# yahoo/bftkv

Measured on AMD Instinct MI355X. Metric: pgp_rsa2048_signature_verifies_per_sec, higher is better.
Workload: dtype u32; 1 GPU; 64-replica quorum, 10000 RSA-2048 signed writes per GPU (cfg2 of BASELINE.json), 534164 signature packets per GPU, 1.0% corrupt / 0.5% unknown issuer / 0.5% duplicate / 1.0% one-short; parallelism=shard-by-write x1, RCCL all-gather of verdict bitmaps on the verifier's stream, replicas=64, writes_per_gpu=10000, sigs_per_gpu=534164, batches_in_flight=3

## Files before the change

### bftkv_amd/_native.py

```python
from __future__ import annotations

import ctypes as C
import os
from typing import Optional

import numpy as np

_HERE = os.path.dirname(os.path.abspath(__file__))
LIB_PATH = os.path.join(_HERE, "libbftkv_gpu.so")


class NativeError(RuntimeError):
    pass


class PubKey(C.Structure):
    _fields_ = [("key_id", C.c_uint64), ("entity_id", C.c_uint64), ("pk_algo", C.c_uint8),
                ("usable_sign", C.c_uint8), ("reserved", C.c_uint8 * 6),
                ("n", C.c_void_p), ("n_len", C.c_uint32), ("e", C.c_void_p), ("e_len", C.c_uint32),
                ("g", C.c_void_p), ("g_len", C.c_uint32), ("y", C.c_void_p), ("y_len", C.c_uint32)]


class QC(C.Structure):
    _fields_ = [("f", C.c_int32), ("min", C.c_int32), ("threshold", C.c_int32), ("suff", C.c_int32),
                ("node_ids", C.c_void_p), ("n_nodes", C.c_uint32)]


EXPORTS = [
    "bftkv_gpu_init", "bftkv_gpu_destroy", "bftkv_gpu_last_error", "bftkv_gpu_error_string",
    "bftkv_gpu_keyring_set", "bftkv_gpu_quorum_create", "bftkv_gpu_quorum_destroy",
    "bftkv_gpu_collective_verify", "bftkv_gpu_collective_verify_dev", "bftkv_gpu_sync",
    "bftkv_gpu_signature_verify", "bftkv_gpu_last_statuses", "bftkv_gpu_last_counters",
    "bftkv_gpu_signers", "bftkv_gpu_quorum_tally", "bftkv_gpu_modexp", "bftkv_gpu_last_timing",
    "bftkv_gpu_stream", "bftkv_gpu_modmul_product", "bftkv_gpu_lagrange_combine", "bftkv_gpu_dsa_calculate_r", "bftkv_gpu_selftest_reduce",
    "bftkv_gpu_comm_unique_id", "bftkv_gpu_comm_init", "bftkv_gpu_allgather_verdicts", "bftkv_gpu_sss_distribute", "bftkv_gpu_modinv",
    "bftkv_gpu_batcher_create", "bftkv_gpu_batcher_destroy", "bftkv_gpu_batcher_collective_verify",
    "bftkv_gpu_batcher_signature_verify", "bftkv_gpu_batcher_stats", "bftkv_gpu_set_dsa_window_bits", "bftkv_gpu_dsa_window_bits", "bftkv_gpu_set_dsa_table_budget", "bftkv_gpu_dsa_table_bytes", "bftkv_gpu_collective_verify_segments", "bftkv_gpu_message_verify", "bftkv_gpu_batcher_message_verify",
    "bftkv_gpu_modexp_ops", "bftkv_gpu_allgather_errs_dev", "bftkv_gpu_set_early_exit", "bftkv_gpu_last_sclk_mhz", "bftkv_gpu_modmul_product_dev", "bftkv_gpu_lagrange_combine_dev",
    "bftkv_gpu_dsa_calculate_r_dev", "bftkv_gpu_sss_distribute_dev", "bftkv_gpu_modinv_dev",
    "bftkv_gpu_ctx_fork", "bftkv_gpu_batcher_create_lanes", "bftkv_gpu_batcher_times", "bftkv_gpu_comm_library", "bftkv_gpu_comm_selftest",
    "bftkv_gpu_collective_verify_small", "bftkv_gpu_signature_verify_small", "bftkv_gpu_set_hash_policy", "bftkv_gpu_signers_fenced",
    "bftkv_gpu_set_host_pipeline", "bftkv_gpu_batcher_cert_verify", "bftkv_gpu_host_pipeline_trace",
    "bftkv_gpu_batcher_cert_entity", "bftkv_gpu_set_lagrange_x_bound", "bftkv_gpu_batcher_modmul_product", "bftkv_gpu_batcher_lagrange_combine", "bftkv_gpu_batcher_dsa_calculate_r", "bftkv_gpu_batcher_modexp",
    "bftkv_gpu_ecdsa_calculate_r", "bftkv_gpu_ecdsa_calculate_r_dev", "bftkv_gpu_batcher_ecdsa_calculate_r", "bftkv_gpu_ec_scalar_base_mult",
    "bftkv_gpu_ecdsa_verify", "bftkv_gpu_ecdsa_verify_dev", "bftkv_gpu_batcher_ecdsa_verify",
    "bftkv_gpu_dsa_verify", "bftkv_gpu_dsa_verify_dev", "bftkv_gpu_batcher_dsa_verify",
    "bftkv_gpu_ecdsa_keyset_create", "bftkv_gpu_ecdsa_keyset_destroy", "bftkv_gpu_ecdsa_keyset_info", "bftkv_gpu_ecdsa_verify_keyset",
    "bftkv_gpu_ecdsa_verify_keyset_dev", "bftkv_gpu_batcher_ecdsa_verify_keyset", "bftkv_gpu_selftest_ecdsa_keyset_table",
    "bftkv_gpu_dsa_keyset_create", "bftkv_gpu_dsa_keyset_destroy", "bftkv_gpu_dsa_keyset_info", "bftkv_gpu_dsa_verify_keyset",
    "bftkv_gpu_dsa_verify_keyset_dev", "bftkv_gpu_batcher_dsa_verify_keyset", "bftkv_gpu_selftest_dsa_keyset_table",
    "bftkv_gpu_rsa_verify", "bftkv_gpu_rsa_verify_dev", "bftkv_gpu_rsa_keyset_create", "bftkv_gpu_rsa_keyset_destroy", "bftkv_gpu_rsa_keyset_info",
    "bftkv_gpu_rsa_verify_keyset", "bftkv_gpu_rsa_verify_keyset_dev", "bftkv_gpu_batcher_rsa_verify", "bftkv_gpu_batcher_rsa_verify_keyset",
]

_lib = None


def load_library() -> C.CDLL:
    global _lib
    if _lib is not None:
        return _lib
    if not os.path.exists(LIB_PATH):
        raise NativeError("%s not built -- run `python -c 'import __graft_entry__ as g; g.build()'`" % LIB_PATH)
    lib = C.CDLL(LIB_PATH)
    vp, u32, u64p, u8p = C.c_void_p, C.c_uint32, C.c_void_p, C.c_void_p
    lib.bftkv_gpu_init.argtypes = [C.c_int, C.POINTER(vp)]
    lib.bftkv_gpu_destroy.argtypes = [vp]
    lib.bftkv_gpu_destroy.restype = None
    lib.bftkv_gpu_last_error.argtypes = [vp]
    lib.bftkv_gpu_last_error.restype = C.c_char_p
    lib.bftkv_gpu_error_string.argtypes = [C.c_int]
    lib.bftkv_gpu_error_string.restype = C.c_char_p
    lib.bftkv_gpu_keyring_set.argtypes = [vp, C.POINTER(PubKey), u32]
    lib.bftkv_gpu_set_dsa_window_bits.argtypes = [vp, u32]
    lib.bftkv_gpu_dsa_window_bits.argtypes = [vp, C.POINTER(u32)]
    lib.bftkv_gpu_set_dsa_table_budget.argtypes = [vp, C.c_uint64]
    lib.bftkv_gpu_dsa_table_bytes.argtypes = [vp, C.POINTER(C.c_uint64), C.POINTER(u32)]
    lib.bftkv_gpu_set_hash_policy.argtypes = [vp, C.c_int, C.c_int]
    lib.bftkv_gpu_message_verify.argtypes = [vp, u32, vp, vp, vp, vp, vp, vp, C.c_uint64, vp, vp, vp]
    lib.bftkv_gpu_quorum_create.argtypes = [vp, C.POINTER(QC), u32, C.POINTER(C.c_int)]
    lib.bftkv_gpu_quorum_destroy.argtypes = [vp, C.c_int]
    lib.bftkv_gpu_collective_verify.argtypes = [vp, C.c_int, u32, u8p, u64p, u8p, u64p, u8p, vp, u8p, u8p]
    lib.bftkv_gpu_collective_verify_segments.argtypes = [vp, C.c_int, u32, u8p, u64p, u8p, u64p, u32, vp, u8p, u64p, u8p, vp, u8p, u8p]
    lib.bftkv_gpu_collective_verify_dev.argtypes = [vp, C.c_int, u32, u8p, u64p, u8p, u64p, C.c_uint64, u8p, vp, u8p, u8p]
    lib.bftkv_gpu_collective_verify_small.argtypes = [vp, C.c_int, u32, u8p, u64p, u8p, u64p, u8p, u8p]
    lib.bftkv_gpu_signature_verify_small.argtypes = [vp, u32, u8p, u64p, u8p, u64p, u64p, u8p, u8p]
    lib.bftkv_gpu_sync.argtypes = [vp]
    lib.bftkv_gpu_signature_verify.argtypes = [vp, u32, u8p, u64p, u8p, u64p, u64p, u8p, u8p]
    lib.bftkv_gpu_last_statuses.argtypes = [vp, u8p, vp, u32, C.POINTER(u32)]
    lib.bftkv_gpu_last_counters.argtypes = [vp, C.POINTER(C.c_uint64)]
    lib.bftkv_gpu_signers.argtypes = [vp, u32, u8p, u64p, u64p, u64p, C.c_uint64]
    lib.bftkv_gpu_signers_fenced.argtypes = [vp, u32, u8p, u64p, u64p, u64p, C.c_uint64, u8p]
    lib.bftkv_gpu_quorum_tally.argtypes = [vp, C.c_int, u32, u64p, u64p, u8p]
    lib.bftkv_gpu_modexp.argtypes = [vp, u32, u8p, u32, vp, u32, u8p, u8p, u32, u8p]
    lib.bftkv_gpu_last_timing.argtypes = [vp, C.POINTER(C.c_float)]
    lib.bftkv_gpu_modmul_product.argtypes = [vp, u32, u32, u8p, u32, vp, u32, u8p, u8p]
    lib.bftkv_gpu_lagrange_combine.argtypes = [vp, u32, u32, vp, u8p, u32, vp, u32, u8p, u8p, u8p]
    lib.bftkv_gpu_dsa_calculate_r.argtypes = [vp, u32, u32, vp, u8p, u32, u8p, u32, vp, u32, u8p, u8p, u8p, u8p]
    lib.bftkv_gpu_stream.argtypes = [vp]
    lib.bftkv_gpu_batcher_create.argtypes = [vp, u32, u32]
    lib.bftkv_gpu_batcher_create.restype = vp
    lib.bftkv_gpu_batcher_create_lanes.argtypes = [vp, u32, u32, u32]
    lib.bftkv_gpu_batcher_create_lanes.restype = vp
    lib.bftkv_gpu_ctx_fork.argtypes = [vp, C.POINTER(vp)]
    lib.bftkv_gpu_batcher_destroy.argtypes = [vp]
    lib.bftkv_gpu_batcher_destroy.restype = None
    lib.bftkv_gpu_batcher_collective_verify.argtypes = [vp, C.c_int, C.c_char_p, C.c_uint64, C.c_char_p, C.c_uint64, u8p, u8p]
    lib.bftkv_gpu_batcher_signature_verify.argtypes = [vp, C.c_char_p, C.c_uint64, C.c_char_p, C.c_uint64, vp, u8p, u8p]
    lib.bftkv_gpu_batcher_cert_verify.argtypes = [vp, C.c_char_p, C.c_uint64, C.c_char_p, C.c_uint64, C.c_char_p, C.c_uint64, u8p, u8p, vp, u8p]
    lib.bftkv_gpu_set_lagrange_x_bound.argtypes = [vp, u32]
    lib.bftkv_gpu_batcher_cert_entity.argtypes = [vp, C.c_char_p, C.c_uint64, u8p, u8p, vp, u8p, vp, vp, vp, u32, vp]
    lib.bftkv_gpu_batcher_message_verify.argtypes = [vp, C.c_char_p, C.c_uint64, vp, vp, vp, vp, C.c_uint64, vp, vp, vp]
    lib.bftkv_gpu_batcher_stats.argtypes = [vp, C.POINTER(C.c_uint64)]
    lib.bftkv_gpu_batcher_modmul_product.argtypes = [vp, u32, u8p, u32, u8p, u8p, u8p]
    lib.bftkv_gpu_batcher_lagrange_combine.argtypes = [vp, u32, vp, u8p, u32, u8p, u8p, u8p]
    lib.bftkv_gpu_batcher_dsa_calculate_r.argtypes = [vp, u32, vp, u8p, u32, u8p, u32, u8p, u8p, u8p, u8p]
    lib.bftkv_gpu_batcher_modexp.argtypes = [vp, u8p, u32, u8p, u32, u8p, u8p, u8p]
    lib.bftkv_gpu_batcher_times.argtypes = [vp, C.POINTER(C.c_uint64)]
    lib.bftkv_gpu_sss_distribute.argtypes = [vp, u32, u32, u32, u8p, u32, vp, u32, u8p, u8p]
    lib.bftkv_gpu_modinv.argtypes = [vp, u32, u8p, u32, vp, u32, u8p, u8p, u8p]
    lib.bftkv_gpu_comm_unique_id.argtypes = [u8p]
    lib.bftkv_gpu_comm_init.argtypes = [vp, C.c_int, C.c_int, u8p]
    lib.bftkv_gpu_comm_library.argtypes = [C.c_char_p, u32, C.POINTER(C.c_int)]
    lib.bftkv_gpu_comm_selftest.argtypes = [vp, u32, C.POINTER(u32)]
    lib.bftkv_gpu_allgather_verdicts.argtypes = [vp, u8p, C.c_uint64, u8p]
    lib.bftkv_gpu_stream.restype = vp
    lib.bftkv_gpu_set_early_exit.argtypes = [vp, C.c_int]
    lib.bftkv_gpu_set_host_pipeline.argtypes = [vp, u32]
    lib.bftkv_gpu_host_pipeline_trace.argtypes = [vp, C.POINTER(C.c_float), u32, C.POINTER(u32)]
    lib.bftkv_gpu_last_sclk_mhz.argtypes = [vp, C.POINTER(C.c_float)]
    lib.bftkv_gpu_modexp_ops.argtypes = lib.bftkv_gpu_modexp.argtypes
    lib.bftkv_gpu_allgather_errs_dev.argtypes = [vp, u8p, u32, u32, u8p]
    lib.bftkv_gpu_modmul_product_dev.argtypes = lib.bftkv_gpu_modmul_product.argtypes
    lib.bftkv_gpu_lagrange_combine_dev.argtypes = lib.bftkv_gpu_lagrange_combine.argtypes
    lib.bftkv_gpu_dsa_calculate_r_dev.argtypes = lib.bftkv_gpu_dsa_calculate_r.argtypes
    lib.bftkv_gpu_sss_distribute_dev.argtypes = lib.bftkv_gpu_sss_distribute.argtypes
    lib.bftkv_gpu_modinv_dev.argtypes = lib.bftkv_gpu_modinv.argtypes
    lib.bftkv_gpu_ecdsa_calculate_r.argtypes = [vp, u32, u32, vp, u8p, u8p, u8p, u32, u8p, u8p]
    lib.bftkv_gpu_ecdsa_calculate_r_dev.argtypes = lib.bftkv_gpu_ecdsa_calculate_r.argtypes
    lib.bftkv_gpu_batcher_ecdsa_calculate_r.argtypes = [vp, u32, vp, u8p, u8p, u8p, u32, u8p, u8p]
    lib.bftkv_gpu_ec_scalar_base_mult.argtypes = [vp, u32, u8p, u32, u8p, u32, u8p, u8p]
    lib.bftkv_gpu_ecdsa_verify.argtypes = [vp, u32, u8p, u32, u8p, vp, u32, u8p, u8p, u32, u8p, u8p]
    lib.bftkv_gpu_ecdsa_verify_dev.argtypes = lib.bftkv_gpu_ecdsa_verify.argtypes
    lib.bftkv_gpu_batcher_ecdsa_verify.argtypes = [vp, u8p, u32, u8p, u8p, u8p, u32, u8p, u8p]
    lib.bftkv_gpu_dsa_verify.argtypes = [vp, u32, u8p, u32, u8p, u32, vp, u32, u8p, vp, u32, u32, u8p, u8p, u8p, u8p, u8p]
    lib.bftkv_gpu_dsa_verify_dev.argtypes = lib.bftkv_gpu_dsa_verify.argtypes
    lib.bftkv_gpu_batcher_dsa_verify.argtypes = [vp, u8p, u32, u8p, u32, u8p, u32, u8p, u8p, u8p, u8p, u8p]
    lib.bftkv_gpu_ecdsa_keyset_create.argtypes = [vp, u32, u8p, u8p, u32, C.POINTER(C.c_int)]
    lib.bftkv_gpu_ecdsa_keyset_destroy.argtypes = [vp, C.c_int]
    lib.bftkv_gpu_ecdsa_keyset_info.argtypes = [vp, C.c_int, C.POINTER(u32), C.POINTER(u32), C.POINTER(u32), C.POINTER(C.c_uint64)]
    lib.bftkv_gpu_ecdsa_verify_keyset.argtypes = [vp, C.c_int, u32, u8p, u32, u8p, vp, u8p, u8p]
    lib.bftkv_gpu_ecdsa_verify_keyset_dev.argtypes = lib.bftkv_gpu_ecdsa_verify_keyset.argtypes
    lib.bftkv_gpu_batcher_ecdsa_verify_keyset.argtypes = [vp, C.c_int, u32, u8p, u32, u8p, u8p, u8p]
    lib.bftkv_gpu_selftest_ecdsa_keyset_table.argtypes = [vp, C.c_int, u32, vp, C.c_uint64]
    lib.bftkv_gpu_dsa_keyset_create.argtypes = [vp, u32, u8p, vp, u32, u32, u8p, u8p, u8p, u32, u32, C.POINTER(C.c_int)]
    lib.bftkv_gpu_dsa_keyset_destroy.argtypes = [vp, C.c_int]
    lib.bftkv_gpu_dsa_keyset_info.argtypes = [vp, C.c_int] + [C.POINTER(u32)] * 6 + [C.POINTER(C.c_uint64)]
    lib.bftkv_gpu_dsa_verify_keyset.argtypes = [vp, C.c_int, u32, u8p, u32, u8p, vp, u8p, u8p]
    lib.bftkv_gpu_dsa_verify_keyset_dev.argtypes = lib.bftkv_gpu_dsa_verify_keyset.argtypes
    lib.bftkv_gpu_batcher_dsa_verify_keyset.argtypes = [vp, C.c_int, u32, u8p, u32, u8p, u8p, u8p]
    lib.bftkv_gpu_selftest_dsa_keyset_table.argtypes = [vp, C.c_int, u32, vp, C.c_uint64]
    lib.bftkv_gpu_rsa_verify.argtypes = [vp, u32, u8p, u32, u32, u8p, u32, vp, u32, u8p, vp, u8p, u8p]
    lib.bftkv_gpu_rsa_verify_dev.argtypes = lib.bftkv_gpu_rsa_verify.argtypes
    lib.bftkv_gpu_rsa_keyset_create.argtypes = [vp, u32, u8p, vp, u32, C.POINTER(C.c_int)]
    lib.bftkv_gpu_rsa_keyset_destroy.argtypes = [vp, C.c_int]
    lib.bftkv_gpu_rsa_keyset_info.argtypes = [vp, C.c_int] + [C.POINTER(u32)] * 3
    lib.bftkv_gpu_rsa_verify_keyset.argtypes = [vp, C.c_int, u32, u8p, u32, u32, u8p, vp, u8p, u8p]
    lib.bftkv_gpu_rsa_verify_keyset_dev.argtypes = lib.bftkv_gpu_rsa_verify_keyset.argtypes
    lib.bftkv_gpu_batcher_rsa_verify.argtypes = [vp, u8p, u32, u32, u8p, u32, u8p, u32, u8p, u8p]
    lib.bftkv_gpu_batcher_rsa_verify_keyset.argtypes = [vp, C.c_int, u32, u8p, u32, u32, u8p, u8p, u8p]
    for name in EXPORTS:
        if name not in ("bftkv_gpu_destroy", "bftkv_gpu_last_error", "bftkv_gpu_error_string", "bftkv_gpu_stream",
                        "bftkv_gpu_batcher_create", "bftkv_gpu_batcher_create_lanes", "bftkv_gpu_batcher_destroy"):
            getattr(lib, name).restype = C.c_int
    _lib = lib
    return lib


def _ptr(a: Optional[np.ndarray]):
    if a is None:
        return None
    assert a.flags["C_CONTIGUOUS"]
    return a.ctypes.data_as(C.c_void_p)


class Context:

    def __init__(self, device: int = 0):
        self.lib = load_library()
        h = C.c_void_p()
        rc = self.lib.bftkv_gpu_init(device, C.byref(h))
        if rc != 0:
            raise NativeError("bftkv_gpu_init(device=%d) failed with %d: no usable MI355X / HIP runtime "
                              "(there is no CPU fallback)" % (device, rc))
        self.h = h
        self._keep = []

    def close(self):
        if self.h:
            self.lib.bftkv_gpu_destroy(self.h)
            self.h = None

    def set_hash_policy(self, hash_id: int, state: int):
        self._check(self.lib.bftkv_gpu_set_hash_policy(self.h, hash_id, state), "set_hash_policy")

    def fork(self) -> "Context":
        h = C.c_void_p()
        self._check(self.lib.bftkv_gpu_ctx_fork(self.h, C.byref(h)), "ctx_fork")
        f = Context.__new__(Context)
        f.lib, f.h, f._keep, f.root = self.lib, h, [], self
        return f

    def __del__(self):
        try:
            self.close()
        except Exception:
            pass

    def _check(self, rc: int, what: str):
        if rc != 0:
            raise NativeError("%s failed (%d): %s" % (what, rc, self.lib.bftkv_gpu_last_error(self.h).decode()))

    def keyring_set(self, keys):
        keys = list(keys)
        arr = (PubKey * max(1, len(keys)))()
        bufs = []
        for i, k in enumerate(keys):
            arr[i].key_id = k["key_id"]
            arr[i].entity_id = k.get("entity_id", k["key_id"])
            arr[i].pk_algo = k["pk_algo"]
            arr[i].usable_sign = 1 if k.get("usable_sign", True) else 0
            for name in ("n", "e", "g", "y"):
                b = k.get(name) or b""
                cb = C.create_string_buffer(b, len(b)) if b else None
                bufs.append(cb)
                setattr(arr[i], name, C.cast(cb, C.c_void_p) if cb is not None else None)
                setattr(arr[i], name + "_len", len(b))
        self._check(self.lib.bftkv_gpu_keyring_set(self.h, arr, len(keys)), "keyring_set")

    def message_verify(self, messages):
        n = len(messages)
        blob = np.frombuffer(b"".join(messages), dtype=np.uint8) if n and sum(map(len, messages)) else np.zeros(1, dtype=np.uint8)
        off = np.zeros(n + 1, dtype=np.uint64)
        off[1:] = np.cumsum([len(m) for m in messages], dtype=np.uint64)
        st = np.zeros(max(1, n), dtype=np.uint8)
        signer = np.zeros(max(1, n), dtype=np.uint64)
        peer = np.zeros(max(1, n), dtype=np.uint64)
        plain = np.zeros(max(1, int(off[n])), dtype=np.uint8)
        poff = np.zeros(n + 1, dtype=np.uint64)
        fn = np.zeros((max(1, n), 256), dtype=np.uint8)
        fl = np.zeros(max(1, n), dtype=np.uint8)
        self._check(self.lib.bftkv_gpu_message_verify(self.h, n, _ptr(np.ascontiguousarray(blob)), _ptr(off), _ptr(st), _ptr(signer), _ptr(peer),
                                                      _ptr(plain), len(plain), _ptr(poff), _ptr(fn), _ptr(fl)), "message_verify")
        plains = [plain[int(poff[i]):int(poff[i + 1])].tobytes() for i in range(n)]
        names = [fn[i, :int(fl[i])].tobytes() for i in range(n)]
        return st[:n], signer[:n], peer[:n], plains, names

    def set_early_exit(self, on: bool) -> None:
        self._check(self.lib.bftkv_gpu_set_early_exit(self.h, 1 if on else 0), "set_early_exit")

    def set_host_pipeline(self, pieces: int, copy: str = "", tight: bool = False) -> None:
        mode = {"": 0, "ring": 0x100, "direct": 0x200}[copy]
        self._check(self.lib.bftkv_gpu_set_host_pipeline(self.h, pieces | mode | (0x400 if tight else 0)), "set_host_pipeline")

    def host_pipeline_trace(self):
        buf = (C.c_float * 96)()
        n = C.c_uint32(0)
        self._check(self.lib.bftkv_gpu_host_pipeline_trace(self.h, buf, 96, C.byref(n)), "host_pipeline_trace")
        v = [float(buf[i]) for i in range(min(96, n.value))]
        if not v:
            return None
        P = int(v[0])
        names = ("ss_enqueued", "payload_enqueued", "picked_up", "payload_hook", "enqueued", "drained", "gpu_start", "gpu_modexp_start", "gpu_modexp_end", "gpu_end")
        return {"pieces": P, "ring": bool(v[1]), "copiers_joined_us": v[2], "copy_stream_drained_us": v[3], "done_us": v[4], "largest_piece_items": int(v[5]), "second_passes": int(v[6]),
                "per_piece_us": [{nm: round(v[8 + 10 * k + j], 1) for j, nm in enumerate(names)} for k in range(P)]}

    def set_dsa_window_bits(self, bits: int) -> None:
        self._check(self.lib.bftkv_gpu_set_dsa_window_bits(self.h, bits), "set_dsa_window_bits")

    def dsa_window_bits(self) -> int:
        b = C.c_uint32(0)
        self._check(self.lib.bftkv_gpu_dsa_window_bits(self.h, C.byref(b)), "dsa_window_bits")
        return int(b.value)

    def set_dsa_table_budget(self, nbytes: int) -> None:
        self._check(self.lib.bftkv_gpu_set_dsa_table_budget(self.h, int(nbytes)), "set_dsa_table_budget")

    def dsa_table_bytes(self):
        b, e = C.c_uint64(0), C.c_uint32(0)
        self._check(self.lib.bftkv_gpu_dsa_table_bytes(self.h, C.byref(b), C.byref(e)), "dsa_table_bytes")
        return int(b.value), int(e.value)

    def quorum_create(self, qcs) -> int:
        qcs = list(qcs)
        arr = (QC * max(1, len(qcs)))()
        keep = []
        for i, (f, mn, thr, suff, nodes) in enumerate(qcs):
            ids = np.ascontiguousarray(np.array(list(nodes), dtype=np.uint64))
            keep.append(ids)
            arr[i].f, arr[i].min, arr[i].threshold, arr[i].suff = f, mn, thr, suff
            arr[i].node_ids = ids.ctypes.data if len(ids) else None
            arr[i].n_nodes = len(ids)
        out = C.c_int(-1)
        self._check(self.lib.bftkv_gpu_quorum_create(self.h, arr, len(qcs), C.byref(out)), "quorum_create")
        return out.value

    def quorum_destroy(self, q: int):
        self._check(self.lib.bftkv_gpu_quorum_destroy(self.h, q), "quorum_destroy")

    def collective_verify(self, quorum: int, tbs_blob, tbs_off, ss_blob, ss_off):
        n = len(tbs_off) - 1
        tbs_blob, ss_blob = _u8(tbs_blob), _u8(ss_blob)
        tbs_off, ss_off = _u64(tbs_off), _u64(ss_off)
        err = np.zeros(n, dtype=np.uint8)
        nver = np.zeros(n, dtype=np.uint32)
        verdict = np.zeros(n, dtype=np.uint8)
        self.last_fenced = np.zeros(n, dtype=np.uint8)
        small = self.collective_verify_small(quorum, tbs_blob, tbs_off, ss_blob, ss_off) if self._cross_check(n) else None
        self._check(self.lib.bftkv_gpu_collective_verify(self.h, quorum, n, _ptr(tbs_blob), _ptr(tbs_off), _ptr(ss_blob),
                                                         _ptr(ss_off), _ptr(err), _ptr(nver), _ptr(verdict), _ptr(self.last_fenced)),
                    "collective_verify")
        self._compare_small("collective_verify", small, err, self.last_fenced)
        return err, nver, verdict

    check_small = False

    def collective_verify_segments(self, quorum: int, prefix_blob, prefix_off, shared_blob, shared_off, seg_of_item, ss_blob, ss_off):
        n = len(prefix_off) - 1
        prefix_blob, shared_blob, ss_blob = _u8(prefix_blob), _u8(shared_blob), _u8(ss_blob)
        prefix_off, shared_off, ss_off = _u64(prefix_off), _u64(shared_off), _u64(ss_off)
        seg = np.ascontiguousarray(seg_of_item, dtype=np.uint32)
        err = np.zeros(n, dtype=np.uint8)
        nver = np.zeros(n, dtype=np.uint32)
        verdict = np.zeros(n, dtype=np.uint8)
        self.last_fenced = np.zeros(n, dtype=np.uint8)
        self._check(self.lib.bftkv_gpu_collective_verify_segments(self.h, quorum, n, _ptr(prefix_blob), _ptr(prefix_off), _ptr(shared_blob),
                                                                  _ptr(shared_off), len(shared_off) - 1, _ptr(seg), _ptr(ss_blob), _ptr(ss_off),
                                                                  _ptr(err), _ptr(nver), _ptr(verdict), _ptr(self.last_fenced)),
                    "collective_verify_segments")
        return err, nver, verdict

    def _cross_check(self, n: int) -> bool:
        return bool(self.check_small) and 0 < n <= 4096

    @staticmethod
    def _compare_small(what, small, err, fenced):
        if small is None:
            return
        e2, f2 = small
        if not (np.array_equal(e2, err) and np.array_equal(f2, fenced)):
            bad = [int(i) for i in np.nonzero((e2 != err) | (f2 != fenced))[0][:8]]
            raise NativeError("%s: the small-call route disagrees with the batched one at items %s: err %s vs %s, fenced %s vs %s"
                              % (what, bad, e2[bad].tolist(), err[bad].tolist(), f2[bad].tolist(), fenced[bad].tolist()))

    def collective_verify_small(self, quorum: int, tbs_blob, tbs_off, ss_blob, ss_off):
        n = len(tbs_off) - 1
        tbs_blob, ss_blob = _u8(tbs_blob), _u8(ss_blob)
        tbs_off, ss_off = _u64(tbs_off), _u64(ss_off)
        err = np.zeros(n, dtype=np.uint8)
        fenced = np.zeros(n, dtype=np.uint8)
        self._check(self.lib.bftkv_gpu_collective_verify_small(self.h, quorum, n, _ptr(tbs_blob), _ptr(tbs_off), _ptr(ss_blob), _ptr(ss_off),
                                                               _ptr(err), _ptr(fenced)), "collective_verify_small")
        return err, fenced

    def signature_verify_small(self, tbs_blob, tbs_off, sig_blob, sig_off, cert_key_id=None):
        n = len(tbs_off) - 1
        tbs_blob, sig_blob = _u8(tbs_blob), _u8(sig_blob)
        tbs_off, sig_off = _u64(tbs_off), _u64(sig_off)
        ck = None if cert_key_id is None else _u64(cert_key_id)
        err = np.zeros(n, dtype=np.uint8)
        fenced = np.zeros(n, dtype=np.uint8)
        self._check(self.lib.bftkv_gpu_signature_verify_small(self.h, n, _ptr(tbs_blob), _ptr(tbs_off), _ptr(sig_blob), _ptr(sig_off), _ptr(ck),
                                                              _ptr(err), _ptr(fenced)), "signature_verify_small")
        return err, fenced

    def collective_verify_dev(self, quorum: int, n_items: int, tbs_ptr: int, tbs_off_ptr: int, ss_ptr: int, ss_off_ptr: int,
                              ss_len: int, err_ptr: int, nver_ptr: int, verdict_ptr: int, fenced_ptr: int = 0):
        self._check(self.lib.bftkv_gpu_collective_verify_dev(self.h, quorum, n_items, tbs_ptr, tbs_off_ptr, ss_ptr, ss_off_ptr,
                                                             ss_len, err_ptr, nver_ptr, verdict_ptr, fenced_ptr or None), "collective_verify_dev")

    def sync(self):
        self._check(self.lib.bftkv_gpu_sync(self.h), "sync")

    def signature_verify(self, tbs_blob, tbs_off, sig_blob, sig_off, cert_key_id=None):
        n = len(tbs_off) - 1
        tbs_blob, sig_blob = _u8(tbs_blob), _u8(sig_blob)
        tbs_off, sig_off = _u64(tbs_off), _u64(sig_off)
        ck = None if cert_key_id is None else _u64(cert_key_id)
        err = np.zeros(n, dtype=np.uint8)
        self.last_fenced = np.zeros(n, dtype=np.uint8)
        small = self.signature_verify_small(tbs_blob, tbs_off, sig_blob, sig_off, cert_key_id) if self._cross_check(n) else None
        self._check(self.lib.bftkv_gpu_signature_verify(self.h, n, _ptr(tbs_blob), _ptr(tbs_off), _ptr(sig_blob), _ptr(sig_off),
                                                        _ptr(ck), _ptr(err), _ptr(self.last_fenced)), "signature_verify")
        self._compare_small("signature_verify", small, err, self.last_fenced)
        return err

    def last_statuses(self):
        n = C.c_uint32(0)
        self._check(self.lib.bftkv_gpu_last_statuses(self.h, None, None, 0, C.byref(n)), "last_statuses")
        st = np.zeros(max(1, n.value), dtype=np.uint8)
        item = np.zeros(max(1, n.value), dtype=np.uint32)
        self._check(self.lib.bftkv_gpu_last_statuses(self.h, _ptr(st), _ptr(item), n.value, C.byref(n)), "last_statuses")
        return st[:n.value], item[:n.value]

    def last_counters(self):
        c = (C.c_uint64 * 4)()
        self._check(self.lib.bftkv_gpu_last_counters(self.h, c), "last_counters")
        return {"packets": c[0], "pubkey_ops": c[1], "items": c[2], "dsa_ops": c[3]}

    def last_sclk_mhz(self) -> float:
        v = C.c_float(0)
        self._check(self.lib.bftkv_gpu_last_sclk_mhz(self.h, C.byref(v)), "last_sclk_mhz")
        return float(v.value)

    def last_timing(self):
        ms = (C.c_float * 8)()
        self._check(self.lib.bftkv_gpu_last_timing(self.h, ms), "last_timing")
        return {"total": ms[0], "parse": ms[1], "hash": ms[2], "rsa": ms[3], "tally": ms[4], "compare": ms[5], "dsa": ms[6]}

    def signers(self, ss_blob, ss_off):
        n = len(ss_off) - 1
        ss_blob, ss_off = _u8(ss_blob), _u64(ss_off)
        cap = max(1, int(len(ss_blob) // 12) + 1)
        ids = np.zeros(cap, dtype=np.uint64)
        off = np.zeros(n + 1, dtype=np.uint64)
        self.last_fenced = np.zeros(n, dtype=np.uint8)
        self._check(self.lib.bftkv_gpu_signers_fenced(self.h, n, _ptr(ss_blob), _ptr(ss_off), _ptr(ids), _ptr(off), cap, _ptr(self.last_fenced)), "signers")
        return ids[:int(off[n])], off

    def quorum_tally(self, quorum: int, ids, list_off):
        n = len(list_off) - 1
        ids, list_off = _u64(ids), _u64(list_off)
        v = np.zeros(n, dtype=np.uint8)
        self._check(self.lib.bftkv_gpu_quorum_tally(self.h, quorum, n, _ptr(ids), _ptr(list_off), _ptr(v)), "quorum_tally")
        return v

    @staticmethod
    def comm_unique_id() -> np.ndarray:
        uid = np.zeros(128, dtype=np.uint8)
        rc = load_library().bftkv_gpu_comm_unique_id(_ptr(uid))
        if rc:
            raise NativeError("bftkv_gpu_comm_unique_id failed (%d): librccl not loadable" % rc)
        return uid

    def comm_init(self, n_ranks: int, rank: int, uid: np.ndarray):
        self._check(self.lib.bftkv_gpu_comm_init(self.h, n_ranks, rank, _ptr(np.ascontiguousarray(uid, dtype=np.uint8))), "comm_init")

    @staticmethod
    def comm_library():
        buf = C.create_string_buffer(1024)
        pre = C.c_int(0)
        rc = load_library().bftkv_gpu_comm_library(buf, 1024, C.byref(pre))
        if rc:
            raise NativeError("bftkv_gpu_comm_library failed (%d): librccl not loadable" % rc)
        return buf.value.decode(), bool(pre.value)

    def comm_selftest(self, nbytes: int = 4096):
        bad = C.c_uint32(0)
        self._check(self.lib.bftkv_gpu_comm_selftest(self.h, nbytes, C.byref(bad)), "comm_selftest")

    def allgather_verdicts(self, local_ptr: int, nbytes: int, out_ptr: int):
        self._check(self.lib.bftkv_gpu_allgather_verdicts(self.h, local_ptr, nbytes, out_ptr), "allgather_verdicts")

    def allgather_errs_dev(self, err_ptr: int, n_items: int, slots: int, out_ptr: int):
        self._check(self.lib.bftkv_gpu_allgather_errs_dev(self.h, err_ptr, n_items, slots, out_ptr), "allgather_errs_dev")

    def modmul_product(self, factors, moduli, mod_idx, nbytes: int = 256):
        n, k = len(factors), len(factors[0])
        f = _ints_to_be([x for row in factors for x in row], nbytes)
        m = _ints_to_be(moduli, nbytes)
        mi = np.ascontiguousarray(mod_idx, dtype=np.uint32)
        out = np.zeros((n, nbytes), dtype=np.uint8)
        self._check(self.lib.bftkv_gpu_modmul_product(self.h, n, k, _ptr(f), nbytes, _ptr(mi), len(moduli), _ptr(m), _ptr(out)), "modmul_product")
        return [int.from_bytes(out[i].tobytes(), "big") for i in range(n)]

    def lagrange_combine(self, xs, ys, moduli, mod_idx, nbytes: int = 256):
        n, k = len(xs), len(xs[0])
        x = np.ascontiguousarray(np.array(xs, dtype=np.int32))
        y = _ints_to_be([v for row in ys for v in row], nbytes)
        m = _ints_to_be(moduli, nbytes)
        mi = np.ascontiguousarray(mod_idx, dtype=np.uint32)
        out = np.zeros((n, nbytes), dtype=np.uint8)
        st = np.zeros(n + 8, dtype=np.uint8)
        self._check(self.lib.bftkv_gpu_lagrange_combine(self.h, n, k, _ptr(x), _ptr(y), nbytes, _ptr(mi), len(moduli), _ptr(m), _ptr(out),
                                                        _ptr(st)), "lagrange_combine")
        return [int.from_bytes(out[i].tobytes(), "big") for i in range(n)], st[:n]

    def dsa_calculate_r(self, xs, ri, vi, groups, group_idx, pbytes: int = 256, qbytes: int = 32):
        n, k = len(xs), len(xs[0])
        x = np.ascontiguousarray(np.array(xs, dtype=np.int32))
        r = _ints_to_be([v for row in ri for v in row], pbytes)
# ... 445 lines not shown
```

### bftkv_amd/csrc/capi.hip

```cpp
#include "../../include/bftkv_gpu.h"

#include <hip/hip_runtime.h>
#include <stdio.h>
#include <stdlib.h>
#include <string.h>

#include <limits.h>
#include <linux/futex.h>
#include <sched.h>
#include <sys/syscall.h>
#include <unistd.h>

#include <algorithm>
#include <array>
#include <atomic>
#include <memory>
#include <functional>
#include <map>
#include <set>
#include <chrono>
#include <condition_variable>
#include <mutex>
#include <shared_mutex>
#include <system_error>
// ... 16 lines not shown

inline void copy_out(void* dst, const void* src, size_t n) { if (n) memcpy(dst, src, n); }

struct DevBuf {
  void* p = nullptr;
  size_t cap = 0;
  hipError_t ensure(size_t bytes) {
    if (bytes <= cap) return hipSuccess;
    if (p) { hipError_t e = hipFree(p); if (e != hipSuccess) return e; p = nullptr; cap = 0; }
    size_t want = bytes + bytes / 4 + 256;
    hipError_t e = hipMalloc(&p, want);
    if (e == hipSuccess) cap = want;
    return e;
  }
  hipError_t ensure_exact(size_t bytes) {
    if (bytes <= cap) return hipSuccess;
    if (p) { hipError_t e = hipFree(p); if (e != hipSuccess) return e; p = nullptr; cap = 0; }
    hipError_t e = hipMalloc(&p, bytes);
    if (e == hipSuccess) cap = bytes;
    return e;
  }
  void release() { if (p) (void)hipFree(p); p = nullptr; cap = 0; }
  template <typename T> T* as() const { return (T*)p; }
};

struct KeyEntry {
  uint64_t key_id = 0, entity_id = 0;
  uint8_t algo = 0, flags = 0;
  uint32_t bits = 0, e = 0, n0 = 0, qbits = 0, n0_29 = 0;
  std::vector<uint32_t> nl29, r2_29;
  std::vector<uint32_t> nl, r2, r2w, qw, dtab, qpow, qconst;
  std::string material;
  bool cert_only = false;
  int cert_group = -1;
  uint32_t entity_index = 0;
  std::string cert_digest;
  uint64_t last_used = 0;
  bool dsa_unslotted = false;
};

struct QuorumHost {
  bool live = false;
  int n_qcs = 0;
  int32_t f[MAX_QC], mn[MAX_QC], thr[MAX_QC], suff[MAX_QC];
  std::vector<std::vector<uint64_t>> nodes;
  DevBuf member;
  uint64_t keyring_gen = ~0ull;
  DevBuf ids;
  uint32_t ids_off[MAX_QC + 1];
};

struct EcKeySet {
  bool live = false;
  int curve_id = -1;
  uint32_t bits = 0, n_keys = 0, n_refused = 0;
  uint32_t w = 0, nwin = 0;
  size_t key_words = 0;
  std::vector<uint8_t> curve;
  DevBuf tab;
  DevBuf refused;
  DevBuf mod[4];
  void release() { tab.release(); refused.release(); for (DevBuf& b : mod) b.release(); }
};

struct DsaKeySet {
  bool live = false;
  uint32_t n_keys = 0, n_groups = 0, pbytes = 0, qbytes = 0;
  uint32_t w = 0, windows = 0;
  DevBuf tab;
  DevBuf modp[3], modq[3];
  DevBuf q_be, key_group;
  uint64_t table_bytes() const { return (uint64_t)(n_groups + n_keys) * windows * ((1u << w) - 1u) * MONT_N * 4; }
  static ModTab rows(const DevBuf (&m)[3]) { return ModTab{m[0].as<uint32_t>(), m[1].as<uint32_t>(), m[2].as<uint32_t>(), nullptr}; }
  void release() { tab.release(); q_be.release(); key_group.release(); for (DevBuf& b : modp) b.release(); for (DevBuf& b : modq) b.release(); }
};

struct RsaKeySet {
  bool live = false;
  uint32_t n_keys = 0, n_refused = 0, nbytes = 0;
  DevBuf n29, r2_29, n80, r2_80;
  DevBuf meta;
  void release() { n29.release(); r2_29.release(); n80.release(); r2_80.release(); meta.release(); }
};

}

using ctx_lock = std::lock_guard<std::recursive_mutex>;

struct bftkv_gpu_ctx {
  int device = 0;
  hipStream_t stream = nullptr;
  hipStream_t stream_h = nullptr;
  hipStream_t stream_d = nullptr;
  std::recursive_mutex mu;
  std::string err;

  uint64_t keyring_gen = 0;
  uint32_t n_keys = 0, n_entities = 0;
  bool have_dsa_keys = false, have_rsa3072 = false, have_rsa4096 = false, have_ambiguous = false;
  std::vector<uint64_t> h_key_id, h_entity_id;
  std::vector<uint32_t> h_key_entity;
  std::vector<uint8_t> h_key_flags;
  std::vector<KeyEntry> ring, certs;
  uint32_t n_ring_entities = 0;
  std::map<std::string, bool> cert_valid;
  DevBuf k_r2w;
  DevBuf k_n29, k_r2_29, k_n0_29;
  DevBuf k_id, k_entity, k_algo, k_flags, k_bits, k_e, k_n, k_r2, k_n0, k_q, k_qbits, k_dsatab, k_dsaslot, k_sorted_id, k_sorted_slot;
  DevBuf dsa_comb;
  uint32_t dsa_wbits = 8, dsa_wbits_pinned = 0;
  std::map<std::string, uint32_t> dsa_comb_slot;
  std::set<std::string> dsa_cert_materials;
  uint64_t ring_epoch = 0, dsa_ring_epoch_seen = ~0ull;
  uint32_t dsa_wbits_want = 0;
  uint32_t dsa_entry_limbs = DSA_N_SMALL;
  size_t dsa_budget_bytes = 0;
  bool have_dsa3072 = false, have_dsa2048 = false;
  DevBuf dsa_idx;
  uint64_t cert_clock = 0;
  struct CertFast { uint64_t issuer_id; int group; uint64_t epoch; };
  std::shared_mutex cert_fast_mu;
  std::unordered_map<std::string, CertFast> cert_fast;
  size_t cert_fast_bytes = 0;
  uint64_t cert_epoch = 0, kt_cert_epoch = 0;
  std::vector<uint32_t> kt_group_ent;
  KeyTableDev kt{};

  std::vector<QuorumHost> quorums;
  std::vector<EcKeySet> ec_keysets;
  std::vector<DsaKeySet> dsa_keysets;
  std::vector<RsaKeySet> rsa_keysets;

  DevBuf txt_mid32, txt_mid64, txt_tail, txt_len;
  DevBuf forced_iss;
  DevBuf counts, base, total, item_flags, walk_scratch, cert_ent, sig_class, mid, mid64, hash_mask, recs, digests, r, xr, pk_list, pk_list3072, pk_list4096, r3072, r4096, pk_count, dsa_list, dsa_u, ids_tmp;
  DevBuf o_err, o_nver, o_verdict, o_fenced;
  DevBuf in_tbs, in_tbs_off, in_ss, in_ss_off;
  hipEvent_t seg_ev = nullptr;
  DevBuf in_prefix, in_prefix_off, in_shared, in_shared_off, in_seg;
  DevBuf st_tmp, item_tmp, bits_tmp, plan_cut;
  DevBuf chunk_arena, chunk_ctr;
  uint32_t multiexp_parts = 0;
  uint32_t ec_split = 0;
  uint32_t ec_window = 0;
  DevBuf ec_fb_tab[4];
  uint32_t ec_fb_w[4] = {};
  uint32_t multiexp_block = 0;
  uint32_t multiexp_lanes = 0;
  uint32_t rsav_lanes = 0;
  uint32_t dsa_inv_mode = 0;
  uint32_t n_cus = 256;
  uint32_t lagrange_x_bound = 0;
  bool early_exit = true;
  std::vector<DevBuf*> scratch_pool;
  std::unordered_map<std::string, std::vector<uint32_t>> modrow_cache;
  std::unordered_map<std::string, std::vector<uint32_t>> rsav_row_cache[2];
  std::map<std::string, std::array<DevBuf, 4>> modtab_cache;
  uint32_t* h_mail = nullptr;
  uint32_t* d_mail = nullptr;
  uint32_t last_total = 0, last_rsa = 0, last_items = 0;
  bool last_total_on_dev = false;
  hipEvent_t ev[10] = {};
  hipEvent_t ev_turn = nullptr;
  bool have_timing = false;
  void* rccl_comm = nullptr;
  int n_ranks = 1, rank = 0;

  bftkv_gpu_ctx* root = nullptr;
  std::shared_mutex kt_rw;
  std::atomic<int> kt_writers{0};
  std::atomic<int> n_forks{0};
  uint64_t quorum_gen = 0;
  uint64_t seen_keyring_gen = ~0ull, seen_quorum_gen = ~0ull;
  size_t n_dsa_slots = 0;
  int kt_read_depth = 0;
  DevBuf in_pack;
  uint8_t* h_out = nullptr; uint8_t* d_out = nullptr; size_t out_cap = 0;
  uint32_t out_seq = 0;
  std::vector<bftkv_gpu_ctx*> hb_workers;
  hipStream_t stream_c = nullptr;
  hipStream_t stream_c2 = nullptr;
  std::vector<hipEvent_t> hb_ev;
  uint8_t* hb_out = nullptr; size_t hb_out_cap = 0;
  uint32_t modexp_lds_pad = 0;
  uint32_t hb_pieces = 0;
  hipEvent_t hb_ev0 = nullptr;
  bool hb_tight = false;
  uint32_t hb_copy_mode = 0;
  void* hb_ring = nullptr;
  std::vector<float> hb_trace;
  uint32_t hb_last_pieces = 0;
  std::vector<uint32_t> hb_item0;
  void* small_pin = nullptr;
  uint32_t staged_spin_us = 50000;
};

void rccl_release(bftkv_gpu_ctx* c);
void release_small_pin(bftkv_gpu_ctx* c);
extern "C" int signature_verify_entities(bftkv_gpu_ctx* c, uint32_t n_items, const uint8_t* tbs, const uint64_t* tbs_off, const uint8_t* sig,
                                         const uint64_t* sig_off, const uint32_t* ent, uint8_t* err_out, const uint8_t* sig_class = nullptr,
                                         uint8_t* fenced_out = nullptr, const uint64_t* forced_issuer = nullptr);

namespace {

int fork_refresh(bftkv_gpu_ctx* c);

struct KtWrite {
  bftkv_gpu_ctx* c;
  explicit KtWrite(bftkv_gpu_ctx* c_) : c(c_) { c->kt_writers.fetch_add(1); c->kt_rw.lock(); }
  ~KtWrite() { c->kt_rw.unlock(); c->kt_writers.fetch_sub(1); }
};
struct KtRead {
  bftkv_gpu_ctx *c, *r;
  int rc = 0;
  explicit KtRead(bftkv_gpu_ctx* c_) : c(c_), r(c_->root) {
    if (!r || c->kt_read_depth++ > 0) return;
    while (r->kt_writers.load(std::memory_order_acquire) > 0) std::this_thread::yield();
    r->kt_rw.lock_shared();
    rc = fork_refresh(c);
  }
  ~KtRead() { if (r && --c->kt_read_depth == 0) r->kt_rw.unlock_shared(); }
};

struct Turnstile { std::mutex mu; hipEvent_t last = nullptr; const void* owner = nullptr; };
Turnstile g_turnstile[16];
constexpr uint64_t HB_PIPE_MIN_BYTES = 24ull << 20;
constexpr uint32_t HB_PIPE_MAX_PIECES = 8;
std::mutex g_hb_mu[16];
constexpr size_t HB_TR = 10;
struct HbRing {
  static constexpr size_t SLOT = 16u << 20;
  static constexpr int NSLOT = 6;
  static constexpr int THREADS = 4;
  uint8_t* base = nullptr;
  hipEvent_t ev[NSLOT] = {};
  bool used[NSLOT] = {};
// ... 138 lines not shown
  HIPCHK(c, c->mid.ensure(sizeof(uint32_t) * 8 * N_MID32 * (size_t)n_items + 16));
  HIPCHK(c, c->mid64.ensure(sizeof(uint64_t) * 8 * 2 * (size_t)n_items + 16));
  HIPCHK(c, c->hash_mask.ensure(sizeof(uint32_t) * (size_t)n_items + 16));
  constexpr size_t CHUNK_ARENA_MIN = 64u << 10;
  if (!c->chunk_ctr.p) { HIPCHK(c, c->chunk_ctr.ensure(16)); HIPCHK(c, hipMemsetAsync(c->chunk_ctr.p, 0, 16, c->stream)); }
  HIPCHK(c, c->chunk_arena.ensure(CHUNK_ARENA_MIN + (staged_cap ? 2 * (size_t)ss_len : 0)));
  HIPCHK(c, c->pk_count.ensure(96));
  if (plan_q) HIPCHK(c, c->plan_cut.ensure(sizeof(uint32_t) * (size_t)n_items + 16));
  TextDev txt{nullptr, nullptr, nullptr, nullptr};
  if (!d_mid_in) {
    HIPCHK(c, c->txt_mid32.ensure(sizeof(uint32_t) * 8 * N_MID32 * (size_t)n_items + 16));
    HIPCHK(c, c->txt_mid64.ensure(sizeof(uint64_t) * 8 * N_MID64 * (size_t)n_items + 16));
    HIPCHK(c, c->txt_tail.ensure((size_t)128 * N_HASHES * n_items + 16));
    HIPCHK(c, c->txt_len.ensure(sizeof(uint64_t) * N_HASHES * (size_t)n_items + 16));
    txt = TextDev{c->txt_mid32.as<uint32_t>(), c->txt_mid64.as<uint64_t>(), c->txt_tail.as<uint8_t>(), c->txt_len.as<uint64_t>()};
  }
  if (ev_input) HIPCHK(c, hipStreamWaitEvent(s, ev_input, 0));
  HIPCHK(c, rec(0, s));
  HIPCHK(c, join(sh, 0));
  HIPCHK(c, rec(5, sh));
  if (!upload_tbs && !d_mid_in)
    hipLaunchKernelGGL(k_sha256_mid, dim3((n_items + 63) / 64), dim3(64), 0, sh, d_tbs, d_tbs_off, n_items, c->mid.as<uint32_t>());
  hipLaunchKernelGGL(k_walk<false>, dim3(n_items), dim3(64), 0, s, d_ss, d_ss_off, n_items, c->counts.as<uint32_t>(),
                     (const uint32_t*)nullptr, (SigRec*)nullptr, c->item_flags.as<uint8_t>(), c->walk_scratch.as<WalkEnt>(), walk_cap,
                     c->chunk_ctr.as<uint32_t>());
  constexpr uint32_t MAIL_EMPTY = 0xFFFFFFFFu;
  if (c->h_mail && !staged_cap) __atomic_store_n(&c->h_mail[0], MAIL_EMPTY, __ATOMIC_RELEASE);
  hipLaunchKernelGGL(k_scan_counts, dim3(1), dim3(1024), 0, s, c->counts.as<uint32_t>(), n_items, c->base.as<uint32_t>(),
                     c->total.as<uint32_t>(), staged_cap ? (uint32_t*)nullptr : c->d_mail, c->pk_count.as<uint32_t>(), c->hash_mask.as<uint32_t>(),
                     staged_cap, c->chunk_ctr.as<uint32_t>());
  uint32_t total = staged_cap ? staged_cap : MAIL_EMPTY;
  const uint32_t* const n_recs_dev = staged_cap ? c->total.as<uint32_t>() : nullptr;
  if (c->h_mail && !staged_cap) {
    const auto t_spin = std::chrono::steady_clock::now();
    for (uint32_t it = 0;; ++it) {
      total = __atomic_load_n(&c->h_mail[0], __ATOMIC_ACQUIRE);
      if (total != MAIL_EMPTY) break;
      if ((it & 1023u) == 1023u && std::chrono::steady_clock::now() - t_spin > std::chrono::milliseconds(20)) break;
      __builtin_ia32_pause();
    }
  }
  uint32_t chunk_units = (c->h_mail && !staged_cap && total != MAIL_EMPTY) ? c->h_mail[2] : 0u;
  if (total == MAIL_EMPTY) {
    HIPCHK(c, hipMemcpyAsync(&total, c->total.p, sizeof(uint32_t), hipMemcpyDeviceToHost, s));
    HIPCHK(c, hipMemcpyAsync(&chunk_units, c->chunk_ctr.as<uint32_t>() + 2, sizeof(uint32_t), hipMemcpyDeviceToHost, s));
    HIPCHK(c, hipStreamSynchronize(s));
  }
  if (!staged_cap && (size_t)chunk_units * 16 > c->chunk_arena.cap) HIPCHK(c, c->chunk_arena.ensure((size_t)chunk_units * 16));
  c->last_total = staged_cap ? 0u : total;
  c->last_total_on_dev = staged_cap != 0 && ev_input != nullptr;
  c->last_items = n_items;
  c->hb_last_pieces = 0;
  const size_t tr = total ? total : 1;
  HIPCHK(c, c->recs.ensure(sizeof(SigRec) * tr));
  HIPCHK(c, c->digests.ensure(sizeof(uint32_t) * 16 * tr));
  HIPCHK(c, c->r.ensure(sizeof(uint32_t) * EM_LOW_LIMBS * tr));
  HIPCHK(c, c->xr.ensure(sizeof(uint32_t) * (c->have_rsa4096 ? MONT_NMAX : c->have_rsa3072 ? MONT_TPI_BIG * MONT_L3072 : 80) * tr));
  HIPCHK(c, c->pk_list.ensure(sizeof(uint32_t) * tr));
  HIPCHK(c, c->pk_list3072.ensure(c->have_rsa3072 ? sizeof(uint32_t) * tr : 16));
  HIPCHK(c, c->pk_list4096.ensure(c->have_rsa4096 ? sizeof(uint32_t) * tr : 16));
  if (c->have_rsa3072) HIPCHK(c, c->r3072.ensure(sizeof(uint32_t) * EM_LOW_LIMBS * tr));
  if (c->have_rsa4096) HIPCHK(c, c->r4096.ensure(sizeof(uint32_t) * EM_LOW_LIMBS * tr));
  HIPCHK(c, c->dsa_list.ensure(sizeof(uint32_t) * tr));
  if (c->have_dsa_keys) HIPCHK(c, c->dsa_u.ensure(sizeof(uint32_t) * DSA_U_WORDS * tr));
  if (c->have_dsa3072 && c->have_dsa2048) HIPCHK(c, c->dsa_idx.ensure(sizeof(uint32_t) * 4 * (size_t)tr + 16));
  hipLaunchKernelGGL(k_walk<true>, dim3(n_items), dim3(64), 0, s, d_ss, d_ss_off, n_items, c->counts.as<uint32_t>(),
                     c->base.as<uint32_t>(), c->recs.as<SigRec>(), c->item_flags.as<uint8_t>(), (WalkEnt*)nullptr, walk_cap, (uint32_t*)nullptr);
  if (total) {
    ParseArgs pa;
    pa.sig_blob = d_ss; pa.sig_off = d_ss_off; pa.rec_base = c->base.as<uint32_t>(); pa.counts = c->counts.as<uint32_t>(); pa.n_items = n_items;
    pa.scratch = c->walk_scratch.as<WalkEnt>(); pa.walk_cap = walk_cap; pa.recs = c->recs.as<SigRec>(); pa.n_recs = total; pa.cert_ent = d_cert_ent;
    pa.pk_list = c->pk_list.as<uint32_t>(); pa.pk_list3072 = c->pk_list3072.as<uint32_t>(); pa.pk_list4096 = c->pk_list4096.as<uint32_t>();
    pa.pk_count = c->pk_count.as<uint32_t>(); pa.dsa_list = c->dsa_list.as<uint32_t>(); pa.item_hash_mask = c->hash_mask.as<uint32_t>();
    pa.sig_class = d_sig_class; pa.forced_issuer = d_forced_issuer; pa.msg_slot = d_msg_slot; pa.msg_hash = d_msg_hash; pa.item_flags = c->item_flags.as<uint8_t>();
    pa.defer_queue = plan_q ? 1u : 0u;
    pa.n_recs_dev = n_recs_dev;
    pa.chunk_arena = c->chunk_arena.as<uint8_t>(); pa.chunk_cap_units = (uint32_t)std::min<size_t>(c->chunk_arena.cap / 16, 0xFFFFFFF0u);
    pa.chunk_bump = c->chunk_ctr.as<uint32_t>() + 1;
    if (!staged_cap && (uint64_t)total >= 128ull * n_items)
      hipLaunchKernelGGL(k_parse_body_items, dim3(n_items), dim3(PARSE_ITEM_BLOCK), 0, s, pa, c->kt);
    else
      hipLaunchKernelGGL(k_parse_body, dim3((total + 255) / 256), dim3(256), 0, s, pa, c->kt);
  }
  uint32_t* const cnt_p = c->pk_count.as<uint32_t>();
  const uint32_t* const start0 = cnt_p + 12;
  PlanArgs pl{};
  if (total && plan_q) {
    pl.recs = c->recs.as<SigRec>(); pl.rec_base = c->base.as<uint32_t>(); pl.counts = c->counts.as<uint32_t>(); pl.n_items = n_items;
    pl.pk_list = c->pk_list.as<uint32_t>(); pl.dsa_list = c->dsa_list.as<uint32_t>(); pl.pk_list3072 = c->pk_list3072.as<uint32_t>();
    pl.pk_list4096 = c->pk_list4096.as<uint32_t>(); pl.pk_count = cnt_p; pl.plan_cut = c->plan_cut.as<uint32_t>(); pl.verdict = nullptr;
    int min_suff = 0;
    for (int i = 0; i < plan_q->n_qcs; ++i) if (plan_q->suff[i] > 0 && (min_suff == 0 || plan_q->suff[i] < min_suff)) min_suff = plan_q->suff[i];
    pl.margin = 1u + (uint32_t)min_suff / 64u;
    pl.mail = c->d_mail ? c->d_mail + 3 : nullptr;
    if (c->h_mail) __atomic_store_n(&c->h_mail[3], 0u, __ATOMIC_RELEASE);
    hipLaunchKernelGGL(k_plan<1>, dim3((n_items + PLAN_ITEMS - 1) / PLAN_ITEMS), dim3(PLAN_BLOCK), 0, s, pl, c->kt, *plan_q);
  }
  const bool dsa_side = total && c->have_dsa_keys;
  if (one_stream && dsa_side) HIPCHK(c, hipEventRecord(c->ev[1], s)); else HIPCHK(c, rec(1, s));
  const size_t n_slots = c->root ? c->n_dsa_slots : c->dsa_comb_slot.size();
  const uint32_t inv_batch_min = c->dsa_inv_mode == 1 || n_slots > (c->dsa_inv_mode == 2 ? (size_t)INV_MAX_SLOTS : 256) ? 0xFFFFFFFFu
                                 : c->dsa_inv_mode == 2 ? 0u : (uint32_t)std::max<size_t>(4096, 64 * n_slots);
  auto launch_dsa_inv = [&](hipStream_t st, const uint32_t* start) {
    if (inv_batch_min != 0xFFFFFFFFu)
      hipLaunchKernelGGL(k_dsa_inv_batched, dim3((total + INV_TILE - 1) / INV_TILE), dim3(INV_BLOCK), 0, st, d_ss, c->recs.as<SigRec>(),
                         c->dsa_list.as<uint32_t>(), c->pk_count.as<uint32_t>(), start, c->kt, c->dsa_u.as<uint32_t>(), inv_batch_min);
    if (inv_batch_min != 0u)
      hipLaunchKernelGGL(k_dsa_inv, dim3((total + 63) / 64), dim3(64), 0, st, d_ss, c->recs.as<SigRec>(), c->dsa_list.as<uint32_t>(),
                         c->pk_count.as<uint32_t>(), start, c->kt, c->dsa_u.as<uint32_t>(), inv_batch_min);
  };
  if (total && c->have_dsa_keys) {
    HIPCHK(c, hipStreamWaitEvent(c->stream_d, c->ev[1], 0));
    launch_dsa_inv(c->stream_d, start0);
    HIPCHK(c, hipEventRecord(c->ev[7], c->stream_d));
  }
  auto hash_stream_work = [&]() -> int {
    HIPCHK(c, join(sh, 1));
    if (total) {
      if (!d_mid_in) {
        hipLaunchKernelGGL(k_hash_mid_other, dim3((n_items + 63) / 64, N_HASHES - 1), dim3(64), 0, sh, d_tbs, d_tbs_off, n_items,
                           c->hash_mask.as<uint32_t>(), c->mid.as<uint32_t>(), c->mid64.as<uint64_t>());
        hipLaunchKernelGGL(k_hash_mid_text, dim3((n_items + 63) / 64, N_HASHES), dim3(64), 0, sh, d_tbs, d_tbs_off, n_items, c->hash_mask.as<uint32_t>(), txt);
      }
      hipLaunchKernelGGL(k_digest_sha256, dim3((total + 255) / 256), dim3(256), 0, sh, d_tbs, d_tbs_off, d_ss,
                         d_mid_in ? d_mid_in : c->mid.as<uint32_t>(), c->mid64.as<uint64_t>(), n_items, c->recs.as<SigRec>(), total,
                         c->digests.as<uint32_t>(), d_tbs_prefix, n_recs_dev);
    }
    HIPCHK(c, rec(6, sh));
    return 0;
  };
  if (!upload_tbs) { int hrc = hash_stream_work(); if (hrc) return hrc; }
  const dim3 qg((total + MODEXP_BLOCK / MONT_TPI - 1) / (MODEXP_BLOCK / MONT_TPI));
  const dim3 qg8((total + MODEXP_BLOCK / MONT_TPI_BIG - 1) / (MODEXP_BLOCK / MONT_TPI_BIG));
  static const bool wide8_off = getenv("BFTKV_NO_WIDE8") != nullptr;
  const bool wide8 = staged_cap != 0 && ss_len / 256 <= 8192 && !wide8_off;
  auto launch_modexp = [&](const uint32_t* start) {
    if (wide8)
      hipLaunchKernelGGL((k_rsa_modexp<10, MONT_TPI_BIG>), qg8, dim3(MODEXP_BLOCK), 0, s, d_ss, c->recs.as<SigRec>(), c->pk_list.as<uint32_t>(),
                         cnt_p, start, c->kt, c->r.as<uint32_t>(), c->xr.as<uint32_t>(), (uint64_t*)(cnt_p + 16));
    else {
#if BFTKV_RSA_FORM == 29
      hipLaunchKernelGGL((k_rsa_modexp<RSA29_L, MONT_TPI, RSA29_W>), qg, dim3(MODEXP_BLOCK), c->modexp_lds_pad, s, d_ss, c->recs.as<SigRec>(), c->pk_list.as<uint32_t>(),
                         cnt_p, start, c->kt, c->r.as<uint32_t>(), c->xr.as<uint32_t>(), (uint64_t*)(cnt_p + 16), (const uint32_t*)(cnt_p + 5));
      hipLaunchKernelGGL((k_rsa_modexp<MONT_L, MONT_TPI, MONT_W, true>), qg, dim3(MODEXP_BLOCK), c->modexp_lds_pad, s, d_ss, c->recs.as<SigRec>(), c->pk_list.as<uint32_t>(),
                         cnt_p, start, c->kt, c->r.as<uint32_t>(), c->xr.as<uint32_t>(), (uint64_t*)nullptr, (const uint32_t*)(cnt_p + 5));
#else
      hipLaunchKernelGGL((k_rsa_modexp<MONT_L, MONT_TPI>), qg, dim3(MODEXP_BLOCK), c->modexp_lds_pad, s, d_ss, c->recs.as<SigRec>(), c->pk_list.as<uint32_t>(),
                         cnt_p, start, c->kt, c->r.as<uint32_t>(), c->xr.as<uint32_t>(), (uint64_t*)(cnt_p + 16));
#endif
    }
    if (c->have_rsa3072)
      hipLaunchKernelGGL((k_rsa_modexp<MONT_L3072, MONT_TPI_BIG>), qg8, dim3(MODEXP_BLOCK), 0, s, d_ss, c->recs.as<SigRec>(), c->pk_list3072.as<uint32_t>(),
                         cnt_p + 2, start + 2, c->kt, c->r3072.as<uint32_t>(), c->xr.as<uint32_t>(), (uint64_t*)nullptr);
    if (c->have_rsa4096)
      hipLaunchKernelGGL((k_rsa_modexp<MONT_L4096, MONT_TPI_BIG>), qg8, dim3(MODEXP_BLOCK), 0, s, d_ss, c->recs.as<SigRec>(), c->pk_list4096.as<uint32_t>(),
                         cnt_p + 3, start + 3, c->kt, c->r4096.as<uint32_t>(), c->xr.as<uint32_t>(), (uint64_t*)nullptr);
  };
  static const bool turnstile_off = getenv("BFTKV_NO_TURNSTILE") != nullptr;
  const bool big = staged_cap ? (ev_input != nullptr && ss_len / 320 >= TURNSTILE_MIN_PACKETS) : total >= TURNSTILE_MIN_PACKETS;
  if (big && !turnstile_off) {
    Turnstile& g = g_turnstile[(unsigned)c->device & 15u];
    std::lock_guard<std::mutex> tl(g.mu);
    if (g.last && g.owner != c) HIPCHK(c, hipStreamWaitEvent(s, g.last, 0));
    HIPCHK(c, rec(9, s));
    launch_modexp(start0);
    if (!c->ev_turn) HIPCHK(c, hipEventCreateWithFlags(&c->ev_turn, hipEventDisableTiming));
    HIPCHK(c, hipEventRecord(c->ev_turn, s));
    g.last = c->ev_turn; g.owner = c;
  } else {
    HIPCHK(c, rec(9, s));
    if (total) launch_modexp(start0);
  }
  HIPCHK(c, rec(2, s));
  if (upload_tbs) {
    int hrc = (*upload_tbs)(sh);
    if (hrc) return hrc;
    if (!mid_prelaunched)
      hipLaunchKernelGGL(k_sha256_mid, dim3((n_items + 63) / 64), dim3(64), 0, sh, d_tbs, d_tbs_off, n_items, c->mid.as<uint32_t>());
    if ((hrc = hash_stream_work())) return hrc;
  }
  HIPCHK(c, join(s, 6));
  bool other_hashes = true;
  if (total && !d_mid_in && plan_q && big && c->h_mail) {
    const auto t_spin = std::chrono::steady_clock::now();
    for (uint32_t it = 0;; ++it) {
      const uint32_t v = __atomic_load_n(&c->h_mail[3], __ATOMIC_ACQUIRE);
      if (v) { other_hashes = (v & 1u) != 0; break; }
      if ((it & 255u) == 255u && std::chrono::steady_clock::now() - t_spin > std::chrono::microseconds(300) + std::chrono::nanoseconds((uint64_t)total / 2)) break;
      __builtin_ia32_pause();
    }
  }
  if (total && !d_mid_in && other_hashes)
    hipLaunchKernelGGL(k_digest_other, dim3(std::min<uint32_t>((total + 255) / 256, DIGEST_OTHER_MAX_BLOCKS)), dim3(256), 0, s,
                       d_tbs, d_tbs_off, d_ss, c->mid.as<uint32_t>(), c->mid64.as<uint64_t>(), n_items, c->recs.as<SigRec>(), total,
                       c->digests.as<uint32_t>(), c->pk_count.as<uint32_t>() + 4, txt, n_recs_dev);
  const dim3 cg(((uint64_t)total * CMP_LANES + 255) / 256);
  auto launch_compare = [&](const uint32_t* start) {
    hipLaunchKernelGGL(k_rsa_compare, cg, dim3(256), 0, s, c->recs.as<SigRec>(), c->pk_list.as<uint32_t>(),
                       cnt_p, start, c->kt, c->r.as<uint32_t>(), c->digests.as<uint32_t>());
    if (c->have_rsa3072)
      hipLaunchKernelGGL(k_rsa_compare, cg, dim3(256), 0, s, c->recs.as<SigRec>(), c->pk_list3072.as<uint32_t>(),
                         cnt_p + 2, start + 2, c->kt, c->r3072.as<uint32_t>(), c->digests.as<uint32_t>());
    if (c->have_rsa4096)
      hipLaunchKernelGGL(k_rsa_compare, cg, dim3(256), 0, s, c->recs.as<SigRec>(), c->pk_list4096.as<uint32_t>(),
                         cnt_p + 3, start + 3, c->kt, c->r4096.as<uint32_t>(), c->digests.as<uint32_t>());
  };
  auto launch_dsa = [&](const uint32_t* start) {
    hipLaunchKernelGGL(k_dsa_mul, dim3((total + 63) / 64), dim3(64), 0, s, c->recs.as<SigRec>(), c->dsa_list.as<uint32_t>(),
                       cnt_p, start, c->kt, c->digests.as<uint32_t>(), c->dsa_u.as<uint32_t>());
    const uint32_t* idx_s = nullptr; const uint32_t* idx_b = nullptr; const uint32_t* cnt_cls = nullptr;
    if (c->have_dsa3072 && c->have_dsa2048) {
      uint32_t* cc = cnt_p + (start == start0 ? 20 : 22);
      uint32_t* is = c->dsa_idx.as<uint32_t>() + (start == start0 ? 0 : 2 * (size_t)total);
      hipLaunchKernelGGL(k_dsa_split, dim3((total + 255) / 256), dim3(256), 0, s, c->recs.as<SigRec>(), c->dsa_list.as<uint32_t>(), cnt_p, start, c->kt,
                         is, is + total, cc);
      idx_s = is; idx_b = is + total; cnt_cls = cc;
    }
    if (c->have_dsa2048)
      hipLaunchKernelGGL((k_dsa_modexp<MONT_L, MONT_TPI>), dim3((total + QUADS_PER_BLOCK - 1) / QUADS_PER_BLOCK), dim3(RSA_BLOCK), 0, s,
                         c->recs.as<SigRec>(), c->dsa_list.as<uint32_t>(), cnt_p, start, c->kt, c->dsa_u.as<uint32_t>(), idx_s, cnt_cls);
    if (c->have_dsa3072)
      hipLaunchKernelGGL((k_dsa_modexp<MONT_L3072, MONT_TPI_BIG>), dim3((total + RSA_BLOCK / MONT_TPI_BIG - 1) / (RSA_BLOCK / MONT_TPI_BIG)), dim3(RSA_BLOCK), 0, s,
                         c->recs.as<SigRec>(), c->dsa_list.as<uint32_t>(), cnt_p, start, c->kt, c->dsa_u.as<uint32_t>(), idx_b, cnt_cls ? cnt_cls + 1 : nullptr);
  };
  if (total) launch_compare(start0);
  HIPCHK(c, rec(8, s));
  if (total && c->have_dsa_keys) {
    HIPCHK(c, hipStreamWaitEvent(s, c->ev[7], 0));
    launch_dsa(start0);
  }
  if (total && plan_q) {
    HIPCHK(c, c->o_nver.ensure(sizeof(uint32_t) * n_items));
    HIPCHK(c, c->o_verdict.ensure(n_items));
    hipLaunchKernelGGL(k_tally, dim3((n_items + 3) / 4), dim3(256), 0, s, c->recs.as<SigRec>(), c->base.as<uint32_t>(), c->counts.as<uint32_t>(),
                       n_items, c->kt, *plan_q, c->o_verdict.as<uint8_t>(), c->o_nver.as<uint32_t>(), (uint32_t*)nullptr);
    hipLaunchKernelGGL(k_plan_snapshot, dim3(1), dim3(64), 0, s, cnt_p);
    pl.verdict = c->o_verdict.as<uint8_t>();
    hipLaunchKernelGGL(k_plan<2>, dim3((n_items + PLAN_ITEMS - 1) / PLAN_ITEMS), dim3(PLAN_BLOCK), 0, s, pl, c->kt, *plan_q);
    const uint32_t* const start1 = cnt_p + 8;
    if (c->have_dsa_keys) launch_dsa_inv(s, start1);
    launch_modexp(start1);
    launch_compare(start1);
    if (c->have_dsa_keys) launch_dsa(start1);
  }
  if (total && c->have_ambiguous && !d_msg_slot)
    hipLaunchKernelGGL(k_candidates, dim3((total + 63) / 64), dim3(64), 0, s, d_tbs, d_tbs_off, d_ss, d_mid_in ? d_mid_in : c->mid.as<uint32_t>(),
                       c->mid64.as<uint64_t>(), n_items, c->recs.as<SigRec>(), total, n_recs_dev, d_tbs_prefix, c->kt, d_cert_ent, d_sig_class, txt,
                       c->hash_mask.as<uint32_t>());
  HIPCHK(c, rec(3, s));
  HIPCHK(c, hipGetLastError());
  return 0;
}

int make_key_entry(bftkv_gpu_ctx* c, const bftkv_gpu_pubkey& k, bool cert_only, KeyEntry* out) {
  KeyEntry& e = *out;
  e.key_id = k.key_id; e.entity_id = k.entity_id; e.algo = k.pk_algo; e.cert_only = cert_only;
  e.material.clear();
  e.material.push_back((char)k.pk_algo);
  e.material.push_back((char)k.usable_sign);
  auto app = [&](const uint8_t* p, uint32_t l) {
    uint32_t z = 0;
    while (z < l && p[z] == 0) ++z;
    if (l > z) e.material.append((const char*)p + z, l - z);
    e.material.push_back('|');
  };
  app(k.n, k.n_len); app(k.e, k.e_len); app(k.g, k.g_len); app(k.y, k.y_len);
  e.flags = 0;
  if (k.usable_sign) e.flags |= KEYF_USABLE_SIGN;
  if (k.pk_algo != PK_RSA_ENCRYPT_ONLY && k.pk_algo != PK_ELGAMAL) e.flags |= KEYF_CAN_SIGN;
  if (k.key_id == k.entity_id) e.flags |= KEYF_PRIMARY;
  if (cert_only) e.flags |= KEYF_CERT_ONLY;
  e.bits = (uint32_t)hostbn::bit_length(k.n, k.n_len);
  e.e = 0; e.n0 = 0; e.qbits = 0;
  e.r2w.clear(); e.nl29.clear(); e.r2_29.clear(); e.n0_29 = 0;
  e.nl.assign(MONT_NMAX, 0); e.r2.assign(MONT_NMAX, 0); e.qw.assign(8, 0); e.dtab.assign(2 * DSA_N_BIG, 0); e.qpow.clear(); e.qconst.clear();
  if (k.pk_algo == PK_RSA || k.pk_algo == PK_RSA_SIGN_ONLY) {
    if (hostbn::bit_length(k.e, k.e_len) > 32) return fail(c, BFTKV_E_UNSUPPORTED, "RSA public exponent wider than 32 bits");
    for (uint32_t j = 0; j < k.e_len; ++j) e.e = (e.e << 8) | k.e[j];
    const int nlimbs = e.bits <= 2048 ? MONT_N : (e.bits <= 3072 ? MONT_TPI_BIG * MONT_L3072 : MONT_TPI_BIG * MONT_L4096);
    if (e.bits > 4096) e.bits = 0xFFFFFFFFu;
    else if (!hostbn::mont_setup(k.n, k.n_len, nlimbs, e.nl.data(), e.r2.data(), &e.n0)) e.bits = 0xFFFFFFFFu;
    else if (e.bits <= 2048) {
      std::vector<uint32_t> nl80(80);
      uint32_t n0b = 0;
      e.r2w.assign(80, 0);
      (void)hostbn::mont_setup(k.n, k.n_len, 80, nl80.data(), e.r2w.data(), &n0b);
      e.nl29.assign(RSA29_N, 0); e.r2_29.assign(RSA29_N, 0);
      (void)hostbn::mont_setup(k.n, k.n_len, RSA29_N, e.nl29.data(), e.r2_29.data(), &e.n0_29, RSA29_W);
    }
  } else if (k.pk_algo == PK_DSA) {
    e.qbits = (uint32_t)hostbn::bit_length(k.e, k.e_len);
    const int NLp = e.bits <= 2048 ? (int)DSA_N_SMALL : (int)DSA_N_BIG;
    const uint32_t cap_bits = e.bits <= 2048 ? 2048u : 3072u;
    const int nwords = (28 * NLp + 31) / 32 + 1;
    std::vector<uint32_t> p(nwords), g(nwords), y(nwords), q(nwords);
    hostbn::from_be(k.e, k.e_len, q.data(), nwords);
    bool ok = e.bits >= 2 && e.bits <= 3072 && e.qbits >= 32 && e.qbits <= 256 && (q[0] & 1u) &&
              hostbn::mont_setup(k.n, k.n_len, NLp, e.nl.data(), e.r2.data(), &e.n0);
    if (ok && (hostbn::bit_length(k.g, k.g_len) > cap_bits || hostbn::bit_length(k.y, k.y_len) > cap_bits)) ok = false;
    if (ok) {
      hostbn::from_be(k.n, k.n_len, p.data(), nwords);
      hostbn::from_be(k.g, k.g_len, g.data(), nwords);
      hostbn::from_be(k.y, k.y_len, y.data(), nwords);
      hostbn::reduce(g.data(), p.data(), nwords);
      hostbn::reduce(y.data(), p.data(), nwords);
      hostbn::to_mont_limbs(g.data(), p.data(), nwords, NLp, &e.dtab[0]);
      hostbn::to_mont_limbs(y.data(), p.data(), nwords, NLp, &e.dtab[DSA_N_BIG]);
      for (int j = 0; j < 8; ++j) e.qw[j] = q[j];
      e.qpow.assign((size_t)NLp * 10, 0);
      uint32_t x[9] = {1, 0, 0, 0, 0, 0, 0, 0, 0}, q9[9];
      for (int j = 0; j < 9; ++j) q9[j] = j < 8 ? q[j] : 0;
      for (int j = 0; j < NLp; ++j) {
        hostbn::to_limbs28(x, 9, &e.qpow[(size_t)j * 10], 10);
        for (int b = 0; b < MONT_W; ++b) hostbn::dbl_mod(x, q9, 9);
      }
      e.qconst.assign(12, 0);
      uint32_t r2q[9] = {1, 0, 0, 0, 0, 0, 0, 0, 0};
      for (int b = 0; b < 512; ++b) hostbn::dbl_mod(r2q, q9, 9);
      for (int j = 0; j < 8; ++j) e.qconst[j] = r2q[j];
      uint32_t inv = 1;
      for (int it = 0; it < 5; ++it) inv *= 2u - q[0] * inv;
      e.qconst[8] = 0u - inv;
    } else {
      e.bits = 0xFFFFFFFFu;
// ... 221 lines not shown
    const_cast<KeyEntry&>(e).entity_index = group_ent;
    if (e.cert_group >= 0) {
      if (group_ents.size() <= (size_t)e.cert_group) group_ents.resize((size_t)e.cert_group + 1, 0xFFFFFFFEu);
      group_ents[(size_t)e.cert_group] = group_ent;
    }
  }
  std::vector<uint32_t> sorted_slot(key_id.size());
  for (size_t i = 0; i < sorted_slot.size(); ++i) sorted_slot[i] = (uint32_t)i;
  std::stable_sort(sorted_slot.begin(), sorted_slot.end(), [&](uint32_t a, uint32_t b) { return key_id[a] < key_id[b]; });
  std::vector<uint64_t> sorted_id(key_id.size());
  for (size_t i = 0; i < sorted_slot.size(); ++i) sorted_id[i] = key_id[sorted_slot[i]];
  int rc;
  if ((rc = upload(c, c->k_sorted_id, sorted_id)) || (rc = upload(c, c->k_sorted_slot, sorted_slot))) return rc;
  if ((rc = upload(c, c->k_id, key_id)) || (rc = upload(c, c->k_entity, entity)) || (rc = upload(c, c->k_algo, algo)) ||
      (rc = upload(c, c->k_flags, flags)) || (rc = upload(c, c->k_bits, bits)) || (rc = upload(c, c->k_e, e32)) ||
      (rc = upload(c, c->k_n, nl)) || (rc = upload(c, c->k_r2, r2)) || (rc = upload(c, c->k_n0, n0)) ||
      (rc = upload(c, c->k_q, qw)) || (rc = upload(c, c->k_qbits, qbits)) || (rc = upload(c, c->k_dsatab, dtab)) || (rc = upload(c, c->k_r2w, r2w)) ||
      (rc = upload(c, c->k_n29, nl29)) || (rc = upload(c, c->k_r2_29, r2_29)) || (rc = upload(c, c->k_n0_29, n0_29)))
    return rc;
  c->kt.r2_limbs80 = c->k_r2w.as<uint32_t>();
  c->kt.n_limbs29 = c->k_n29.as<uint32_t>(); c->kt.r2_limbs29 = c->k_r2_29.as<uint32_t>(); c->kt.n0inv29 = c->k_n0_29.as<uint32_t>();
  c->n_keys = (uint32_t)key_id.size();
  c->kt.n_keys = c->n_keys;
  c->kt.n_limbs = c->k_n.as<uint32_t>();
  c->kt.r2_limbs = c->k_r2.as<uint32_t>();
  c->kt.n0inv = c->k_n0.as<uint32_t>();
  c->kt.dsa_tab = c->k_dsatab.as<uint32_t>();
  bool bits_changed = false;
  if ((rc = sync_dsa_tables(c, rows, algo, bits, &bits_changed))) return rc;
  if (bits_changed && (rc = upload(c, c->k_bits, bits))) return rc;
  HIPCHK(c, hipStreamSynchronize(c->stream));
  c->have_dsa_keys = c->have_dsa3072 = c->have_dsa2048 = c->have_rsa3072 = c->have_rsa4096 = c->have_ambiguous = false;
  for (size_t i = 0; i < algo.size(); ++i) {
    if (flags[i] & KEYF_AMBIGUOUS) c->have_ambiguous = true;
    if (algo[i] == PK_DSA) c->have_dsa_keys = true;
    if (algo[i] == PK_DSA && bits[i] != 0xFFFFFFFFu && bits[i] > 2048) c->have_dsa3072 = true;
    if (algo[i] == PK_DSA && (bits[i] == 0xFFFFFFFFu || bits[i] <= 2048)) c->have_dsa2048 = true;
    if ((algo[i] == PK_RSA || algo[i] == PK_RSA_SIGN_ONLY) && bits[i] != 0xFFFFFFFFu) {
      if (bits[i] > 3072) c->have_rsa4096 = true; else if (bits[i] > 2048) c->have_rsa3072 = true;
    }
  }
  c->n_entities = (uint32_t)entity_ids.size();
  c->h_key_id = key_id;
  c->h_entity_id = entity_ids;
  c->h_key_entity = entity;
  c->h_key_flags = flags;
  c->kt.n_keys = c->n_keys;
  c->kt.key_id = c->k_id.as<uint64_t>();
  c->kt.sorted_id = c->k_sorted_id.as<uint64_t>();
  c->kt.sorted_slot = c->k_sorted_slot.as<uint32_t>();
  c->kt.entity = c->k_entity.as<uint32_t>();
  c->kt.pk_algo = c->k_algo.as<uint8_t>();
  c->kt.flags = c->k_flags.as<uint8_t>();
  c->kt.mod_bits = c->k_bits.as<uint32_t>();
  c->kt.rsa_e = c->k_e.as<uint32_t>();
  c->kt.n_limbs = c->k_n.as<uint32_t>();
  c->kt.r2_limbs = c->k_r2.as<uint32_t>();
  c->kt.n0inv = c->k_n0.as<uint32_t>();
  c->kt.q_words = c->k_q.as<uint32_t>();
  c->kt.q_bits = c->k_qbits.as<uint32_t>();
  c->kt.dsa_tab = c->k_dsatab.as<uint32_t>();
  c->kt.dsa_slot = c->k_dsaslot.as<uint32_t>();
  c->kt.dsa_comb = c->dsa_comb.as<uint32_t>();
  c->kt.dsa_wbits = c->dsa_wbits;
  c->kt.dsa_entry_limbs = c->dsa_entry_limbs;
  c->kt_group_ent = std::move(group_ents);
  c->kt_cert_epoch = c->cert_epoch;
  ++c->keyring_gen;
  return 0;
}

int fork_refresh(bftkv_gpu_ctx* c) {
  bftkv_gpu_ctx* r = c->root;
  if (c->seen_keyring_gen != r->keyring_gen) {
    c->kt = r->kt;
    c->n_keys = r->n_keys; c->n_entities = r->n_entities; c->n_ring_entities = r->n_ring_entities;
    c->have_dsa_keys = r->have_dsa_keys; c->have_dsa3072 = r->have_dsa3072; c->have_dsa2048 = r->have_dsa2048; c->have_rsa3072 = r->have_rsa3072; c->have_rsa4096 = r->have_rsa4096; c->have_ambiguous = r->have_ambiguous;
    c->h_key_id = r->h_key_id; c->h_entity_id = r->h_entity_id; c->h_key_entity = r->h_key_entity; c->h_key_flags = r->h_key_flags;
    c->n_dsa_slots = r->dsa_comb_slot.size(); c->dsa_wbits = r->dsa_wbits; c->dsa_entry_limbs = r->dsa_entry_limbs;
    c->keyring_gen = r->keyring_gen;
    c->seen_keyring_gen = r->keyring_gen;
  }
  c->early_exit = r->early_exit;
  if (c->seen_quorum_gen != r->quorum_gen) {
    for (auto& q : c->quorums) { q.member.release(); q.ids.release(); }
    c->quorums.clear();
    c->quorums.resize(r->quorums.size());
    for (size_t i = 0; i < r->quorums.size(); ++i) {
      const QuorumHost& s = r->quorums[i];
      QuorumHost& d = c->quorums[i];
      d.live = s.live; d.n_qcs = s.n_qcs; d.nodes = s.nodes;
      for (int k = 0; k < MAX_QC; ++k) { d.f[k] = s.f[k]; d.mn[k] = s.mn[k]; d.thr[k] = s.thr[k]; d.suff[k] = s.suff[k]; }
      d.keyring_gen = ~0ull;
    }
    c->seen_quorum_gen = r->quorum_gen;
  }
  return 0;
}

int check_offsets(bftkv_gpu_ctx* c, const uint64_t* off, uint32_t n, const char* what) {
  if (off[0] != 0) return fail(c, BFTKV_E_INVALID, what);
  for (uint32_t i = 0; i < n; ++i) if (off[i + 1] < off[i]) return fail(c, BFTKV_E_INVALID, what);
  return 0;
}

int check_quorum(bftkv_gpu_ctx* c, int quorum) {
  if (quorum < 0 || (size_t)quorum >= c->quorums.size() || !c->quorums[quorum].live) return fail(c, BFTKV_E_INVALID, "bad quorum handle");
  return 0;
}

}

extern "C" {

int bftkv_gpu_init(int device_ordinal, bftkv_gpu_ctx** out) {
  if (!out) return BFTKV_E_INVALID;
  int n = 0;
  if (hipGetDeviceCount(&n) != hipSuccess || n <= 0) return BFTKV_E_DEVICE;
  if (device_ordinal < 0 || device_ordinal >= n) return BFTKV_E_INVALID;
  if (hipSetDevice(device_ordinal) != hipSuccess) return BFTKV_E_DEVICE;
  bftkv_gpu_ctx* c = new bftkv_gpu_ctx();
  c->device = device_ordinal;
  if (hipHostMalloc((void**)&c->h_mail, 64, hipHostMallocMapped) == hipSuccess) {
    if (hipHostGetDevicePointer((void**)&c->d_mail, c->h_mail, 0) != hipSuccess) { (void)hipHostFree(c->h_mail); c->h_mail = nullptr; c->d_mail = nullptr; }
    else memset(c->h_mail, 0, 64);
  } else c->h_mail = nullptr;
  if (hipStreamCreateWithFlags(&c->stream, hipStreamNonBlocking) != hipSuccess ||
      hipStreamCreateWithFlags(&c->stream_h, hipStreamNonBlocking) != hipSuccess ||
      hipStreamCreateWithFlags(&c->stream_d, hipStreamNonBlocking) != hipSuccess) { delete c; return BFTKV_E_DEVICE; }
  { std::lock_guard<std::mutex> lk(g_live_mu); g_live.push_back(c); }
  if (const char* e = getenv("BFTKV_STAGED_SPIN_US")) c->staged_spin_us = (uint32_t)atoi(e);
  if (const char* e = getenv("BFTKV_MODEXP_LDS_PAD")) c->modexp_lds_pad = (uint32_t)atoi(e);
  if (const char* e = getenv("BFTKV_MULTIEXP_PARTS")) c->multiexp_parts = (uint32_t)atoi(e);
  if (const char* e = getenv("BFTKV_EC_SPLIT")) c->ec_split = (uint32_t)atoi(e);
  if (const char* e = getenv("BFTKV_EC_WINDOW")) c->ec_window = (uint32_t)atoi(e);
  if (const char* e = getenv("BFTKV_MULTIEXP_LANES")) c->multiexp_lanes = (uint32_t)atoi(e);
  if (const char* e = getenv("BFTKV_RSAV_LANES")) c->rsav_lanes = (uint32_t)atoi(e);
  if (const char* e = getenv("BFTKV_MULTIEXP_BLOCK")) c->multiexp_block = (uint32_t)atoi(e);
  if (const char* e = getenv("BFTKV_DSA_INV")) c->dsa_inv_mode = !strcmp(e, "batched") ? 2u : !strcmp(e, "single") ? 1u : 0u;
  { int cus = 0; if (hipDeviceGetAttribute(&cus, hipDeviceAttributeMultiprocessorCount, device_ordinal) == hipSuccess && cus > 0) c->n_cus = (uint32_t)cus; }
  *out = c;
  return BFTKV_OK;
}

int bftkv_gpu_ctx_fork(bftkv_gpu_ctx* root, bftkv_gpu_ctx** out) {
  if (!root || !out) return BFTKV_E_INVALID;
  if (root->root) return fail(root, BFTKV_E_INVALID, "fork of a fork");
  bftkv_gpu_ctx* c = nullptr;
  int rc = bftkv_gpu_init(root->device, &c);
  if (rc) return rc;
  c->root = root;
  c->early_exit = root->early_exit;
  c->dsa_inv_mode = root->dsa_inv_mode;
  root->n_forks.fetch_add(1);
  *out = c;
  return 0;
}

void bftkv_gpu_destroy(bftkv_gpu_ctx* c) {
  if (!c) return;
  for (bftkv_gpu_ctx* w : c->hb_workers) bftkv_gpu_destroy(w);
  c->hb_workers.clear();
  if (!c->root && c->n_forks.load() > 0) {
    fprintf(stderr, "bftkv_gpu_destroy: context still has %d forked context(s); not destroyed\n", c->n_forks.load());
    return;
  }
  {
    std::lock_guard<std::mutex> lk(g_live_mu);
    for (size_t i = 0; i < g_live.size(); ++i) if (g_live[i] == c) { g_live.erase(g_live.begin() + i); break; }
  }
  (void)hipSetDevice(c->device);
  (void)hipStreamSynchronize(c->stream);
  (void)hipStreamSynchronize(c->stream_h);
  (void)hipStreamSynchronize(c->stream_d);
  for (DevBuf* b : {&c->k_id, &c->k_entity, &c->k_algo, &c->k_flags, &c->k_bits, &c->k_e, &c->k_n, &c->k_r2, &c->k_n0, &c->k_q, &c->k_qbits, &c->k_dsatab, &c->k_dsaslot, &c->dsa_comb, &c->k_sorted_id, &c->k_sorted_slot, &c->k_r2w, &c->k_n29, &c->k_r2_29, &c->k_n0_29,
                    &c->chunk_arena, &c->chunk_ctr, &c->counts, &c->base, &c->total, &c->item_flags, &c->walk_scratch, &c->cert_ent, &c->sig_class, &c->mid, &c->mid64, &c->hash_mask, &c->recs, &c->digests, &c->r, &c->xr,
                    &c->pk_list, &c->pk_list3072, &c->pk_list4096, &c->r3072, &c->r4096, &c->pk_count, &c->dsa_list, &c->dsa_u, &c->dsa_idx, &c->ids_tmp, &c->o_err, &c->o_nver, &c->o_verdict, &c->o_fenced, &c->in_tbs, &c->in_tbs_off,
                    &c->in_ss, &c->in_ss_off, &c->in_prefix, &c->in_prefix_off, &c->in_shared, &c->in_shared_off, &c->in_seg, &c->st_tmp, &c->item_tmp, &c->bits_tmp, &c->plan_cut, &c->txt_mid32, &c->txt_mid64, &c->txt_tail, &c->txt_len})
    b->release();
  for (auto& q : c->quorums) { q.member.release(); q.ids.release(); }
  for (EcKeySet& ks : c->ec_keysets) ks.release();
  for (DsaKeySet& ks : c->dsa_keysets) ks.release();
  for (RsaKeySet& ks : c->rsa_keysets) ks.release();
  c->in_pack.release();
  c->forced_iss.release();
  release_small_pin(c);
  if (c->h_out) (void)hipHostFree(c->h_out);
  if (c->root) c->root->n_forks.fetch_sub(1);
  for (DevBuf* b : c->scratch_pool) { b->release(); delete b; }
  for (auto& kv : c->modtab_cache) for (DevBuf& b : kv.second) b.release();
  for (DevBuf& b : c->ec_fb_tab) b.release();
  if (c->h_mail) (void)hipHostFree(c->h_mail);
  if (c->hb_out) (void)hipHostFree(c->hb_out);
  if (c->hb_ring) { if (c->stream_c) (void)hipStreamSynchronize(c->stream_c); delete (HbRing*)c->hb_ring; }
  for (hipEvent_t e : c->hb_ev) (void)hipEventDestroy(e);
  if (c->hb_ev0) (void)hipEventDestroy(c->hb_ev0);
  if (c->seg_ev) (void)hipEventDestroy(c->seg_ev);
  if (c->stream_c) { (void)hipStreamSynchronize(c->stream_c); (void)hipStreamDestroy(c->stream_c); }
  if (c->stream_c2) { (void)hipStreamSynchronize(c->stream_c2); (void)hipStreamDestroy(c->stream_c2); }
  rccl_release(c);
  for (auto& e : c->ev) if (e) (void)hipEventDestroy(e);
  if (c->ev_turn) {
    Turnstile& g = g_turnstile[(unsigned)c->device & 15u];
    std::lock_guard<std::mutex> tl(g.mu);
    if (g.owner == c) { g.last = nullptr; g.owner = nullptr; }
    (void)hipEventDestroy(c->ev_turn);
  }
  (void)hipStreamDestroy(c->stream);
  (void)hipStreamDestroy(c->stream_h);
  (void)hipStreamDestroy(c->stream_d);
  delete c;
}

const char* bftkv_gpu_last_error(const bftkv_gpu_ctx* c) { return c ? c->err.c_str() : "null context"; }

const char* bftkv_gpu_error_string(int e) {
  switch (e) {
    case BFTKV_ERR_NONE: return "";
    case BFTKV_ERR_INVALID_SIGNATURE: return "crypto: invalid signature";
    case BFTKV_ERR_INSUFFICIENT_SIGNATURES: return "crypto: insufficient number of signatures";
    default: return "unknown";
  }
}

void* bftkv_gpu_stream(bftkv_gpu_ctx* c) { return c ? (void*)c->stream : nullptr; }

int bftkv_gpu_sync(bftkv_gpu_ctx* c) {
  if (!c) return BFTKV_E_INVALID;
  HIPCHK(c, hipStreamSynchronize(c->stream));
  return 0;
}

int bftkv_gpu_set_host_pipeline(bftkv_gpu_ctx* c, uint32_t pieces) {
  const uint32_t mode = (pieces >> 8) & 3u, tight = (pieces >> 10) & 1u;
  if (!c || (pieces & 0xFFu) > HB_PIPE_MAX_PIECES || mode > 2 || (pieces >> 11)) return BFTKV_E_INVALID;
  pieces &= 0xFFu;
  ctx_lock lk(c->mu);
  c->hb_pieces = pieces;
  c->hb_copy_mode = mode;
  c->hb_tight = tight != 0;
  return 0;
}

int bftkv_gpu_host_pipeline_trace(bftkv_gpu_ctx* c, float* out, uint32_t cap, uint32_t* n_out) {
  if (!c || !n_out) return BFTKV_E_INVALID;
  ctx_lock lk(c->mu);
  *n_out = (uint32_t)c->hb_trace.size();
  if (out) copy_out(out, c->hb_trace.data(), sizeof(float) * std::min<size_t>(cap, c->hb_trace.size()));
  return 0;
}

int bftkv_gpu_set_early_exit(bftkv_gpu_ctx* c, int on) {
  if (!c) return BFTKV_E_INVALID;
  ctx_lock lk(c->mu);
  if (c->root) return fail(c, BFTKV_E_STATE, "set on the root context; its forks follow");
  KtWrite kw(c);
  c->early_exit = on != 0;
  return 0;
}

int bftkv_gpu_set_hash_policy(bftkv_gpu_ctx* c, int hash_id, int state) {
  if (!c || (hash_id != HASH_MD5 && hash_id != HASH_RIPEMD160) || state < 0 || state > 2) return BFTKV_E_INVALID;
  ctx_lock lk(c->mu);
  if (c->root) return fail(c, BFTKV_E_STATE, "set on the root context; its forks follow");
  KtWrite kw(c);
  const int sh = hash_id == HASH_MD5 ? 0 : 2;
  c->kt.hash_policy = (c->kt.hash_policy & ~(3u << sh)) | ((uint32_t)state << sh);
  ++c->keyring_gen;
  return 0;
}

static bool dsa_width_ok(uint32_t bits) { return bits == 4 || (bits >= 8 && bits <= 20); }

int bftkv_gpu_set_dsa_window_bits(bftkv_gpu_ctx* c, uint32_t bits) {
  if (!c || (bits != 0 && !dsa_width_ok(bits))) return BFTKV_E_INVALID;
  ctx_lock lk(c->mu);
  c->dsa_wbits_pinned = bits;
  return 0;
}

int bftkv_gpu_set_dsa_table_budget(bftkv_gpu_ctx* c, uint64_t bytes) {
  if (!c) return BFTKV_E_INVALID;
  ctx_lock lk(c->mu);
  if (c->root) return fail(c, BFTKV_E_STATE, "a forked context cannot change the key table (use its root)");
  c->dsa_budget_bytes = (size_t)bytes;
  c->dsa_wbits_want = 0;
  return 0;
}

int bftkv_gpu_dsa_table_bytes(bftkv_gpu_ctx* c, uint64_t* bytes_out, uint32_t* entry_limbs_out) {
  if (!c) return BFTKV_E_INVALID;
  ctx_lock lk(c->mu);
  const bftkv_gpu_ctx* r = c->root ? c->root : c;
  if (bytes_out) *bytes_out = (uint64_t)r->dsa_comb.cap;
  if (entry_limbs_out) *entry_limbs_out = r->dsa_entry_limbs;
  return 0;
}

int bftkv_gpu_dsa_window_bits(bftkv_gpu_ctx* c, uint32_t* bits_out) {
  if (!c || !bits_out) return BFTKV_E_INVALID;
  ctx_lock lk(c->mu);
  const bftkv_gpu_ctx* r = c->root ? c->root : c;
  *bits_out = r->dsa_comb_slot.empty() ? 0u : r->dsa_wbits;
  return 0;
}

int bftkv_gpu_keyring_set(bftkv_gpu_ctx* c, const bftkv_gpu_pubkey* keys, uint32_t n_keys) {
  if (!c || (!keys && n_keys)) return BFTKV_E_INVALID;
  ctx_lock lk(c->mu);
  if (c->root) return fail(c, BFTKV_E_STATE, "a forked context cannot change the key table (use its root)");
  HIPCHK(c, hipSetDevice(c->device));
  std::vector<KeyEntry> ring;
  for (uint32_t i = 0; i < n_keys; ++i) {
    KeyEntry e;
    int rc = make_key_entry(c, keys[i], false, &e);
    if (rc) return rc;
    bool dup = false;
    for (auto& o : ring) {
      if (o.key_id == e.key_id) {
        if (o.material == e.material) { dup = true; break; }
        o.flags |= KEYF_AMBIGUOUS; e.flags |= KEYF_AMBIGUOUS;
      }
    }
    if (!dup) ring.push_back(std::move(e));
  }
  c->ring = std::move(ring);
  c->certs.clear();
  c->cert_valid.clear();
  ++c->cert_epoch;
  { std::unique_lock<std::shared_mutex> fl(c->cert_fast_mu); c->cert_fast.clear(); c->cert_fast_bytes = 0; }
  ++c->ring_epoch;
  return upload_key_table(c);
}

int bftkv_gpu_quorum_create(bftkv_gpu_ctx* c, const bftkv_gpu_qc* qcs, uint32_t n_qcs, int* out) {
  if (!c || !out || (!qcs && n_qcs)) return BFTKV_E_INVALID;
  if (n_qcs > MAX_QC) return fail(c, BFTKV_E_UNSUPPORTED, "more than MAX_QC cliques in one quorum");
  ctx_lock lk(c->mu);
  if (c->root) return fail(c, BFTKV_E_STATE, "quorums are created on the root context; its forks see them");
  HIPCHK(c, hipSetDevice(c->device));
  QuorumHost q;
  q.live = true;
  q.n_qcs = (int)n_qcs;
  std::vector<uint64_t> all;
  q.ids_off[0] = 0;
  for (uint32_t i = 0; i < n_qcs; ++i) {
    q.f[i] = qcs[i].f; q.mn[i] = qcs[i].min; q.thr[i] = qcs[i].threshold; q.suff[i] = qcs[i].suff;
    q.nodes.emplace_back(qcs[i].node_ids, qcs[i].node_ids + qcs[i].n_nodes);
    all.insert(all.end(), qcs[i].node_ids, qcs[i].node_ids + qcs[i].n_nodes);
    q.ids_off[i + 1] = (uint32_t)all.size();
  }
  std::vector<uint64_t> blob = all;
  size_t ids_words = blob.size();
  blob.resize(ids_words + (MAX_QC + 2) / 2 + 1, 0);
  memcpy(&blob[ids_words], q.ids_off, sizeof(uint32_t) * (n_qcs + 1));
  int rc = upload(c, q.ids, blob);
  if (rc) return rc;
  HIPCHK(c, hipStreamSynchronize(c->stream));
  q.ids_off[MAX_QC] = (uint32_t)ids_words;
  int h = -1;
  for (size_t i = 0; i < c->quorums.size(); ++i) if (!c->quorums[i].live) { h = (int)i; break; }
  KtWrite kw(c);
  if (h < 0) { c->quorums.emplace_back(); h = (int)c->quorums.size() - 1; }
  c->quorums[h] = std::move(q);
  ++c->quorum_gen;
  *out = h;
  return 0;
}

int bftkv_gpu_quorum_destroy(bftkv_gpu_ctx* c, int quorum) {
  if (!c) return BFTKV_E_INVALID;
  ctx_lock lk(c->mu);
  if (c->root) return fail(c, BFTKV_E_STATE, "quorums are destroyed on the root context");
  int rc = check_quorum(c, quorum);
  if (rc) return rc;
  KtWrite kw(c);
  c->quorums[quorum].member.release();
  c->quorums[quorum].ids.release();
  c->quorums[quorum] = QuorumHost();
  ++c->quorum_gen;
  return 0;
}

static int collective_verify_impl(bftkv_gpu_ctx* c, int quorum, uint32_t n_items, const uint8_t* tbs, const uint64_t* tbs_off,
                                  const uint8_t* ss, const uint64_t* ss_off, uint8_t* err_out, uint32_t* nver_out,
                                  uint8_t* verdict_out, uint8_t* fenced_out, const std::function<int(hipStream_t)>* upload_tbs, uint64_t ss_len,
                                  hipEvent_t ev_input = nullptr, uint32_t cap = 0, bool mid_prelaunched = false) {
  HIPCHK(c, hipSetDevice(c->device));
  int rc = check_quorum(c, quorum);
  if (rc) return rc;
  if (n_items == 0) return 0;
  QuorumHost& q = c->quorums[quorum];
  if ((rc = build_member(c, q))) return rc;
  const QuorumDev qd = quorum_dev(c, q);
  if ((rc = run_pipeline(c, n_items, tbs, tbs_off, ss, ss_off, nullptr, nullptr, nullptr, nullptr, upload_tbs, c->early_exit ? &qd : nullptr, ss_len, nullptr, nullptr, cap, ev_input, mid_prelaunched))) return rc;
  HIPCHK(c, c->o_nver.ensure(sizeof(uint32_t) * n_items));
  HIPCHK(c, c->o_verdict.ensure(n_items));
  uint32_t* nv = nver_out ? nver_out : c->o_nver.as<uint32_t>();
  uint8_t* vd = verdict_out ? verdict_out : c->o_verdict.as<uint8_t>();
  hipLaunchKernelGGL(k_tally, dim3((n_items + 3) / 4), dim3(256), 0, c->stream, c->recs.as<SigRec>(), c->base.as<uint32_t>(),
                     c->counts.as<uint32_t>(), n_items, c->kt, quorum_dev(c, q), vd, nv, (uint32_t*)nullptr);
  if (err_out) {
    hipLaunchKernelGGL(k_err_from_verdict, dim3((n_items + 255) / 256), dim3(256), 0, c->stream, vd, n_items, err_out);
  }
  if (fenced_out)
    hipLaunchKernelGGL(k_fenced_out, dim3((n_items + 255) / 256), dim3(256), 0, c->stream, c->item_flags.as<uint8_t>(),
                       c->hash_mask.as<uint32_t>(), n_items, fenced_out);
  HIPCHK(c, hipEventRecord(c->ev[4], c->stream));
  HIPCHK(c, hipGetLastError());
  c->have_timing = true;
  return 0;
}

int bftkv_gpu_collective_verify_dev(bftkv_gpu_ctx* c, int quorum, uint32_t n_items, const uint8_t* tbs, const uint64_t* tbs_off,
                                    const uint8_t* ss, const uint64_t* ss_off, uint64_t ss_len, uint8_t* err_out,
                                    uint32_t* nver_out, uint8_t* verdict_out, uint8_t* fenced_out) {
  if (!c) return BFTKV_E_INVALID;
  ctx_lock lk(c->mu);
  KtRead kr(c);
  if (kr.rc) return kr.rc;
  return collective_verify_impl(c, quorum, n_items, tbs, tbs_off, ss, ss_off, err_out, nver_out, verdict_out, fenced_out, nullptr, ss_len);
}


struct HbPiece { uint32_t i0, i1; };

struct HbSeg { const uint8_t* prefix; const uint64_t* prefix_off; const uint8_t* shared; const uint64_t* shared_off; uint32_t n_shared; const uint32_t* seg; };

struct HbCopy { uint32_t piece; int half; const uint8_t* src; uint8_t* dst; uint64_t len; };

static uint32_t hb_forced_pieces(const bftkv_gpu_ctx* c) {
  static const int env = getenv("BFTKV_HB_PIECES") ? atoi(getenv("BFTKV_HB_PIECES")) : 0;
  return c->hb_pieces ? c->hb_pieces : (uint32_t)std::max(env, 0);
}

static uint32_t hb_pieces_for(const bftkv_gpu_ctx* c, uint64_t bytes, uint32_t n_items) {
  const uint32_t forced = hb_forced_pieces(c);
  if (forced == 1) return 1;
  if (forced > 1) return std::max<uint32_t>(1, std::min<uint32_t>(std::min(forced, HB_PIPE_MAX_PIECES), n_items));
  if (bytes < HB_PIPE_MIN_BYTES || n_items < 64) return 1;
  const uint32_t p = (uint32_t)std::min<uint64_t>(HB_PIPE_MAX_PIECES, std::max<uint64_t>(2, bytes / (40ull << 20)));
  return std::min<uint32_t>(p, n_items / 16);
}

static int collective_verify_pipelined(bftkv_gpu_ctx* c, int quorum, uint32_t n_items, const uint8_t* tbs, const uint64_t* tbs_off,
                                       const uint8_t* ss, const uint64_t* ss_off, uint8_t* err_out, uint32_t* nver_out,
                                       uint8_t* verdict_out, uint8_t* fenced_out, uint32_t n_pieces, const HbSeg* sg = nullptr) {
  std::unique_lock<std::mutex> link_turn(g_hb_mu[(unsigned)c->device & 15u]);
  const auto t_call = std::chrono::steady_clock::now();
  auto us_now = [&] { return (float)std::chrono::duration_cast<std::chrono::nanoseconds>(std::chrono::steady_clock::now() - t_call).count() * 1e-3f; };
  bftkv_gpu_ctx* const root = c->root ? c->root : c;
  int rc = check_quorum(c, quorum);
  if (rc) return rc;
  const uint64_t tl = tbs_off[n_items], sl = ss_off[n_items];
  std::vector<HbPiece> pc;
  {
    const uint64_t* const poff = sg ? sg->prefix_off : tbs_off;
    const uint64_t total = poff[n_items] + sl;
    uint32_t i = 0;
    for (uint32_t k = 0; k < n_pieces && i < n_items; ++k) {
      const uint64_t want = total / n_pieces * (k + 1);
      uint32_t lo = i + 1, hi = n_items;
      while (lo < hi) { const uint32_t m = lo + (hi - lo) / 2; if (poff[m] + ss_off[m] < want) lo = m + 1; else hi = m; }
      const uint32_t j = (k + 1 == n_pieces) ? n_items : lo;
      pc.push_back({i, j});
      i = j;
    }
  }
  const uint32_t P = (uint32_t)pc.size();
  while (c->hb_workers.size() < P) {
    bftkv_gpu_ctx* w = nullptr;
    if ((rc = bftkv_gpu_init(c->device, &w))) return fail(c, rc, "host-buffer pipeline: worker context");
    w->root = root; w->dsa_inv_mode = root->dsa_inv_mode;
    if (const char* e = getenv("BFTKV_HB_MODEXP_LDS_PAD")) w->modexp_lds_pad = (uint32_t)atoi(e);
    root->n_forks.fetch_add(1);
    c->hb_workers.push_back(w);
  }
  if (!c->stream_c) {
    int lo_p = 0, hi_p = 0;
    (void)hipDeviceGetStreamPriorityRange(&lo_p, &hi_p);
    static const bool prio = !getenv("BFTKV_HB_COPY_NO_PRIORITY");
    if (!prio || hipStreamCreateWithPriority(&c->stream_c, hipStreamNonBlocking, hi_p) != hipSuccess) { c->stream_c = nullptr; HIPCHK(c, hipStreamCreateWithFlags(&c->stream_c, hipStreamNonBlocking)); }
    if (!prio || hipStreamCreateWithPriority(&c->stream_c2, hipStreamNonBlocking, hi_p) != hipSuccess) { c->stream_c2 = nullptr; HIPCHK(c, hipStreamCreateWithFlags(&c->stream_c2, hipStreamNonBlocking)); }
  }
// ... 433 lines not shown
    HIPCHK(c, hipMemcpyAsync(c->cert_ent.p, ent, sizeof(uint32_t) * n_items, hipMemcpyHostToDevice, c->stream));
    d_cert = c->cert_ent.as<uint32_t>();
  }
  const uint8_t* d_cls = nullptr;
  if (sig_class) {
    HIPCHK(c, c->sig_class.ensure(n_items + 16));
    HIPCHK(c, hipMemcpyAsync(c->sig_class.p, sig_class, n_items, hipMemcpyHostToDevice, c->stream));
    d_cls = c->sig_class.as<uint8_t>();
  }
  const uint64_t* d_forced = nullptr;
  if (forced_issuer && sig_class) {
    HIPCHK(c, c->forced_iss.ensure(sizeof(uint64_t) * n_items + 16));
    HIPCHK(c, hipMemcpyAsync(c->forced_iss.p, forced_issuer, sizeof(uint64_t) * n_items, hipMemcpyHostToDevice, c->stream));
    d_forced = c->forced_iss.as<uint64_t>();
  }
  int rc = run_pipeline(c, n_items, c->in_tbs.as<uint8_t>(), c->in_tbs_off.as<uint64_t>(), c->in_ss.as<uint8_t>(),
                        c->in_ss_off.as<uint64_t>(), d_cert, d_cls, nullptr, nullptr, nullptr, nullptr, sl, nullptr, nullptr, 0, nullptr, false, d_forced);
  if (rc) return rc;
  hipLaunchKernelGGL(k_sigverify_fold, dim3((n_items + 255) / 256), dim3(256), 0, c->stream, c->recs.as<SigRec>(),
                     c->base.as<uint32_t>(), c->counts.as<uint32_t>(), c->item_flags.as<uint8_t>(), n_items, c->o_err.as<uint8_t>());
  if (fenced_out) {
    HIPCHK(c, c->o_fenced.ensure(n_items));
    hipLaunchKernelGGL(k_fenced_out, dim3((n_items + 255) / 256), dim3(256), 0, c->stream, c->item_flags.as<uint8_t>(),
                       c->hash_mask.as<uint32_t>(), n_items, c->o_fenced.as<uint8_t>());
    HIPCHK(c, hipMemcpyAsync(fenced_out, c->o_fenced.p, n_items, hipMemcpyDeviceToHost, c->stream));
  }
  HIPCHK(c, hipEventRecord(c->ev[4], c->stream));
  HIPCHK(c, hipMemcpyAsync(err_out, c->o_err.p, n_items, hipMemcpyDeviceToHost, c->stream));
  HIPCHK(c, hipStreamSynchronize(c->stream));
  HIPCHK(c, hipGetLastError());
  c->have_timing = true;
  return 0;
}

int bftkv_gpu_signature_verify(bftkv_gpu_ctx* c, uint32_t n_items, const uint8_t* tbs, const uint64_t* tbs_off,
                               const uint8_t* sig, const uint64_t* sig_off, const uint64_t* cert_key_id, uint8_t* err_out,
                               uint8_t* fenced_out) {
  if (!c || (n_items && (!tbs_off || !sig_off || !err_out))) return BFTKV_E_INVALID;
  if (n_items == 0) return 0;
  std::vector<uint32_t> ce;
  ctx_lock lk(c->mu);
  KtRead kr(c);
  if (kr.rc) return kr.rc;
  if (cert_key_id) {
    ce.resize(n_items);
    for (uint32_t i = 0; i < n_items; ++i) {
      uint32_t e = 0xFFFFFFFEu;
      for (uint32_t k = 0; k < c->n_entities; ++k) if (c->h_entity_id[k] == cert_key_id[i]) { e = k; break; }
      ce[i] = e;
    }
  }
  int rc = signature_verify_entities(c, n_items, tbs, tbs_off, sig, sig_off, cert_key_id ? ce.data() : nullptr, err_out, nullptr, fenced_out);
  if (!rc && fenced_out && cert_key_id)
    for (uint32_t i = 0; i < n_items; ++i) if (ce[i] == 0xFFFFFFFEu) fenced_out[i] = 1;
  return rc;
}

int bftkv_gpu_last_statuses(bftkv_gpu_ctx* c, uint8_t* st, uint32_t* item, uint32_t cap, uint32_t* n_out) {
  if (!c || !n_out) return BFTKV_E_INVALID;
  ctx_lock lk(c->mu);
  HIPCHK(c, hipSetDevice(c->device));
  if (c->last_total_on_dev && !c->hb_last_pieces) {
    HIPCHK(c, hipMemcpy(&c->last_total, c->total.p, sizeof(uint32_t), hipMemcpyDeviceToHost));
    c->last_total_on_dev = false;
  }
  *n_out = c->last_total;
  if (c->hb_last_pieces) {
    uint32_t done = 0;
    for (uint32_t k = 0; k < c->hb_last_pieces && st && done < cap; ++k) {
      uint32_t nk = 0;
      const int rc = bftkv_gpu_last_statuses(c->hb_workers[k], st + done, item ? item + done : nullptr, cap - done, &nk);
      if (rc) return fail(c, rc, c->hb_workers[k]->err.c_str());
      nk = std::min(nk, cap - done);
      if (item) for (uint32_t j = 0; j < nk; ++j) item[done + j] += c->hb_item0[k];
      done += nk;
    }
    return 0;
  }
  uint32_t n = c->last_total < cap ? c->last_total : cap;
  if (!n || !st) return 0;
  HIPCHK(c, c->st_tmp.ensure(n));
  HIPCHK(c, c->item_tmp.ensure(sizeof(uint32_t) * n));
  hipLaunchKernelGGL(k_export_status, dim3((n + 255) / 256), dim3(256), 0, c->stream, c->recs.as<SigRec>(), n,
                     c->st_tmp.as<uint8_t>(), c->item_tmp.as<uint32_t>());
  HIPCHK(c, hipMemcpyAsync(st, c->st_tmp.p, n, hipMemcpyDeviceToHost, c->stream));
  if (item) HIPCHK(c, hipMemcpyAsync(item, c->item_tmp.p, sizeof(uint32_t) * n, hipMemcpyDeviceToHost, c->stream));
  HIPCHK(c, hipStreamSynchronize(c->stream));
  return 0;
}

int bftkv_gpu_last_counters(bftkv_gpu_ctx* c, uint64_t counters[4]) {
  if (!c || !counters) return BFTKV_E_INVALID;
  ctx_lock lk(c->mu);
  HIPCHK(c, hipSetDevice(c->device));
  uint32_t cnt[4] = {0, 0, 0, 0};
  if (c->hb_last_pieces) {
    for (uint32_t k = 0; k < c->hb_last_pieces; ++k) {
      uint32_t ck[4] = {0, 0, 0, 0};
      if (c->hb_workers[k]->pk_count.p) HIPCHK(c, hipMemcpy(ck, c->hb_workers[k]->pk_count.p, 16, hipMemcpyDeviceToHost));
      for (int j = 0; j < 4; ++j) cnt[j] += ck[j];
    }
  } else
  if (c->pk_count.p) HIPCHK(c, hipMemcpy(cnt, c->pk_count.p, 16, hipMemcpyDeviceToHost));
  counters[0] = c->last_total;
  counters[1] = (uint64_t)cnt[0] + cnt[1] + cnt[2] + cnt[3];
  counters[2] = c->last_items;
  counters[3] = cnt[1];
  return 0;
}

int bftkv_gpu_last_sclk_mhz(bftkv_gpu_ctx* c, float* mhz) {
  if (!c || !mhz) return BFTKV_E_INVALID;
  ctx_lock lk(c->mu);
  HIPCHK(c, hipSetDevice(c->device));
  uint64_t v[2] = {0, 0};
  if (c->pk_count.p) HIPCHK(c, hipMemcpy(v, (const char*)c->pk_count.p + 64, 16, hipMemcpyDeviceToHost));
  *mhz = v[1] ? (float)((double)v[0] / (double)v[1] * 100.0) : 0.0f;
  return 0;
}

int bftkv_gpu_last_timing(bftkv_gpu_ctx* c, float ms[8]) {
  if (!c || !ms) return BFTKV_E_INVALID;
  ctx_lock lk(c->mu);
  if (!c->have_timing) return fail(c, BFTKV_E_STATE, "no timed call yet");
  HIPCHK(c, hipSetDevice(c->device));
  HIPCHK(c, hipEventSynchronize(c->ev[4]));
  for (int i = 0; i < 8; ++i) ms[i] = 0;
  HIPCHK(c, hipEventElapsedTime(&ms[0], c->ev[0], c->ev[4]));
  HIPCHK(c, hipEventElapsedTime(&ms[1], c->ev[0], c->ev[1]));
  HIPCHK(c, hipEventElapsedTime(&ms[2], c->ev[5], c->ev[6]));
  HIPCHK(c, hipEventElapsedTime(&ms[3], c->ev[9], c->ev[2]));
  HIPCHK(c, hipEventElapsedTime(&ms[4], c->ev[3], c->ev[4]));
  HIPCHK(c, hipEventElapsedTime(&ms[5], c->ev[2], c->ev[8]));
  HIPCHK(c, hipEventElapsedTime(&ms[6], c->ev[8], c->ev[3]));
  return 0;
}

int bftkv_gpu_quorum_tally(bftkv_gpu_ctx* c, int quorum, uint32_t n_lists, const uint64_t* ids, const uint64_t* list_off,
                           uint8_t* verdict_out) {
  if (!c || (n_lists && (!list_off || !verdict_out))) return BFTKV_E_INVALID;
  if (n_lists == 0) return 0;
  ctx_lock lk(c->mu);
  if (c->root) return fail(c, BFTKV_E_STATE, "bftkv_gpu_quorum_tally runs on the root context");
  HIPCHK(c, hipSetDevice(c->device));
  int rc = check_quorum(c, quorum);
  if (rc) return rc;
  QuorumHost& q = c->quorums[quorum];
  if ((rc = check_offsets(c, list_off, n_lists, "list_off not monotone from 0"))) return rc;
  const uint64_t n_ids = list_off[n_lists];
  HIPCHK(c, c->in_ss.ensure(sizeof(uint64_t) * (n_ids + 1)));
  HIPCHK(c, c->in_ss_off.ensure(sizeof(uint64_t) * (n_lists + 1)));
  HIPCHK(c, c->o_verdict.ensure(n_lists));
  if (n_ids) HIPCHK(c, hipMemcpyAsync(c->in_ss.p, ids, sizeof(uint64_t) * n_ids, hipMemcpyHostToDevice, c->stream));
  HIPCHK(c, hipMemcpyAsync(c->in_ss_off.p, list_off, sizeof(uint64_t) * (n_lists + 1), hipMemcpyHostToDevice, c->stream));
  QuorumDev qd = quorum_dev(c, q);
  const uint64_t* d_ids = q.ids.as<uint64_t>();
  const uint32_t* d_off = (const uint32_t*)(d_ids + q.ids_off[MAX_QC]);
  hipLaunchKernelGGL(k_tally_ids, dim3((n_lists + 3) / 4), dim3(256), 0, c->stream, c->in_ss.as<uint64_t>(),
                     c->in_ss_off.as<uint64_t>(), n_lists, d_ids, d_off, qd, c->o_verdict.as<uint8_t>());
  HIPCHK(c, hipMemcpyAsync(verdict_out, c->o_verdict.p, n_lists, hipMemcpyDeviceToHost, c->stream));
  HIPCHK(c, hipStreamSynchronize(c->stream));
  HIPCHK(c, hipGetLastError());
  return 0;
}

int bftkv_gpu_signers(bftkv_gpu_ctx* c, uint32_t n_items, const uint8_t* ss, const uint64_t* ss_off, uint64_t* ids_out,
                      uint64_t* ids_off_out, uint64_t cap) {
  return bftkv_gpu_signers_fenced(c, n_items, ss, ss_off, ids_out, ids_off_out, cap, nullptr);
}

int bftkv_gpu_signers_fenced(bftkv_gpu_ctx* c, uint32_t n_items, const uint8_t* ss, const uint64_t* ss_off, uint64_t* ids_out,
                             uint64_t* ids_off_out, uint64_t cap, uint8_t* fenced_out) {
  if (!c || (n_items && (!ss_off || !ids_off_out))) return BFTKV_E_INVALID;
  ctx_lock lk(c->mu);
  KtRead kr(c);
  if (kr.rc) return kr.rc;
  HIPCHK(c, hipSetDevice(c->device));
  ids_off_out[0] = 0;
  if (n_items == 0) return 0;
  hipStream_t s = c->stream;
  { int rco = check_offsets(c, ss_off, n_items, "ss_off not monotone from 0"); if (rco) return rco; }
  const uint64_t sl = ss_off[n_items];
  HIPCHK(c, c->in_ss.ensure(sl + 64));
  HIPCHK(c, c->in_ss_off.ensure(sizeof(uint64_t) * (n_items + 1)));
  if (sl) HIPCHK(c, hipMemcpyAsync(c->in_ss.p, ss, sl, hipMemcpyHostToDevice, s));
  HIPCHK(c, hipMemcpyAsync(c->in_ss_off.p, ss_off, sizeof(uint64_t) * (n_items + 1), hipMemcpyHostToDevice, s));
  HIPCHK(c, c->counts.ensure(sizeof(uint32_t) * (n_items + 1)));
  HIPCHK(c, c->base.ensure(sizeof(uint32_t) * (n_items + 1)));
  HIPCHK(c, c->total.ensure(16));
  const uint32_t nb = (n_items + 63) / 64;
  if (fenced_out) HIPCHK(c, c->o_fenced.ensure(n_items));
// ... 41 lines not shown
```

### bftkv_amd/csrc/kernels.hip

```cpp
#include <hip/hip_runtime.h>
#include <stdint.h>

#include "device_types.h"
#include "mont28.h"
#include "value_load.h"
#include "u256.h"
#include "hashes.h"

namespace bftkv {

struct ParsedPacket {
  uint64_t next;
  bool event;
  SigRec rec;
};

__host__ __device__ __forceinline__ bool known_tag(uint32_t tag) {
  return tag < 32 && ((0x00066BFEu >> tag) & 1u);
}

struct SubpacketState {
  bool have_ctime = false, have_issuer = false, have_embedded = false;
  bool too_deep = false;
  uint64_t issuer = 0;
// ... 1037 lines not shown
  if ((uint8_t)(tag_hi >> 24) != rec.hash_tag[0] || (uint8_t)(tag_hi >> 16) != rec.hash_tag[1]) st = ST_HASH_TAG;
  else st = (rec.after_tag == AFTER_TAG_PUBKEY) ? (uint8_t)ST_PENDING_RSA : rec.after_tag;
  recs[ri].status = st;
}

__global__ void __launch_bounds__(256) k_digest_sha256(const uint8_t* __restrict__ tbs_blob, const uint64_t* __restrict__ tbs_off,
                                                       const uint8_t* __restrict__ sig_blob, const uint32_t* __restrict__ mid32,
                                                       const uint64_t* __restrict__ mid64, uint32_t n_items, SigRec* __restrict__ recs,
                                                       uint32_t n_recs, uint32_t* __restrict__ digests,
                                                       const uint64_t* __restrict__ tbs_prefix, const uint32_t* __restrict__ n_recs_dev) {
  digest_body<false>(tbs_blob, tbs_off, sig_blob, mid32, mid64, n_items, recs, n_recs_dev ? *n_recs_dev : n_recs, digests,
                     blockIdx.x * blockDim.x + threadIdx.x, tbs_prefix);
}
__global__ void __launch_bounds__(256) k_digest_other(const uint8_t* __restrict__ tbs_blob, const uint64_t* __restrict__ tbs_off,
                                                         const uint8_t* __restrict__ sig_blob, const uint32_t* __restrict__ mid32,
                                                         const uint64_t* __restrict__ mid64, uint32_t n_items, SigRec* __restrict__ recs,
                                                         uint32_t n_recs, uint32_t* __restrict__ digests,
                                                         const uint32_t* __restrict__ any_other , TextDev txt,
                                                         const uint32_t* __restrict__ n_recs_dev ) {
  if (*any_other == 0) return;
  if (n_recs_dev) n_recs = *n_recs_dev;
  for (uint64_t ri = (uint64_t)blockIdx.x * blockDim.x + threadIdx.x; ri < n_recs; ri += (uint64_t)gridDim.x * blockDim.x)
    digest_body<true>(tbs_blob, tbs_off, sig_blob, mid32, mid64, n_items, recs, n_recs, digests, (uint32_t)ri, nullptr, 1, nullptr, txt);
}

__global__ void __launch_bounds__(64) k_candidates(const uint8_t* __restrict__ tbs_blob, const uint64_t* __restrict__ tbs_off,
                                                   const uint8_t* __restrict__ sig_blob, const uint32_t* __restrict__ mid32,
                                                   const uint64_t* __restrict__ mid64, uint32_t n_items, SigRec* __restrict__ recs,
                                                   uint32_t n_recs, const uint32_t* __restrict__ n_recs_dev, const uint64_t* __restrict__ tbs_prefix,
                                                   KeyTableDev kt, const uint32_t* __restrict__ cert_ent, const uint8_t* __restrict__ sig_class,
                                                   TextDev txt, uint32_t* __restrict__ item_hash_mask) {
  const uint32_t ri = blockIdx.x * blockDim.x + threadIdx.x;
  const uint32_t nr = n_recs_dev ? *n_recs_dev : n_recs;
  if (ri >= nr) return;
  const SigRec rec = recs[ri];
  if (!(rec.flags & SIGF_MORE_CANDIDATES)) return;
  uint8_t st = rec.status;
  if (!(st == ST_KEY_CANNOT_SIGN || st == ST_HASH_TAG || st == ST_ALGO_MISMATCH || st == ST_BAD_SIG)) return;
  if (tbs_prefix && (rec.hash_id != HASH_SHA256 || (rec.flags & SIGF_TEXT))) return;
  const uint32_t slot = (uint32_t)rec.key_slot;
  const uint64_t issuer = kt.key_id[slot];
  const uint32_t only_ent = cert_ent ? cert_ent[rec.item] : 0xFFFFFFFFu;
  const uint32_t cls = sig_class ? sig_class[rec.item] : 0;
  uint32_t lo_i = 0, hi_i = kt.n_keys;
  while (lo_i < hi_i) {
    const uint32_t mid = (lo_i + hi_i) >> 1;
    if (kt.sorted_id[mid] < issuer) lo_i = mid + 1; else hi_i = mid;
  }
  bool behind = false;
  uint32_t writes = (kt.flags[slot] & KEYF_CAN_SIGN) ? 1u : 0u;
  for (uint32_t i = lo_i; i < kt.n_keys && kt.sorted_id[i] == issuer; ++i) {
    const uint32_t k = kt.sorted_slot[i];
    if (!key_is_candidate(kt, k, only_ent, cls)) continue;
    if (k == slot) { behind = true; continue; }
    if (!behind) continue;
    if (!(kt.flags[k] & KEYF_CAN_SIGN)) { st = ST_KEY_CANNOT_SIGN; continue; }
    ++writes;
    uint32_t tag = 0;
    if (rec.hash_id == HASH_SHA256 && !(rec.flags & SIGF_TEXT))
      digest_body<false>(tbs_blob, tbs_off, sig_blob, mid32, mid64, n_items, recs, nr, nullptr, ri, tbs_prefix, writes, &tag);
    else digest_body<true>(tbs_blob, tbs_off, sig_blob, mid32, mid64, n_items, recs, nr, nullptr, ri, tbs_prefix, writes, &tag, txt);
    if ((uint8_t)(tag >> 8) != rec.hash_tag[0] || (uint8_t)tag != rec.hash_tag[1]) st = ST_HASH_TAG;
    else if (kt.pk_algo[k] != rec.pk_algo) st = ST_ALGO_MISMATCH;
    else {
      st = ST_BAD_SIG;
      atomicOr(&item_hash_mask[rec.item], ITEM_FENCED);
    }
  }
  recs[ri].status = st;
}

constexpr int RSA_BLOCK = 256;
constexpr int QUADS_PER_BLOCK = RSA_BLOCK / MONT_TPI;
#ifndef BFTKV_MODEXP_BLOCK
#define BFTKV_MODEXP_BLOCK 256
#endif
constexpr int MODEXP_BLOCK = BFTKV_MODEXP_BLOCK;
#ifndef BFTKV_RSA_FORM
#define BFTKV_RSA_FORM 29
#endif
static_assert(BFTKV_RSA_FORM == 28 || BFTKV_RSA_FORM == 29, "BFTKV_RSA_FORM: 28 or 29");

enum : int { OP_TO_MONT = 0, OP_SQR = 1, OP_MULX = 2, OP_MULP = 3, OP_MUL1 = 4 };

constexpr int EM_LOW_BYTES = 84;
constexpr int EM_LOW_LIMBS = EM_LOW_BYTES * 8 / MONT_W;
static_assert(EM_LOW_LIMBS * MONT_W == EM_LOW_BYTES * 8, "the EM split must fall on a limb boundary");
constexpr uint32_t EM_HEAD_BAD = 0xFFFFFFFFu;

template <int W = MONT_W>
__device__ __forceinline__ uint32_t em_head_limb(uint32_t gi, uint32_t kbytes) {
  const int32_t top = 8 * ((int32_t)kbytes - 2), lo = (int32_t)gi * W;
  if (top < lo) return 0u;
  if (top >= lo + W - 1) return (1u << W) - 1u;
  return (1u << (top - lo + 1)) - 1u;
}

template <int L, int TPI, int W = MONT_W, bool WIDE_ONLY = false>
__global__ void __launch_bounds__(MODEXP_BLOCK, 3) k_rsa_modexp(const uint8_t* __restrict__ sig_blob, const SigRec* __restrict__ recs,
                                                          const uint32_t* __restrict__ pk_list, const uint32_t* __restrict__ pk_count_ptr,
                                                          const uint32_t* __restrict__ pk_start_ptr,
                                                          KeyTableDev kt, uint32_t* __restrict__ r_low,
                                                          uint32_t* __restrict__ xr_scratch, uint64_t* __restrict__ clk,
                                                          const uint32_t* __restrict__ wide_word = nullptr) {
  static_assert(W == MONT_W || (W == 29 && L == 18 && TPI == 4 && !WIDE_ONLY), "the only form at another radix is 18 x 4 at 2^29");
  constexpr int NL = TPI * L;
  constexpr int GROUPS = MODEXP_BLOCK / TPI;
  const bool stamp = clk && blockIdx.x == 0 && threadIdx.x == 0;
  uint64_t t0 = 0, r0 = 0;
  if (stamp) { t0 = __builtin_readcyclecounter(); r0 = __builtin_amdgcn_s_memrealtime(); }
  __shared__ uint32_t a_sh[GROUPS * NL];
  __shared__ uint32_t x_sh[GROUPS * NL];
  const uint32_t count = *pk_count_ptr, start = *pk_start_ptr;
  if (start + blockIdx.x * GROUPS >= count) return;
  if constexpr (WIDE_ONLY) { if (*wide_word == 0u) return; }
  const uint32_t quad = threadIdx.x / TPI;
  const int qlane = threadIdx.x % TPI;
  const uint32_t gq = start + blockIdx.x * GROUPS + quad;
  bool active = gq < count;
  if constexpr (W != MONT_W || WIDE_ONLY) {
    const bool wide = active && (recs[pk_list[gq]].flags & SIGF_WIDE_VALUE) != 0;
    active = active && (wide == WIDE_ONLY);
    if (WIDE_ONLY && !__any(active)) return;
  }
  const uint32_t pi = active ? gq : (count - 1);
  const uint32_t ri = pk_list[pi];
  const SigRec rec = recs[ri];
  const uint32_t key = (uint32_t)rec.key_slot;
  uint32_t* a_lds = a_sh + quad * NL + qlane * L;
  const uint32_t* a_rd = a_sh + quad * NL;
  uint32_t* x_lds = x_sh + quad * NL + qlane * L;

  uint32_t n[L], b[L], y[L];
  const uint32_t* np = W == 29 ? kt.n_limbs29 + (uint64_t)key * NL + qlane * L : kt.n_limbs + (uint64_t)key * MONT_NMAX + qlane * L;
  const uint32_t* rp = W == 29                 ? kt.r2_limbs29 + (uint64_t)key * NL + qlane * L
                       : (L == 10 && TPI == 8) ? kt.r2_limbs80 + (uint64_t)key * 80 + qlane * L
                                               : kt.r2_limbs + (uint64_t)key * MONT_NMAX + qlane * L;
  uint32_t* xrp = xr_scratch + (uint64_t)pi * NL + qlane * L;
#pragma unroll
  for (int k = 0; k < L; ++k) n[k] = np[k];
  {
    const uint32_t nb = (rec.mpi_bits[0] + 7u) >> 3;
    const uint8_t* mp = sig_blob + rec.body_off + rec.mpi_off[0];
    if constexpr (VALUE_LOAD_DWORDS) {
      uint32_t x[L];
      value_limbs<W, L, TPI>(x, nb, qlane,
                             [&](uint32_t o) -> uint32_t { uint32_t v; __builtin_memcpy(&v, mp + o, 4); return v; },
                             [&](uint32_t o) -> uint32_t { return mp[o]; });
#pragma unroll
      for (int k = 0; k < L; ++k) x_lds[k] = x[k];
    } else {
      auto sig_b = [&](uint32_t i) -> uint32_t { return i < nb ? mp[nb - 1 - i] : 0u; };
#pragma unroll
      for (int k = 0; k < L; ++k) x_lds[k] = limb_of<W>(sig_b, qlane * L + k);
    }
  }
  const uint32_t n0inv = W == 29 ? kt.n0inv29[key] : kt.n0inv[key];
  const uint32_t e = kt.rsa_e[key];
  const uint32_t kbytes = (kt.mod_bits[key] + 7) >> 3;
  const uint32_t cls = (e << 1) | (((e & 1u) && e > 1u && !(rec.flags & 1u)) ? 1u : 0u);

  uint64_t todo = __builtin_amdgcn_ballot_w64(true);
  while (todo) {
    const int lead = __builtin_ctzll(todo);
    const uint32_t cls_u = (uint32_t)__builtin_amdgcn_readlane((int)cls, lead);
    const bool live = (cls == cls_u);
    const uint32_t e_u = cls_u >> 1;
    const bool sc_u = cls_u & 1u;
    const int top = 31 - __builtin_clz(e_u | 1u);
    int kind = OP_TO_MONT, bitpos = top;
    while (true) {
      if (kind == OP_TO_MONT) {
#pragma unroll
        for (int k = 0; k < L; ++k) { b[k] = rp[k]; a_lds[k] = x_lds[k]; }
      } else {
#pragma unroll
        for (int k = 0; k < L; ++k) b[k] = y[k];
        if (kind == OP_SQR) {
#pragma unroll
          for (int k = 0; k < L; ++k) a_lds[k] = y[k];
        } else if (kind == OP_MULX) {
#pragma unroll
          for (int k = 0; k < L; ++k) a_lds[k] = xrp[k];
        } else if (kind == OP_MULP) {
#pragma unroll
          for (int k = 0; k < L; ++k) a_lds[k] = x_lds[k];
        } else {
#pragma unroll
          for (int k = 0; k < L; ++k) a_lds[k] = (qlane == 0 && k == 0) ? 1u : 0u;
        }
      }
      __builtin_amdgcn_fence(__ATOMIC_ACQ_REL, "wavefront");
      if (kind == OP_SQR) mont_mul<L, TPI, true, W>(y, a_rd, b, n, n0inv, qlane);
      else mont_mul<L, TPI, false, W>(y, a_rd, b, n, n0inv, qlane);
      __builtin_amdgcn_fence(__ATOMIC_ACQ_REL, "wavefront");
      if (kind == OP_TO_MONT && (e_u & (e_u - 1u)) != 0 && !(sc_u && __builtin_popcount(e_u) == 2)) {
#pragma unroll
// ... 583 lines not shown
  const uint32_t mi = mod_idx[op];
  uint32_t* a_lds = a_sh + quad * MONT_N + qlane * L;
  uint32_t* x_lds = x_sh + quad * MONT_N + qlane * L;
  const uint32_t* a_rd = a_sh + quad * MONT_N;
  const uint32_t* x_rd = x_sh + quad * MONT_N;
  uint32_t n[L], b[L], y[L], t[L];
#pragma unroll
  for (int k = 0; k < L; ++k) n[k] = n_limbs[(uint64_t)mi * MONT_N + qlane * L + k];
  const uint32_t n0inv = n0inv_tab[mi];
  const uint32_t* ew = exp_words + (uint64_t)(exp_per_op ? op : mi) * exp_nwords;
  const int nbits = (int)exp_nwords * 32;
  for (int step = -2; step <= 2 * nbits; ++step) {
    const uint32_t* ard = a_rd;
    if (step == -2) {
#pragma unroll
      for (int k = 0; k < L; ++k) { b[k] = r2_limbs[(uint64_t)mi * MONT_N + qlane * L + k]; a_lds[k] = base_limbs[(uint64_t)op * MONT_N + qlane * L + k]; }
    } else if (step == -1 || step == 2 * nbits) {
#pragma unroll
      for (int k = 0; k < L; ++k) a_lds[k] = (qlane == 0 && k == 0) ? 1u : 0u;
      if (step >= 0) {
#pragma unroll
        for (int k = 0; k < L; ++k) b[k] = y[k];
      }
    } else if ((step & 1) == 0) {
#pragma unroll
      for (int k = 0; k < L; ++k) { a_lds[k] = y[k]; b[k] = y[k]; }
    } else {
#pragma unroll
      for (int k = 0; k < L; ++k) b[k] = y[k];
      ard = x_rd;
    }
    __builtin_amdgcn_fence(__ATOMIC_ACQ_REL, "wavefront");
    if (step >= 0 && step < 2 * nbits && (step & 1) == 0) mont_mul<L, MONT_TPI, true>(t, ard, b, n, n0inv, qlane);
    else mont_mul(t, ard, b, n, n0inv, qlane);
    __builtin_amdgcn_fence(__ATOMIC_ACQ_REL, "wavefront");
    if (step == -2) {
#pragma unroll
      for (int k = 0; k < L; ++k) x_lds[k] = t[k];
    } else if (step >= 0 && step < 2 * nbits && (step & 1)) {
      const int bi = nbits - 1 - (step >> 1);
      const bool bit = (ew[bi >> 5] >> (bi & 31)) & 1u;
      if (bit) {
#pragma unroll
        for (int k = 0; k < L; ++k) y[k] = t[k];
      }
    } else {
#pragma unroll
      for (int k = 0; k < L; ++k) y[k] = t[k];
    }
  }
  canonicalize(y, qlane);
  uint32_t diff = 0;
#pragma unroll
  for (int k = 0; k < L; ++k) diff |= y[k] ^ n[k];
  diff = quad_or(diff);
  if (active) {
#pragma unroll
    for (int k = 0; k < L; ++k) out_limbs[(uint64_t)op * MONT_N + qlane * L + k] = (diff == 0) ? 0u : y[k];
  }
}

__global__ void k_bytes_to_limbs(const uint8_t* __restrict__ src, uint32_t nbytes, uint32_t n_nums, uint32_t* __restrict__ dst) {
  uint32_t i = blockIdx.x * blockDim.x + threadIdx.x;
  if (i >= n_nums * MONT_N) return;
  uint32_t num = i / MONT_N, j = i % MONT_N;
  const uint8_t* p = src + (uint64_t)num * nbytes;
  auto bf = [&](uint32_t k) -> uint32_t { return k < nbytes ? p[nbytes - 1 - k] : 0u; };
  dst[i] = limb_of(bf, (int)j);
}
__global__ void k_limbs_to_bytes(const uint32_t* __restrict__ src, uint32_t nbytes, uint32_t n_nums, uint8_t* __restrict__ dst) {
  uint32_t i = blockIdx.x * blockDim.x + threadIdx.x;
  if (i >= n_nums * nbytes) return;
  uint32_t num = i / nbytes, k = i % nbytes;
  uint32_t bit = k * 8, j = bit / 28, sh = bit % 28;
  const uint32_t* l = src + (uint64_t)num * MONT_N;
  uint64_t v = (j < MONT_N ? l[j] : 0u);
  if (j + 1 < MONT_N) v |= (uint64_t)l[j + 1] << 28;
  dst[(uint64_t)num * nbytes + (nbytes - 1 - k)] = (uint8_t)(v >> sh);
}

__global__ void __launch_bounds__(256) k_tally(const SigRec* __restrict__ recs, const uint32_t* __restrict__ rec_base,
                                               const uint32_t* __restrict__ counts, uint32_t n_items, KeyTableDev kt,
                                               QuorumDev q, uint8_t* __restrict__ verdict, uint32_t* __restrict__ n_verified,
                                               uint32_t* __restrict__ clique_counts ) {
  const uint32_t wave = (blockIdx.x * blockDim.x + threadIdx.x) >> 6;
  const uint32_t lane = threadIdx.x & 63;
  if (wave >= n_items) return;
  const uint32_t base = rec_base[wave], cnt = counts[wave];
  uint32_t cq[MAX_QC];
#pragma unroll
  for (int c = 0; c < MAX_QC; ++c) cq[c] = 0;
  uint32_t total_ok = 0;
  uint32_t first_suff = 0xFFFFFFFFu;
  for (uint32_t off = 0; off < cnt; off += 64) {
    const uint32_t i = off + lane;
    bool ok = false;
    uint32_t ent = 0;
    if (i < cnt) {
      const SigRec r = recs[base + i];
      ok = (r.status == ST_OK);
      if (ok) ent = kt.entity[r.key_slot];
    }
    const uint64_t okm = __builtin_amdgcn_ballot_w64(ok);
    const uint64_t below = (lane == 0) ? 0ull : (~0ull >> (64 - lane));
    bool reached = false;
#pragma unroll
    for (int c = 0; c < MAX_QC; ++c) {
      if (c < q.n_qcs) {
        const bool mem = ok && q.member[(uint64_t)c * q.n_entities + ent];
        const uint64_t mm = __builtin_amdgcn_ballot_w64(mem);
        const uint32_t run = cq[c] + (uint32_t)__builtin_popcountll(mm & below) + (mem ? 1u : 0u);
        if (ok && q.suff[c] > 0 && run >= (uint32_t)q.suff[c]) reached = true;
        cq[c] += (uint32_t)__builtin_popcountll(mm);
      }
    }
    const uint64_t rm = __builtin_amdgcn_ballot_w64(reached);
    if (rm != 0 && first_suff == 0xFFFFFFFFu) {
      const uint32_t fl = (uint32_t)__builtin_ctzll(rm);
      first_suff = total_ok + (uint32_t)__builtin_popcountll(okm & ((fl == 63) ? ~0ull : ((1ull << (fl + 1)) - 1)));
    }
    total_ok += (uint32_t)__builtin_popcountll(okm);
  }
  if (lane == 0) {
    bool is_quorum = q.n_qcs > 0, is_thr = q.n_qcs > 0, is_suff = false, reject = true;
    for (int c = 0; c < q.n_qcs; ++c) {
      if (q.f[c] > 0 && (int32_t)cq[c] < q.min[c]) is_quorum = false;
      if (q.threshold[c] > 0 && (int32_t)cq[c] < q.threshold[c]) is_thr = false;
      if (q.suff[c] > 0 && (int32_t)cq[c] >= q.suff[c]) is_suff = true;
      if (q.f[c] == 0 || (int32_t)cq[c] <= q.f[c]) reject = false;
    }
    verdict[wave] = (is_quorum ? V_IS_QUORUM : 0) | (is_thr ? V_IS_THRESHOLD : 0) | (is_suff ? V_IS_SUFFICIENT : 0) |
                    (reject ? V_REJECT : 0);
    n_verified[wave] = is_suff ? first_suff : total_ok;
    if (clique_counts)
      for (int c = 0; c < MAX_QC; ++c) clique_counts[(uint64_t)wave * MAX_QC + c] = cq[c];
  }
}

struct PlanArgs {
  SigRec* recs; const uint32_t* rec_base; const uint32_t* counts; uint32_t n_items;
  uint32_t *pk_list, *dsa_list, *pk_list3072, *pk_list4096;
  uint32_t* pk_count;
  uint32_t* plan_cut;
  const uint8_t* verdict;
  uint32_t margin;
  uint32_t* mail;
};

constexpr int PLAN_BLOCK = 1024, PLAN_ITEMS = PLAN_BLOCK / 64;
template <int PHASE>
__global__ void __launch_bounds__(PLAN_BLOCK) k_plan(PlanArgs a, KeyTableDev kt, QuorumDev q) {
  __shared__ uint32_t cnt_sh[PLAN_ITEMS][4];
  const uint32_t wib = threadIdx.x >> 6, lane = threadIdx.x & 63;
  const uint32_t item = blockIdx.x * PLAN_ITEMS + wib;
  if (PHASE == 1 && a.mail && blockIdx.x == 0 && threadIdx.x == 0)
    __hip_atomic_store(a.mail, 0x80000000u | (a.pk_count[4] ? 1u : 0u), __ATOMIC_RELEASE, __HIP_MEMORY_SCOPE_SYSTEM);
  const bool have = item < a.n_items;
  const uint32_t base = have ? a.rec_base[item] : 0, cnt = have ? a.counts[item] : 0;
  uint32_t* const lists[4] = {a.pk_list, a.dsa_list, a.pk_list3072, a.pk_list4096};
  const uint64_t below = (lane == 0) ? 0ull : (~0ull >> (64 - lane));
  uint32_t from = 0, covered = cnt;
  if (PHASE == 1) {
    uint32_t cq[MAX_QC];
#pragma unroll
    for (int c = 0; c < MAX_QC; ++c) cq[c] = 0;
    bool done = false;
    for (uint32_t off = 0; off < cnt && !done; off += 64) {
      const uint32_t i = off + lane;
      uint32_t kind = 0, ent = 0;
      if (i < cnt) {
        kind = a.recs[base + i].q_kind1;
        if (kind) ent = kt.entity[a.recs[base + i].key_slot];
      }
      bool reached = false;
#pragma unroll
      for (int c = 0; c < MAX_QC; ++c) {
        if (c < q.n_qcs) {
          const bool mem = kind != 0 && q.member[(uint64_t)c * q.n_entities + ent];
          const uint64_t mm = __builtin_amdgcn_ballot_w64(mem);
          const uint32_t run = cq[c] + (uint32_t)__builtin_popcountll(mm & below) + (mem ? 1u : 0u);
          if (mem && q.suff[c] > 0 && run >= (uint32_t)q.suff[c] + a.margin) reached = true;
          cq[c] += (uint32_t)__builtin_popcountll(mm);
        }
      }
      const uint64_t rm = __builtin_amdgcn_ballot_w64(reached);
      if (rm) { done = true; covered = off + (uint32_t)__builtin_ctzll(rm) + 1; }
    }
  } else {
    from = have ? a.plan_cut[item] : 0;
    if (!have || (a.verdict[item] & V_IS_SUFFICIENT)) from = covered;
  }
  auto wants = [&](uint32_t i, uint32_t& kind) -> bool {
    kind = 0;
    if (i >= covered) return false;
    if (PHASE == 1) { kind = a.recs[base + i].q_kind1; return kind != 0; }
    const SigRec r = a.recs[base + i];
    kind = r.q_kind1;
    return kind != 0 && !r.queued && r.status == ST_PENDING_RSA;
  };
  uint32_t n_k[4] = {0, 0, 0, 0};
  for (uint32_t off = from; off < covered; off += 64) {
    uint32_t kind;
    const bool w = wants(off + lane, kind);
#pragma unroll
    for (int k = 0; k < 4; ++k) n_k[k] += (uint32_t)__builtin_popcountll(__builtin_amdgcn_ballot_w64(w && kind == (uint32_t)k + 1));
  }
  if (lane == 0) {
#pragma unroll
    for (int k = 0; k < 4; ++k) cnt_sh[wib][k] = n_k[k];
  }
  __syncthreads();
  if (threadIdx.x < 4) {
    uint32_t tot = 0;
    for (int w = 0; w < PLAN_ITEMS; ++w) { const uint32_t v = cnt_sh[w][threadIdx.x]; cnt_sh[w][threadIdx.x] = tot; tot += v; }
    const uint32_t b0 = tot ? atomicAdd(a.pk_count + threadIdx.x, tot) : 0u;
    for (int w = 0; w < PLAN_ITEMS; ++w) cnt_sh[w][threadIdx.x] += b0;
  }
  __syncthreads();
  uint32_t run_k[4];
#pragma unroll
  for (int k = 0; k < 4; ++k) run_k[k] = cnt_sh[wib][k];
  for (uint32_t off = from; off < covered; off += 64) {
    const uint32_t i = off + lane;
    uint32_t kind;
    const bool w = wants(i, kind);
#pragma unroll
    for (int k = 0; k < 4; ++k) {
      const bool mine = w && kind == (uint32_t)k + 1;
      const uint64_t m = __builtin_amdgcn_ballot_w64(mine);
      if (mine) {
        const uint32_t idx = run_k[k] + (uint32_t)__builtin_popcountll(m & below);
        a.recs[base + i].pk_idx = idx; a.recs[base + i].queued = 1; lists[k][idx] = base + i;
      }
      run_k[k] += (uint32_t)__builtin_popcountll(m);
    }
  }
  if (have && lane == 0) a.plan_cut[item] = (PHASE == 1) ? covered : cnt;
}

__global__ void k_plan_snapshot(uint32_t* __restrict__ pk_count) {
  if (threadIdx.x < 4) pk_count[8 + threadIdx.x] = pk_count[threadIdx.x];
}

__global__ void k_fenced_out(const uint8_t* __restrict__ item_flags, const uint32_t* __restrict__ item_hash_mask, uint32_t n,
                             uint8_t* __restrict__ out, uint32_t rehash_bits = 0) {
  uint32_t i = blockIdx.x * blockDim.x + threadIdx.x;
  if (i < n) out[i] = (((item_flags[i] & 4) || (item_hash_mask[i] & ITEM_FENCED)) ? 1 : 0) | ((item_hash_mask[i] & rehash_bits) ? 2 : 0);
}

__device__ __forceinline__ void wave_copy_bytes(uint8_t* __restrict__ dst, const uint8_t* __restrict__ src, uint64_t len, uint32_t lane) {
  if (len == 0) return;
  const uint64_t head = ((4u - ((uintptr_t)dst & 3u)) & 3u) < len ? ((4u - ((uintptr_t)dst & 3u)) & 3u) : len;
  if (lane < head) dst[lane] = src[lane];
  const uint64_t body = (len - head) & ~(uint64_t)3;
  uint32_t* __restrict__ d4 = (uint32_t*)(dst + head);
  const uint8_t* sp = src + head;
  const uint32_t mis = (uint32_t)((uintptr_t)sp & 3u);
  const uint32_t* __restrict__ s4 = (const uint32_t*)(sp - mis);
  for (uint64_t w = lane; w < body / 4; w += 64) {
    const uint32_t lo = s4[w], hi = mis ? s4[w + 1] : 0u;
    d4[w] = mis ? __builtin_amdgcn_alignbyte(hi, lo, mis) : lo;
  }
  const uint64_t done = head + body;
  if (lane < len - done) dst[done + lane] = src[done + lane];
}
__global__ void __launch_bounds__(256) k_expand_segments(const uint8_t* __restrict__ prefix, const uint64_t* __restrict__ prefix_off,
                                                         const uint8_t* __restrict__ shared, const uint64_t* __restrict__ shared_off,
                                                         const uint32_t* __restrict__ seg, const uint64_t* __restrict__ tbs_off,
                                                         uint32_t i0, uint32_t n, uint8_t* __restrict__ out) {
  const uint32_t item = i0 + blockIdx.x * (blockDim.x / 64) + threadIdx.x / 64, lane = threadIdx.x & 63u;
  if (item >= i0 + n) return;
  const uint64_t p0 = prefix_off[item], pl = prefix_off[item + 1] - p0;
  uint8_t* dst = out + tbs_off[item];
  wave_copy_bytes(dst, prefix + p0, pl, lane);
  const uint32_t sg = seg[item];
  if (sg != 0xFFFFFFFFu) wave_copy_bytes(dst + pl, shared + shared_off[sg], shared_off[sg + 1] - shared_off[sg], lane);
}

__global__ void k_err_from_verdict(const uint8_t* __restrict__ v, uint32_t n, uint8_t* __restrict__ e) {
  uint32_t i = blockIdx.x * blockDim.x + threadIdx.x;
  if (i < n) e[i] = (v[i] & V_IS_SUFFICIENT) ? 0 : 2;
}

__global__ void __launch_bounds__(256) k_finish_staged(const uint8_t* __restrict__ verdict_or_err, uint32_t from_verdict,
                                                       const uint8_t* __restrict__ item_flags, const uint32_t* __restrict__ item_hash_mask,
                                                       uint32_t n, uint32_t rehash_bits, uint8_t* __restrict__ host_out ,
                                                       uint32_t* __restrict__ host_flag, uint32_t seq,
                                                       const uint32_t* __restrict__ total ) {
  if (threadIdx.x < 8) host_out[2 * (size_t)n + threadIdx.x] = (uint8_t)(total[threadIdx.x >> 2] >> (8 * (threadIdx.x & 3)));
  for (uint32_t i = threadIdx.x; i < n; i += blockDim.x) {
    const uint8_t v = verdict_or_err[i];
    host_out[i] = from_verdict ? ((v & V_IS_SUFFICIENT) ? 0 : 2) : v;
    host_out[n + i] = (((item_flags[i] & 4) || (item_hash_mask[i] & ITEM_FENCED)) ? 1 : 0) | ((item_hash_mask[i] & rehash_bits) ? 2 : 0);
  }
  __threadfence_system();
  __syncthreads();
  if (threadIdx.x == 0) __hip_atomic_store(host_flag, seq, __ATOMIC_RELEASE, __HIP_MEMORY_SCOPE_SYSTEM);
}

__global__ void k_export_status(const SigRec* __restrict__ recs, uint32_t n, uint8_t* __restrict__ st, uint32_t* __restrict__ item) {
  uint32_t i = blockIdx.x * blockDim.x + threadIdx.x;
  if (i >= n) return;
  const uint8_t v = recs[i].status;
  st[i] = v >= ST_PENDING_PARSE ? (uint8_t)ST_NOT_EXAMINED : v;
  if (item) item[i] = recs[i].item;
}

}
```

### include/bftkv_gpu.h

```cpp
#ifndef BFTKV_GPU_H
#define BFTKV_GPU_H

#include <stddef.h>
#include <stdint.h>

#ifdef __cplusplus
extern "C" {
#endif

typedef struct bftkv_gpu_ctx bftkv_gpu_ctx;

#define BFTKV_OK 0
#define BFTKV_E_INVALID (-1)
#define BFTKV_E_DEVICE (-2)
#define BFTKV_E_NOMEM (-3)
#define BFTKV_E_UNSUPPORTED (-4)
#define BFTKV_E_STATE (-5)

#define BFTKV_ST_OK 0
#define BFTKV_ST_UNKNOWN_ISSUER 1
#define BFTKV_ST_PARSE_ERROR 2
#define BFTKV_ST_NOT_SIGNATURE 3
#define BFTKV_ST_NO_ISSUER 4
#define BFTKV_ST_HASH_UNSUPPORTED 5
#define BFTKV_ST_HASH_TAG 6
#define BFTKV_ST_ALGO_MISMATCH 7
#define BFTKV_ST_BAD_SIG 8
#define BFTKV_ST_KEY_CANNOT_SIGN 9
#define BFTKV_ST_UNSUPPORTED 10
#define BFTKV_ST_NOT_EXAMINED 11

#define BFTKV_ERR_NONE 0
#define BFTKV_ERR_INVALID_SIGNATURE 1
#define BFTKV_ERR_INSUFFICIENT_SIGNATURES 2
#define BFTKV_ERR_CERTIFICATE_NOT_FOUND 3

#define BFTKV_V_IS_QUORUM 1
#define BFTKV_V_IS_THRESHOLD 2
#define BFTKV_V_IS_SUFFICIENT 4
#define BFTKV_V_REJECT 8

int bftkv_gpu_init(int device_ordinal, bftkv_gpu_ctx** out);
void bftkv_gpu_destroy(bftkv_gpu_ctx* ctx);
const char* bftkv_gpu_last_error(const bftkv_gpu_ctx* ctx);
const char* bftkv_gpu_error_string(int bftkv_err);

typedef struct {
  uint64_t key_id;
  uint64_t entity_id;
  uint8_t pk_algo;
  uint8_t usable_sign;
  uint8_t reserved[6];
  const uint8_t* n; uint32_t n_len;
  const uint8_t* e; uint32_t e_len;
  const uint8_t* g; uint32_t g_len;
  const uint8_t* y; uint32_t y_len;
} bftkv_gpu_pubkey;

int bftkv_gpu_keyring_set(bftkv_gpu_ctx* ctx, const bftkv_gpu_pubkey* keys, uint32_t n_keys);

int bftkv_gpu_set_hash_policy(bftkv_gpu_ctx* ctx, int hash_id, int state);

int bftkv_gpu_set_dsa_window_bits(bftkv_gpu_ctx* ctx, uint32_t bits);
int bftkv_gpu_dsa_window_bits(bftkv_gpu_ctx* ctx, uint32_t* bits_out);
int bftkv_gpu_set_dsa_table_budget(bftkv_gpu_ctx* ctx, uint64_t bytes);
int bftkv_gpu_dsa_table_bytes(bftkv_gpu_ctx* ctx, uint64_t* bytes_out, uint32_t* entry_limbs_out);

#define BFTKV_MSG_OK 0
#define BFTKV_MSG_SIGNATURE_ERROR 1
#define BFTKV_MSG_READ_ERROR 2
#define BFTKV_MSG_NOT_SIGNED 3
#define BFTKV_MSG_UNVERIFIED 4
#define BFTKV_MSG_UNSUPPORTED 5
int bftkv_gpu_message_verify(bftkv_gpu_ctx* ctx, uint32_t n_msgs, const uint8_t* msgs, const uint64_t* msg_off, uint8_t* status_out,
                             uint64_t* signer_key_id_out, uint64_t* peer_id_out, uint8_t* plain_out, uint64_t plain_cap,
                             uint64_t* plain_off_out, uint8_t* fname_out, uint8_t* fname_len_out);

typedef struct {
  int32_t f, min, threshold, suff;
  const uint64_t* node_ids; uint32_t n_nodes;
} bftkv_gpu_qc;
int bftkv_gpu_quorum_create(bftkv_gpu_ctx* ctx, const bftkv_gpu_qc* qcs, uint32_t n_qcs, int* quorum_out);
int bftkv_gpu_quorum_destroy(bftkv_gpu_ctx* ctx, int quorum);


int bftkv_gpu_collective_verify(bftkv_gpu_ctx* ctx, int quorum, uint32_t n_items,
                                const uint8_t* tbs_blob, const uint64_t* tbs_off,
                                const uint8_t* ss_blob, const uint64_t* ss_off,
                                uint8_t* err_out, uint32_t* n_verified_out, uint8_t* verdict_out, uint8_t* fenced_out);
int bftkv_gpu_collective_verify_segments(bftkv_gpu_ctx* ctx, int quorum, uint32_t n_items,
                                         const uint8_t* prefix_blob, const uint64_t* prefix_off,
                                         const uint8_t* shared_blob, const uint64_t* shared_off, uint32_t n_shared,
                                         const uint32_t* seg_of_item,
                                         const uint8_t* ss_blob, const uint64_t* ss_off,
                                         uint8_t* err_out, uint32_t* n_verified_out, uint8_t* verdict_out, uint8_t* fenced_out);
int bftkv_gpu_collective_verify_dev(bftkv_gpu_ctx* ctx, int quorum, uint32_t n_items,
                                    const uint8_t* tbs_blob, const uint64_t* tbs_off,
                                    const uint8_t* ss_blob, const uint64_t* ss_off, uint64_t ss_blob_len,
                                    uint8_t* err_out, uint32_t* n_verified_out, uint8_t* verdict_out, uint8_t* fenced_out);
int bftkv_gpu_sync(bftkv_gpu_ctx* ctx);
int bftkv_gpu_set_host_pipeline(bftkv_gpu_ctx* ctx, uint32_t pieces);
#define BFTKV_HOST_PIPELINE_RING 0x100u
#define BFTKV_HOST_PIPELINE_DIRECT 0x200u
#define BFTKV_HOST_PIPELINE_TIGHT_BOUND 0x400u
int bftkv_gpu_host_pipeline_trace(bftkv_gpu_ctx* ctx, float* out, uint32_t cap, uint32_t* n_out);
int bftkv_gpu_set_early_exit(bftkv_gpu_ctx* ctx, int on);

int bftkv_gpu_signature_verify(bftkv_gpu_ctx* ctx, uint32_t n_items,
                               const uint8_t* tbs_blob, const uint64_t* tbs_off,
                               const uint8_t* sig_blob, const uint64_t* sig_off,
                               const uint64_t* cert_key_id, uint8_t* err_out, uint8_t* fenced_out);

int bftkv_gpu_ctx_fork(bftkv_gpu_ctx* root, bftkv_gpu_ctx** fork_out);

int bftkv_gpu_collective_verify_small(bftkv_gpu_ctx* ctx, int quorum, uint32_t n_items, const uint8_t* tbs_blob, const uint64_t* tbs_off,
                                      const uint8_t* ss_blob, const uint64_t* ss_off, uint8_t* err_out, uint8_t* fenced_out);
int bftkv_gpu_signature_verify_small(bftkv_gpu_ctx* ctx, uint32_t n_items, const uint8_t* tbs_blob, const uint64_t* tbs_off,
                                     const uint8_t* sig_blob, const uint64_t* sig_off, const uint64_t* cert_key_id, uint8_t* err_out,
                                     uint8_t* fenced_out);

typedef struct bftkv_gpu_batcher bftkv_gpu_batcher;
bftkv_gpu_batcher* bftkv_gpu_batcher_create(bftkv_gpu_ctx* ctx, uint32_t max_items, uint32_t max_wait_us);
bftkv_gpu_batcher* bftkv_gpu_batcher_create_lanes(bftkv_gpu_ctx* ctx, uint32_t max_items, uint32_t max_wait_us, uint32_t n_lanes);
void bftkv_gpu_batcher_destroy(bftkv_gpu_batcher* b);
int bftkv_gpu_batcher_collective_verify(bftkv_gpu_batcher* b, int quorum, const uint8_t* tbs, uint64_t tbs_len,
                                        const uint8_t* ss, uint64_t ss_len, uint8_t* err_out, uint8_t* fenced_out);
int bftkv_gpu_batcher_signature_verify(bftkv_gpu_batcher* b, const uint8_t* tbs, uint64_t tbs_len, const uint8_t* sig,
                                       uint64_t sig_len, const uint64_t* cert_key_id, uint8_t* err_out, uint8_t* fenced_out);
int bftkv_gpu_batcher_cert_verify(bftkv_gpu_batcher* b, const uint8_t* cert, uint64_t cert_len, const uint8_t* tbs, uint64_t tbs_len,
                                  const uint8_t* sig, uint64_t sig_len, uint8_t* err_out, uint8_t* fenced_out,
                                  uint64_t* issuer_id_out, uint8_t* fingerprint_out);
#define BFTKV_ROLE_IGNORED 0u
#define BFTKV_ROLE_PRIMARY_KEY 1u
#define BFTKV_ROLE_USER_ID 2u
#define BFTKV_ROLE_SELF_SIGNATURE 3u
#define BFTKV_ROLE_IDENTITY_SIGNATURE 4u
#define BFTKV_ROLE_SUBKEY 5u
#define BFTKV_ROLE_SUBKEY_SIGNATURE 6u
#define BFTKV_ROLE_REVOCATION 7u
int bftkv_gpu_batcher_cert_entity(bftkv_gpu_batcher* b, const uint8_t* cert, uint64_t cert_len, uint8_t* err_out, uint8_t* fenced_out,
                                  uint64_t* issuer_id_out, uint8_t* fingerprint_out, uint64_t* entity_off_out, uint64_t* entity_len_out,
                                  uint32_t* roles_out, uint32_t roles_cap, uint32_t* n_roles_out);
int bftkv_gpu_batcher_message_verify(bftkv_gpu_batcher* b, const uint8_t* msg, uint64_t msg_len, uint8_t* status_out,
                                     uint64_t* signer_key_id_out, uint64_t* peer_id_out, uint8_t* plain_out, uint64_t plain_cap,
                                     uint64_t* plain_len_out, uint8_t* fname_out, uint8_t* fname_len_out);
#define BFTKV_TH_OK 0
#define BFTKV_TH_NO_INVERSE 1
#define BFTKV_TH_FENCED 2
#define BFTKV_TH_FAILED 0xFF
int bftkv_gpu_batcher_modmul_product(bftkv_gpu_batcher* b, uint32_t k, const uint8_t* factors, uint32_t nbytes, const uint8_t* mod,
                                     uint8_t* out, uint8_t* status_out);
int bftkv_gpu_batcher_lagrange_combine(bftkv_gpu_batcher* b, uint32_t k, const int32_t* xs, const uint8_t* ys, uint32_t nbytes,
                                       const uint8_t* mod, uint8_t* out, uint8_t* status_out);
int bftkv_gpu_batcher_dsa_calculate_r(bftkv_gpu_batcher* b, uint32_t k, const int32_t* xs, const uint8_t* ri, uint32_t pbytes,
                                      const uint8_t* vi, uint32_t qbytes, const uint8_t* p, const uint8_t* q, uint8_t* r_out,
                                      uint8_t* status_out);
int bftkv_gpu_batcher_modexp(bftkv_gpu_batcher* b, const uint8_t* base, uint32_t nbytes, const uint8_t* exp, uint32_t exp_len,
                             const uint8_t* mod, uint8_t* out, uint8_t* status_out);
int bftkv_gpu_batcher_ecdsa_calculate_r(bftkv_gpu_batcher* b, uint32_t k, const int32_t* xs, const uint8_t* ri, const uint8_t* vi,
                                        const uint8_t* curve, uint32_t bit_size, uint8_t* r_out, uint8_t* status_out);
int bftkv_gpu_batcher_ecdsa_verify(bftkv_gpu_batcher* b, const uint8_t* digest, uint32_t dlen, const uint8_t* sig, const uint8_t* key,
                                   const uint8_t* curve, uint32_t bit_size, uint8_t* valid_out, uint8_t* status_out);
int bftkv_gpu_batcher_ecdsa_verify_keyset(bftkv_gpu_batcher* b, int keyset, uint32_t key, const uint8_t* digest, uint32_t dlen,
                                          const uint8_t* sig, uint8_t* valid_out, uint8_t* status_out);
int bftkv_gpu_batcher_dsa_verify(bftkv_gpu_batcher* b, const uint8_t* digest, uint32_t dlen, const uint8_t* sig, uint32_t qbytes,
                                 const uint8_t* y, uint32_t pbytes, const uint8_t* p, const uint8_t* q, const uint8_t* g, uint8_t* valid_out,
                                 uint8_t* status_out);
int bftkv_gpu_batcher_dsa_verify_keyset(bftkv_gpu_batcher* b, int keyset, uint32_t key, const uint8_t* digest, uint32_t dlen,
                                        const uint8_t* sig, uint8_t* valid_out, uint8_t* status_out);
int bftkv_gpu_batcher_rsa_verify(bftkv_gpu_batcher* b, const uint8_t* digest, uint32_t hash_id, uint32_t dlen, const uint8_t* sig,
                                 uint32_t nbytes, const uint8_t* n, uint32_t e, uint8_t* valid_out, uint8_t* status_out);
int bftkv_gpu_batcher_rsa_verify_keyset(bftkv_gpu_batcher* b, int keyset, uint32_t key, const uint8_t* digest, uint32_t hash_id, uint32_t dlen,
                                        const uint8_t* sig, uint8_t* valid_out, uint8_t* status_out);
int bftkv_gpu_batcher_stats(bftkv_gpu_batcher* b, uint64_t stats[4]);
int bftkv_gpu_batcher_times(bftkv_gpu_batcher* b, uint64_t ns[8]);

int bftkv_gpu_last_statuses(bftkv_gpu_ctx* ctx, uint8_t* status_out, uint32_t* item_out, uint32_t cap, uint32_t* n_out);
int bftkv_gpu_last_counters(bftkv_gpu_ctx* ctx, uint64_t counters[4]);

int bftkv_gpu_signers(bftkv_gpu_ctx* ctx, uint32_t n_items, const uint8_t* ss_blob, const uint64_t* ss_off,
                      uint64_t* ids_out, uint64_t* ids_off_out, uint64_t cap);
int bftkv_gpu_signers_fenced(bftkv_gpu_ctx* ctx, uint32_t n_items, const uint8_t* ss_blob, const uint64_t* ss_off,
                             uint64_t* ids_out, uint64_t* ids_off_out, uint64_t cap, uint8_t* fenced_out);

int bftkv_gpu_quorum_tally(bftkv_gpu_ctx* ctx, int quorum, uint32_t n_lists,
                           const uint64_t* ids, const uint64_t* list_off, uint8_t* verdict_out);

int bftkv_gpu_modexp(bftkv_gpu_ctx* ctx, uint32_t n_ops, const uint8_t* base, uint32_t nbytes,
                     const uint32_t* mod_idx, uint32_t n_mods, const uint8_t* mods,
                     const uint8_t* exps, uint32_t exp_len, uint8_t* out);

int bftkv_gpu_modexp_ops(bftkv_gpu_ctx* ctx, uint32_t n_ops, const uint8_t* base, uint32_t nbytes,
                         const uint32_t* mod_idx, uint32_t n_mods, const uint8_t* mods,
                         const uint8_t* exps, uint32_t exp_len, uint8_t* out);

int bftkv_gpu_comm_unique_id(uint8_t uid_out[128]);
int bftkv_gpu_comm_init(bftkv_gpu_ctx* ctx, int n_ranks, int rank, const uint8_t uid[128]);
int bftkv_gpu_comm_library(char* path_out, uint32_t cap, int* preloaded_out);
int bftkv_gpu_comm_selftest(bftkv_gpu_ctx* ctx, uint32_t nbytes, uint32_t* bad_rows_out);
int bftkv_gpu_allgather_verdicts(bftkv_gpu_ctx* ctx, const uint8_t* local_bits, uint64_t nbytes, uint8_t* all_bits_out);
int bftkv_gpu_allgather_errs_dev(bftkv_gpu_ctx* ctx, const uint8_t* err_dev, uint32_t n_items, uint32_t slots, uint8_t* all_bits_out);


int bftkv_gpu_modmul_product(bftkv_gpu_ctx* ctx, uint32_t n_ops, uint32_t k, const uint8_t* factors, uint32_t nbytes,
                             const uint32_t* mod_idx, uint32_t n_mods, const uint8_t* mods, uint8_t* out);
int bftkv_gpu_lagrange_combine(bftkv_gpu_ctx* ctx, uint32_t n_ops, uint32_t k, const int32_t* xs, const uint8_t* ys,
                               uint32_t nbytes, const uint32_t* mod_idx, uint32_t n_mods, const uint8_t* mods,
                               uint8_t* out, uint8_t* status_out);
int bftkv_gpu_dsa_calculate_r(bftkv_gpu_ctx* ctx, uint32_t n_ops, uint32_t k, const int32_t* xs, const uint8_t* ri, uint32_t pbytes,
                              const uint8_t* vi, uint32_t qbytes, const uint32_t* group_idx, uint32_t n_groups,
                              const uint8_t* p, const uint8_t* q, uint8_t* r_out, uint8_t* status_out);

int bftkv_gpu_sss_distribute(bftkv_gpu_ctx* ctx, uint32_t n_polys, uint32_t n_shares, uint32_t k, const uint8_t* coeffs, uint32_t nbytes,
                             const uint32_t* mod_idx, uint32_t n_mods, const uint8_t* mods, uint8_t* shares_out);
int bftkv_gpu_modinv(bftkv_gpu_ctx* ctx, uint32_t n_ops, const uint8_t* values, uint32_t nbytes, const uint32_t* mod_idx, uint32_t n_mods,
                     const uint8_t* mods, uint8_t* out, uint8_t* status_out);

int bftkv_gpu_selftest_reduce(bftkv_gpu_ctx* ctx, uint32_t n_ops, const uint8_t* values, uint32_t nbytes, const uint32_t* mod_idx,
                              uint32_t n_mods, const uint8_t* mods, uint32_t lanes, uint8_t* out);

int bftkv_gpu_set_lagrange_x_bound(bftkv_gpu_ctx* ctx, uint32_t bound);

int bftkv_gpu_modmul_product_dev(bftkv_gpu_ctx* ctx, uint32_t n_ops, uint32_t k, const uint8_t* factors, uint32_t nbytes,
                                 const uint32_t* mod_idx, uint32_t n_mods, const uint8_t* mods, uint8_t* out);
int bftkv_gpu_lagrange_combine_dev(bftkv_gpu_ctx* ctx, uint32_t n_ops, uint32_t k, const int32_t* xs, const uint8_t* ys,
                                   uint32_t nbytes, const uint32_t* mod_idx, uint32_t n_mods, const uint8_t* mods,
                                   uint8_t* out, uint8_t* status_out);
int bftkv_gpu_dsa_calculate_r_dev(bftkv_gpu_ctx* ctx, uint32_t n_ops, uint32_t k, const int32_t* xs, const uint8_t* ri, uint32_t pbytes,
                                  const uint8_t* vi, uint32_t qbytes, const uint32_t* group_idx, uint32_t n_groups,
                                  const uint8_t* p, const uint8_t* q, uint8_t* r_out, uint8_t* status_out);
int bftkv_gpu_sss_distribute_dev(bftkv_gpu_ctx* ctx, uint32_t n_polys, uint32_t n_shares, uint32_t k, const uint8_t* coeffs, uint32_t nbytes,
                                 const uint32_t* mod_idx, uint32_t n_mods, const uint8_t* mods, uint8_t* shares_out);
int bftkv_gpu_modinv_dev(bftkv_gpu_ctx* ctx, uint32_t n_ops, const uint8_t* values, uint32_t nbytes, const uint32_t* mod_idx, uint32_t n_mods,
                         const uint8_t* mods, uint8_t* out, uint8_t* status_out);

int bftkv_gpu_ecdsa_calculate_r(bftkv_gpu_ctx* ctx, uint32_t n_ops, uint32_t k, const int32_t* xs, const uint8_t* ri, const uint8_t* vi,
                                const uint8_t* curve, uint32_t bit_size, uint8_t* r_out, uint8_t* status_out);
int bftkv_gpu_ecdsa_calculate_r_dev(bftkv_gpu_ctx* ctx, uint32_t n_ops, uint32_t k, const int32_t* xs, const uint8_t* ri, const uint8_t* vi,
                                    const uint8_t* curve, uint32_t bit_size, uint8_t* r_out, uint8_t* status_out);
int bftkv_gpu_ec_scalar_base_mult(bftkv_gpu_ctx* ctx, uint32_t n_ops, const uint8_t* scalars, uint32_t sbytes, const uint8_t* curve,
                                  uint32_t bit_size, uint8_t* out, uint8_t* status_out);
int bftkv_gpu_ecdsa_verify(bftkv_gpu_ctx* ctx, uint32_t n_ops, const uint8_t* digests, uint32_t dlen, const uint8_t* sigs,
                           const uint32_t* key_idx, uint32_t n_keys, const uint8_t* keys, const uint8_t* curve, uint32_t bit_size,
                           uint8_t* valid_out, uint8_t* status_out);
int bftkv_gpu_ecdsa_verify_dev(bftkv_gpu_ctx* ctx, uint32_t n_ops, const uint8_t* digests, uint32_t dlen, const uint8_t* sigs,
                               const uint32_t* key_idx, uint32_t n_keys, const uint8_t* keys, const uint8_t* curve, uint32_t bit_size,
                               uint8_t* valid_out, uint8_t* status_out);

int bftkv_gpu_dsa_verify(bftkv_gpu_ctx* ctx, uint32_t n_ops, const uint8_t* digests, uint32_t dlen, const uint8_t* sigs, uint32_t qbytes,
                         const uint32_t* key_idx, uint32_t n_keys, const uint8_t* keys_y, const uint32_t* key_group, uint32_t pbytes,
                         uint32_t n_groups, const uint8_t* p, const uint8_t* q, const uint8_t* g, uint8_t* valid_out, uint8_t* status_out);
int bftkv_gpu_dsa_verify_dev(bftkv_gpu_ctx* ctx, uint32_t n_ops, const uint8_t* digests, uint32_t dlen, const uint8_t* sigs, uint32_t qbytes,
                             const uint32_t* key_idx, uint32_t n_keys, const uint8_t* keys_y, const uint32_t* key_group, uint32_t pbytes,
                             uint32_t n_groups, const uint8_t* p, const uint8_t* q, const uint8_t* g, uint8_t* valid_out, uint8_t* status_out);

int bftkv_gpu_ecdsa_keyset_create(bftkv_gpu_ctx* ctx, uint32_t n_keys, const uint8_t* keys, const uint8_t* curve, uint32_t bit_size,
                                  int* keyset_out);
int bftkv_gpu_ecdsa_keyset_destroy(bftkv_gpu_ctx* ctx, int keyset);
int bftkv_gpu_ecdsa_keyset_info(bftkv_gpu_ctx* ctx, int keyset, uint32_t* n_keys_out, uint32_t* n_refused_out, uint32_t* window_bits_out,
                                uint64_t* table_bytes_out);
int bftkv_gpu_ecdsa_verify_keyset(bftkv_gpu_ctx* ctx, int keyset, uint32_t n_ops, const uint8_t* digests, uint32_t dlen, const uint8_t* sigs,
// ... 41 lines not shown
```

Before: 166.4 million verifies/s.

## Drop plan margin for big batches and run small second pass on 8-lane modexp

After: 167.4 million verifies/s (median of 6 runs). No clear change (+0.6%).

```diff
diff --git a/bftkv_amd/_native.py b/bftkv_amd/_native.py
--- a/bftkv_amd/_native.py
+++ b/bftkv_amd/_native.py
@@ -51,6 +51,7 @@
     "bftkv_gpu_dsa_verify_keyset_dev", "bftkv_gpu_batcher_dsa_verify_keyset", "bftkv_gpu_selftest_dsa_keyset_table",
     "bftkv_gpu_rsa_verify", "bftkv_gpu_rsa_verify_dev", "bftkv_gpu_rsa_keyset_create", "bftkv_gpu_rsa_keyset_destroy", "bftkv_gpu_rsa_keyset_info",
     "bftkv_gpu_rsa_verify_keyset", "bftkv_gpu_rsa_verify_keyset_dev", "bftkv_gpu_batcher_rsa_verify", "bftkv_gpu_batcher_rsa_verify_keyset",
+    "bftkv_gpu_set_plan_margin", "bftkv_gpu_set_second_pass_limit", "bftkv_gpu_last_plan_counters",
 ]
 
 _lib = None
@@ -126,6 +127,9 @@
     lib.bftkv_gpu_allgather_verdicts.argtypes = [vp, u8p, C.c_uint64, u8p]
     lib.bftkv_gpu_stream.restype = vp
     lib.bftkv_gpu_set_early_exit.argtypes = [vp, C.c_int]
+    lib.bftkv_gpu_set_plan_margin.argtypes = [vp, C.c_int]
+    lib.bftkv_gpu_set_second_pass_limit.argtypes = [vp, C.c_uint32]
+    lib.bftkv_gpu_last_plan_counters.argtypes = [vp, C.POINTER(C.c_uint64)]
     lib.bftkv_gpu_set_host_pipeline.argtypes = [vp, u32]
     lib.bftkv_gpu_host_pipeline_trace.argtypes = [vp, C.POINTER(C.c_float), u32, C.POINTER(u32)]
     lib.bftkv_gpu_last_sclk_mhz.argtypes = [vp, C.POINTER(C.c_float)]
@@ -259,6 +263,12 @@
     def set_early_exit(self, on: bool) -> None:
         self._check(self.lib.bftkv_gpu_set_early_exit(self.h, 1 if on else 0), "set_early_exit")
 
+    def set_plan_margin(self, margin: int) -> None:
+        self._check(self.lib.bftkv_gpu_set_plan_margin(self.h, int(margin)), "set_plan_margin")
+
+    def set_second_pass_limit(self, limit: int) -> None:
+        self._check(self.lib.bftkv_gpu_set_second_pass_limit(self.h, int(limit)), "set_second_pass_limit")
+
     def set_host_pipeline(self, pieces: int, copy: str = "", tight: bool = False) -> None:
         mode = {"": 0, "ring": 0x100, "direct": 0x200}[copy]
         self._check(self.lib.bftkv_gpu_set_host_pipeline(self.h, pieces | mode | (0x400 if tight else 0)), "set_host_pipeline")
@@ -406,7 +416,10 @@
     def last_counters(self):
         c = (C.c_uint64 * 4)()
         self._check(self.lib.bftkv_gpu_last_counters(self.h, c), "last_counters")
-        return {"packets": c[0], "pubkey_ops": c[1], "items": c[2], "dsa_ops": c[3]}
+        p = (C.c_uint64 * 3)()
+        self._check(self.lib.bftkv_gpu_last_plan_counters(self.h, p), "last_plan_counters")
+        return {"packets": c[0], "pubkey_ops": c[1], "items": c[2], "dsa_ops": c[3], "phase1_ops": p[0], "phase2_ops": p[1],
+                "phase2_rsa2048_ops": p[2]}
 
     def last_sclk_mhz(self) -> float:
         v = C.c_float(0)
diff --git a/bftkv_amd/csrc/capi.hip b/bftkv_amd/csrc/capi.hip
--- a/bftkv_amd/csrc/capi.hip
+++ b/bftkv_amd/csrc/capi.hip
@@ -122,6 +122,8 @@
   DevBuf meta;
   void release() { n29.release(); r2_29.release(); n80.release(); r2_80.release(); meta.release(); }
 };
+
+constexpr uint32_t SECOND_PASS_8LANE_MAX = 8192;
 
 }
 
@@ -175,6 +177,8 @@
   DevBuf forced_iss;
   DevBuf counts, base, total, item_flags, walk_scratch, cert_ent, sig_class, mid, mid64, hash_mask, recs, digests, r, xr, pk_list, pk_list3072, pk_list4096, r3072, r4096, pk_count, dsa_list, dsa_u, ids_tmp;
   DevBuf o_err, o_nver, o_verdict, o_fenced;
+  DevBuf o_exit;
+  bool last_exit_valid = false;
   DevBuf in_tbs, in_tbs_off, in_ss, in_ss_off;
   hipEvent_t seg_ev = nullptr;
   DevBuf in_prefix, in_prefix_off, in_shared, in_shared_off, in_seg;
@@ -192,6 +196,9 @@
   uint32_t n_cus = 256;
   uint32_t lagrange_x_bound = 0;
   bool early_exit = true;
+  int plan_margin = -1;
+  uint32_t second_pass_limit = SECOND_PASS_8LANE_MAX;
+  bool last_planned = false;
   std::vector<DevBuf*> scratch_pool;
   std::unordered_map<std::string, std::vector<uint32_t>> modrow_cache;
   std::unordered_map<std::string, std::vector<uint32_t>> rsav_row_cache[2];
@@ -496,6 +503,9 @@
     else
       hipLaunchKernelGGL(k_parse_body, dim3((total + 255) / 256), dim3(256), 0, s, pa, c->kt);
   }
+  const bool big = staged_cap ? (ev_input != nullptr && ss_len / 320 >= TURNSTILE_MIN_PACKETS) : total >= TURNSTILE_MIN_PACKETS;
+  c->last_planned = total && plan_q;
+  c->last_exit_valid = false;
   uint32_t* const cnt_p = c->pk_count.as<uint32_t>();
   const uint32_t* const start0 = cnt_p + 12;
   PlanArgs pl{};
@@ -505,7 +515,7 @@
     pl.pk_list4096 = c->pk_list4096.as<uint32_t>(); pl.pk_count = cnt_p; pl.plan_cut = c->plan_cut.as<uint32_t>(); pl.verdict = nullptr;
     int min_suff = 0;
     for (int i = 0; i < plan_q->n_qcs; ++i) if (plan_q->suff[i] > 0 && (min_suff == 0 || plan_q->suff[i] < min_suff)) min_suff = plan_q->suff[i];
-    pl.margin = 1u + (uint32_t)min_suff / 64u;
+    pl.margin = c->plan_margin >= 0 ? (uint32_t)c->plan_margin : big ? 0u : 1u + (uint32_t)min_suff / 64u;
     pl.mail = c->d_mail ? c->d_mail + 3 : nullptr;
     if (c->h_mail) __atomic_store_n(&c->h_mail[3], 0u, __ATOMIC_RELEASE);
     hipLaunchKernelGGL(k_plan<1>, dim3((n_items + PLAN_ITEMS - 1) / PLAN_ITEMS), dim3(PLAN_BLOCK), 0, s, pl, c->kt, *plan_q);
@@ -547,20 +557,21 @@
   const dim3 qg((total + MODEXP_BLOCK / MONT_TPI - 1) / (MODEXP_BLOCK / MONT_TPI));
   const dim3 qg8((total + MODEXP_BLOCK / MONT_TPI_BIG - 1) / (MODEXP_BLOCK / MONT_TPI_BIG));
   static const bool wide8_off = getenv("BFTKV_NO_WIDE8") != nullptr;
-  const bool wide8 = staged_cap != 0 && ss_len / 256 <= 8192 && !wide8_off;
-  auto launch_modexp = [&](const uint32_t* start) {
-    if (wide8)
+  const bool wide8 = staged_cap != 0 && ss_len / 256 <= SECOND_PASS_8LANE_MAX && !wide8_off;
+  auto launch_modexp = [&](const uint32_t* start, bool second_pass) {
+    const uint32_t limit = second_pass && !wide8 ? c->second_pass_limit : MODEXP_NO_LIMIT;
+    if (wide8 || (limit != MODEXP_NO_LIMIT && limit != 0u))
       hipLaunchKernelGGL((k_rsa_modexp<10, MONT_TPI_BIG>), qg8, dim3(MODEXP_BLOCK), 0, s, d_ss, c->recs.as<SigRec>(), c->pk_list.as<uint32_t>(),
-                         cnt_p, start, c->kt, c->r.as<uint32_t>(), c->xr.as<uint32_t>(), (uint64_t*)(cnt_p + 16));
-    else {
+                         cnt_p, start, c->kt, c->r.as<uint32_t>(), c->xr.as<uint32_t>(), (uint64_t*)(cnt_p + 16), (const uint32_t*)nullptr, limit);
+    if (!wide8) {
 #if BFTKV_RSA_FORM == 29
       hipLaunchKernelGGL((k_rsa_modexp<RSA29_L, MONT_TPI, RSA29_W>), qg, dim3(MODEXP_BLOCK), c->modexp_lds_pad, s, d_ss, c->recs.as<SigRec>(), c->pk_list.as<uint32_t>(),
-                         cnt_p, start, c->kt, c->r.as<uint32_t>(), c->xr.as<uint32_t>(), (uint64_t*)(cnt_p + 16), (const uint32_t*)(cnt_p + 5));
+                         cnt_p, start, c->kt, c->r.as<uint32_t>(), c->xr.as<uint32_t>(), (uint64_t*)(cnt_p + 16), (const uint32_t*)(cnt_p + 5), limit);
       hipLaunchKernelGGL((k_rsa_modexp<MONT_L, MONT_TPI, MONT_W, true>), qg, dim3(MODEXP_BLOCK), c->modexp_lds_pad, s, d_ss, c->recs.as<SigRec>(), c->pk_list.as<uint32_t>(),
-                         cnt_p, start, c->kt, c->r.as<uint32_t>(), c->xr.as<uint32_t>(), (uint64_t*)nullptr, (const uint32_t*)(cnt_p + 5));
+                         cnt_p, start, c->kt, c->r.as<uint32_t>(), c->xr.as<uint32_t>(), (uint64_t*)nullptr, (const uint32_t*)(cnt_p + 5), limit);
 #else
       hipLaunchKernelGGL((k_rsa_modexp<MONT_L, MONT_TPI>), qg, dim3(MODEXP_BLOCK), c->modexp_lds_pad, s, d_ss, c->recs.as<SigRec>(), c->pk_list.as<uint32_t>(),
-                         cnt_p, start, c->kt, c->r.as<uint32_t>(), c->xr.as<uint32_t>(), (uint64_t*)(cnt_p + 16));
+                         cnt_p, start, c->kt, c->r.as<uint32_t>(), c->xr.as<uint32_t>(), (uint64_t*)(cnt_p + 16), (const uint32_t*)nullptr, limit);
 #endif
     }
     if (c->have_rsa3072)
@@ -571,19 +582,18 @@
                          cnt_p + 3, start + 3, c->kt, c->r4096.as<uint32_t>(), c->xr.as<uint32_t>(), (uint64_t*)nullptr);
   };
   static const bool turnstile_off = getenv("BFTKV_NO_TURNSTILE") != nullptr;
-  const bool big = staged_cap ? (ev_input != nullptr && ss_len / 320 >= TURNSTILE_MIN_PACKETS) : total >= TURNSTILE_MIN_PACKETS;
   if (big && !turnstile_off) {
     Turnstile& g = g_turnstile[(unsigned)c->device & 15u];
     std::lock_guard<std::mutex> tl(g.mu);
     if (g.last && g.owner != c) HIPCHK(c, hipStreamWaitEvent(s, g.last, 0));
     HIPCHK(c, rec(9, s));
-    launch_modexp(start0);
+    launch_modexp(start0, false);
     if (!c->ev_turn) HIPCHK(c, hipEventCreateWithFlags(&c->ev_turn, hipEventDisableTiming));
     HIPCHK(c, hipEventRecord(c->ev_turn, s));
     g.last = c->ev_turn; g.owner = c;
   } else {
     HIPCHK(c, rec(9, s));
-    if (total) launch_modexp(start0);
+    if (total) launch_modexp(start0, false);
   }
   HIPCHK(c, rec(2, s));
   if (upload_tbs) {
@@ -653,7 +663,7 @@
     hipLaunchKernelGGL(k_plan<2>, dim3((n_items + PLAN_ITEMS - 1) / PLAN_ITEMS), dim3(PLAN_BLOCK), 0, s, pl, c->kt, *plan_q);
     const uint32_t* const start1 = cnt_p + 8;
     if (c->have_dsa_keys) launch_dsa_inv(s, start1);
-    launch_modexp(start1);
+    launch_modexp(start1, true);
     launch_compare(start1);
     if (c->have_dsa_keys) launch_dsa(start1);
   }
@@ -1041,6 +1051,7 @@
     c->seen_keyring_gen = r->keyring_gen;
   }
   c->early_exit = r->early_exit;
+  c->plan_margin = r->plan_margin; c->second_pass_limit = r->second_pass_limit;
   if (c->seen_quorum_gen != r->quorum_gen) {
     for (auto& q : c->quorums) { q.member.release(); q.ids.release(); }
     c->quorums.clear();
@@ -1096,6 +1107,8 @@
   if (const char* e = getenv("BFTKV_MULTIEXP_LANES")) c->multiexp_lanes = (uint32_t)atoi(e);
   if (const char* e = getenv("BFTKV_RSAV_LANES")) c->rsav_lanes = (uint32_t)atoi(e);
   if (const char* e = getenv("BFTKV_MULTIEXP_BLOCK")) c->multiexp_block = (uint32_t)atoi(e);
+  if (const char* e = getenv("BFTKV_PLAN_MARGIN")) c->plan_margin = std::max(-1, atoi(e));
+  if (const char* e = getenv("BFTKV_SECOND_PASS_LIMIT")) c->second_pass_limit = (uint32_t)strtoul(e, nullptr, 10);
   if (const char* e = getenv("BFTKV_DSA_INV")) c->dsa_inv_mode = !strcmp(e, "batched") ? 2u : !strcmp(e, "single") ? 1u : 0u;
   { int cus = 0; if (hipDeviceGetAttribute(&cus, hipDeviceAttributeMultiprocessorCount, device_ordinal) == hipSuccess && cus > 0) c->n_cus = (uint32_t)cus; }
   *out = c;
@@ -1110,6 +1123,7 @@
   if (rc) return rc;
   c->root = root;
   c->early_exit = root->early_exit;
+  c->plan_margin = root->plan_margin; c->second_pass_limit = root->second_pass_limit;
   c->dsa_inv_mode = root->dsa_inv_mode;
   root->n_forks.fetch_add(1);
   *out = c;
@@ -1134,7 +1148,7 @@
   (void)hipStreamSynchronize(c->stream_d);
   for (DevBuf* b : {&c->k_id, &c->k_entity, &c->k_algo, &c->k_flags, &c->k_bits, &c->k_e, &c->k_n, &c->k_r2, &c->k_n0, &c->k_q, &c->k_qbits, &c->k_dsatab, &c->k_dsaslot, &c->dsa_comb, &c->k_sorted_id, &c->k_sorted_slot, &c->k_r2w, &c->k_n29, &c->k_r2_29, &c->k_n0_29,
                     &c->chunk_arena, &c->chunk_ctr, &c->counts, &c->base, &c->total, &c->item_flags, &c->walk_scratch, &c->cert_ent, &c->sig_class, &c->mid, &c->mid64, &c->hash_mask, &c->recs, &c->digests, &c->r, &c->xr,
-                    &c->pk_list, &c->pk_list3072, &c->pk_list4096, &c->r3072, &c->r4096, &c->pk_count, &c->dsa_list, &c->dsa_u, &c->dsa_idx, &c->ids_tmp, &c->o_err, &c->o_nver, &c->o_verdict, &c->o_fenced, &c->in_tbs, &c->in_tbs_off,
+                    &c->pk_list, &c->pk_list3072, &c->pk_list4096, &c->r3072, &c->r4096, &c->pk_count, &c->dsa_list, &c->dsa_u, &c->dsa_idx, &c->ids_tmp, &c->o_err, &c->o_nver, &c->o_verdict, &c->o_fenced, &c->o_exit, &c->in_tbs, &c->in_tbs_off,
                     &c->in_ss, &c->in_ss_off, &c->in_prefix, &c->in_prefix_off, &c->in_shared, &c->in_shared_off, &c->in_seg, &c->st_tmp, &c->item_tmp, &c->bits_tmp, &c->plan_cut, &c->txt_mid32, &c->txt_mid64, &c->txt_tail, &c->txt_len})
     b->release();
   for (auto& q : c->quorums) { q.member.release(); q.ids.release(); }
@@ -1218,6 +1232,24 @@
   return 0;
 }
 
+int bftkv_gpu_set_plan_margin(bftkv_gpu_ctx* c, int margin) {
+  if (!c || margin < -1) return BFTKV_E_INVALID;
+  ctx_lock lk(c->mu);
+  if (c->root) return fail(c, BFTKV_E_STATE, "set on the root context; its forks follow");
+  KtWrite kw(c);
+  c->plan_margin = margin;
+  return 0;
+}
+
+int bftkv_gpu_set_second_pass_limit(bftkv_gpu_ctx* c, uint32_t limit) {
+  if (!c || limit == 0xFFFFFFFFu) return BFTKV_E_INVALID;
+  ctx_lock lk(c->mu);
+  if (c->root) return fail(c, BFTKV_E_STATE, "set on the root context; its forks follow");
+  KtWrite kw(c);
+  c->second_pass_limit = limit;
+  return 0;
+}
+
 int bftkv_gpu_set_hash_policy(bftkv_gpu_ctx* c, int hash_id, int state) {
   if (!c || (hash_id != HASH_MD5 && hash_id != HASH_RIPEMD160) || state < 0 || state > 2) return BFTKV_E_INVALID;
   ctx_lock lk(c->mu);
@@ -1357,8 +1389,11 @@
   HIPCHK(c, c->o_verdict.ensure(n_items));
   uint32_t* nv = nver_out ? nver_out : c->o_nver.as<uint32_t>();
   uint8_t* vd = verdict_out ? verdict_out : c->o_verdict.as<uint8_t>();
+  if (c->last_planned) HIPCHK(c, c->o_exit.ensure(sizeof(uint32_t) * n_items));
   hipLaunchKernelGGL(k_tally, dim3((n_items + 3) / 4), dim3(256), 0, c->stream, c->recs.as<SigRec>(), c->base.as<uint32_t>(),
-                     c->counts.as<uint32_t>(), n_items, c->kt, quorum_dev(c, q), vd, nv, (uint32_t*)nullptr);
+                     c->counts.as<uint32_t>(), n_items, c->kt, quorum_dev(c, q), vd, nv, (uint32_t*)nullptr,
+                     c->last_planned ? c->o_exit.as<uint32_t>() : (uint32_t*)nullptr);
+  c->last_exit_valid = c->last_planned;
   if (err_out) {
     hipLaunchKernelGGL(k_err_from_verdict, dim3((n_items + 255) / 256), dim3(256), 0, c->stream, vd, n_items, err_out);
   }
@@ -1958,7 +1993,8 @@
   HIPCHK(c, c->st_tmp.ensure(n));
   HIPCHK(c, c->item_tmp.ensure(sizeof(uint32_t) * n));
   hipLaunchKernelGGL(k_export_status, dim3((n + 255) / 256), dim3(256), 0, c->stream, c->recs.as<SigRec>(), n,
-                     c->st_tmp.as<uint8_t>(), c->item_tmp.as<uint32_t>());
+                     c->st_tmp.as<uint8_t>(), c->item_tmp.as<uint32_t>(),
+                     c->last_exit_valid ? c->o_exit.as<uint32_t>() : (const uint32_t*)nullptr, c->base.as<uint32_t>());
   HIPCHK(c, hipMemcpyAsync(st, c->st_tmp.p, n, hipMemcpyDeviceToHost, c->stream));
   if (item) HIPCHK(c, hipMemcpyAsync(item, c->item_tmp.p, sizeof(uint32_t) * n, hipMemcpyDeviceToHost, c->stream));
   HIPCHK(c, hipStreamSynchronize(c->stream));
@@ -1983,6 +2019,27 @@
   counters[2] = c->last_items;
   counters[3] = cnt[1];
   return 0;
+}
+
+int bftkv_gpu_last_plan_counters(bftkv_gpu_ctx* c, uint64_t counters[3]) {
+  if (!c || !counters) return BFTKV_E_INVALID;
+  ctx_lock lk(c->mu);
+  HIPCHK(c, hipSetDevice(c->device));
+  counters[0] = counters[1] = counters[2] = 0;
+  auto add = [&](bftkv_gpu_ctx* w) -> int {
+    uint32_t cnt[12] = {};
+    if (w->pk_count.p) HIPCHK(c, hipMemcpy(cnt, w->pk_count.p, sizeof cnt, hipMemcpyDeviceToHost));
+    const uint64_t all = (uint64_t)cnt[0] + cnt[1] + cnt[2] + cnt[3], first = (uint64_t)cnt[8] + cnt[9] + cnt[10] + cnt[11];
+    counters[0] += w->last_planned ? first : all;
+    counters[1] += w->last_planned ? all - first : 0;
+    counters[2] += w->last_planned ? cnt[0] - cnt[8] : 0;
+    return 0;
+  };
+  if (c->hb_last_pieces) {
+    for (uint32_t k = 0; k < c->hb_last_pieces; ++k) if (int rc = add(c->hb_workers[k])) return rc;
+    return 0;
+  }
+  return add(c);
 }
 
 int bftkv_gpu_last_sclk_mhz(bftkv_gpu_ctx* c, float* mhz) {
diff --git a/bftkv_amd/csrc/kernels.hip b/bftkv_amd/csrc/kernels.hip
--- a/bftkv_amd/csrc/kernels.hip
+++ b/bftkv_amd/csrc/kernels.hip
@@ -1143,6 +1143,7 @@
 static_assert(BFTKV_RSA_FORM == 28 || BFTKV_RSA_FORM == 29, "BFTKV_RSA_FORM: 28 or 29");
 
 enum : int { OP_TO_MONT = 0, OP_SQR = 1, OP_MULX = 2, OP_MULP = 3, OP_MUL1 = 4 };
+constexpr uint32_t MODEXP_NO_LIMIT = 0xFFFFFFFFu;
 
 constexpr int EM_LOW_BYTES = 84;
 constexpr int EM_LOW_LIMBS = EM_LOW_BYTES * 8 / MONT_W;
@@ -1163,7 +1164,8 @@
                                                           const uint32_t* __restrict__ pk_start_ptr,
                                                           KeyTableDev kt, uint32_t* __restrict__ r_low,
                                                           uint32_t* __restrict__ xr_scratch, uint64_t* __restrict__ clk,
-                                                          const uint32_t* __restrict__ wide_word = nullptr) {
+                                                          const uint32_t* __restrict__ wide_word = nullptr,
+                                                          uint32_t short_limit = MODEXP_NO_LIMIT) {
   static_assert(W == MONT_W || (W == 29 && L == 18 && TPI == 4 && !WIDE_ONLY), "the only form at another radix is 18 x 4 at 2^29");
   constexpr int NL = TPI * L;
   constexpr int GROUPS = MODEXP_BLOCK / TPI;
@@ -1174,6 +1176,8 @@
   __shared__ uint32_t x_sh[GROUPS * NL];
   const uint32_t count = *pk_count_ptr, start = *pk_start_ptr;
   if (start + blockIdx.x * GROUPS >= count) return;
+  if constexpr (L == 10 && TPI == 8) { if (count - start > short_limit) return; }
+  else if constexpr (TPI == 4) { if (short_limit != MODEXP_NO_LIMIT && count - start <= short_limit) return; }
   if constexpr (WIDE_ONLY) { if (*wide_word == 0u) return; }
   const uint32_t quad = threadIdx.x / TPI;
   const int qlane = threadIdx.x % TPI;
@@ -1923,7 +1927,8 @@
 __global__ void __launch_bounds__(256) k_tally(const SigRec* __restrict__ recs, const uint32_t* __restrict__ rec_base,
                                                const uint32_t* __restrict__ counts, uint32_t n_items, KeyTableDev kt,
                                                QuorumDev q, uint8_t* __restrict__ verdict, uint32_t* __restrict__ n_verified,
-                                               uint32_t* __restrict__ clique_counts ) {
+                                               uint32_t* __restrict__ clique_counts ,
+                                               uint32_t* __restrict__ exit_rec = nullptr ) {
   const uint32_t wave = (blockIdx.x * blockDim.x + threadIdx.x) >> 6;
   const uint32_t lane = threadIdx.x & 63;
   if (wave >= n_items) return;
@@ -1933,6 +1938,7 @@
   for (int c = 0; c < MAX_QC; ++c) cq[c] = 0;
   uint32_t total_ok = 0;
   uint32_t first_suff = 0xFFFFFFFFu;
+  uint32_t exit_at = 0xFFFFFFFFu;
   for (uint32_t off = 0; off < cnt; off += 64) {
     const uint32_t i = off + lane;
     bool ok = false;
@@ -1959,6 +1965,7 @@
     if (rm != 0 && first_suff == 0xFFFFFFFFu) {
       const uint32_t fl = (uint32_t)__builtin_ctzll(rm);
       first_suff = total_ok + (uint32_t)__builtin_popcountll(okm & ((fl == 63) ? ~0ull : ((1ull << (fl + 1)) - 1)));
+      exit_at = off + fl;
     }
     total_ok += (uint32_t)__builtin_popcountll(okm);
   }
@@ -1973,6 +1980,7 @@
     verdict[wave] = (is_quorum ? V_IS_QUORUM : 0) | (is_thr ? V_IS_THRESHOLD : 0) | (is_suff ? V_IS_SUFFICIENT : 0) |
                     (reject ? V_REJECT : 0);
     n_verified[wave] = is_suff ? first_suff : total_ok;
+    if (exit_rec) exit_rec[wave] = exit_at;
     if (clique_counts)
       for (int c = 0; c < MAX_QC; ++c) clique_counts[(uint64_t)wave * MAX_QC + c] = cq[c];
   }
@@ -2139,10 +2147,15 @@
   if (threadIdx.x == 0) __hip_atomic_store(host_flag, seq, __ATOMIC_RELEASE, __HIP_MEMORY_SCOPE_SYSTEM);
 }
 
-__global__ void k_export_status(const SigRec* __restrict__ recs, uint32_t n, uint8_t* __restrict__ st, uint32_t* __restrict__ item) {
+__global__ void k_export_status(const SigRec* __restrict__ recs, uint32_t n, uint8_t* __restrict__ st, uint32_t* __restrict__ item,
+                                const uint32_t* __restrict__ exit_rec = nullptr, const uint32_t* __restrict__ rec_base = nullptr) {
   uint32_t i = blockIdx.x * blockDim.x + threadIdx.x;
   if (i >= n) return;
-  const uint8_t v = recs[i].status;
+  uint8_t v = recs[i].status;
+  if (exit_rec) {
+    const uint32_t it = recs[i].item, ex = exit_rec[it];
+    if (ex != 0xFFFFFFFFu && i - rec_base[it] > ex) v = (uint8_t)ST_NOT_EXAMINED;
+  }
   st[i] = v >= ST_PENDING_PARSE ? (uint8_t)ST_NOT_EXAMINED : v;
   if (item) item[i] = recs[i].item;
 }
diff --git a/include/bftkv_gpu.h b/include/bftkv_gpu.h
--- a/include/bftkv_gpu.h
+++ b/include/bftkv_gpu.h
@@ -105,6 +105,8 @@
 #define BFTKV_HOST_PIPELINE_TIGHT_BOUND 0x400u
 int bftkv_gpu_host_pipeline_trace(bftkv_gpu_ctx* ctx, float* out, uint32_t cap, uint32_t* n_out);
 int bftkv_gpu_set_early_exit(bftkv_gpu_ctx* ctx, int on);
+int bftkv_gpu_set_plan_margin(bftkv_gpu_ctx* ctx, int margin);
+int bftkv_gpu_set_second_pass_limit(bftkv_gpu_ctx* ctx, uint32_t limit);
 
 int bftkv_gpu_signature_verify(bftkv_gpu_ctx* ctx, uint32_t n_items,
                                const uint8_t* tbs_blob, const uint64_t* tbs_off,
@@ -177,6 +179,7 @@
 
 int bftkv_gpu_last_statuses(bftkv_gpu_ctx* ctx, uint8_t* status_out, uint32_t* item_out, uint32_t cap, uint32_t* n_out);
 int bftkv_gpu_last_counters(bftkv_gpu_ctx* ctx, uint64_t counters[4]);
+int bftkv_gpu_last_plan_counters(bftkv_gpu_ctx* ctx, uint64_t counters[3]);
 
 int bftkv_gpu_signers(bftkv_gpu_ctx* ctx, uint32_t n_items, const uint8_t* ss_blob, const uint64_t* ss_off,
                       uint64_t* ids_out, uint64_t* ids_off_out, uint64_t cap);
```
